# JunkyByte/deepcharuco

Hardware: AMD Instinct MI355X
Metric: frames/sec end-to-end (detect+refine) at 320x240; corner-id match vs ref (higher is better)
Workload: dtype f32; 1 GPU; bs=32/GPU x1 GPU(s) = 32 frames of 320x240, full detect+refine pipeline (BASELINE configs[1]); preset=cfg2, batch_per_gpu=32, global_batch=32, height=240, width=320, corner_pool_per_gpu=2048, frames=board, truncated_frames=0, distinct_ids_in_batch=16, parallelism=frames sharded, 1 process/GPU x1

## Files before the change

### deepcharuco_amd/_lib.py

```python
from __future__ import annotations

import ctypes as C
import os
import subprocess
from typing import Optional

_HERE = os.path.dirname(os.path.abspath(__file__))
LIB_PATH = os.environ.get("DCX_LIB") or os.path.join(_HERE, "libdeepcharuco_amd.so")
CSRC = os.path.join(_HERE, "csrc")

_lib: Optional[C.CDLL] = None


class DcxError(RuntimeError):
    def __init__(self, code: int, where: str):
        self.code = code
        try:
            msg = lib().dcx_error_string(code).decode()
        except Exception:
            msg = "?"
        super().__init__(f"{where} failed with code {code}: {msg}")


def build(force: bool = False, verbose: bool = False) -> str:
    cmd = ["make", "-C", CSRC, "-j4"]
    if force:
        subprocess.run(["make", "-C", CSRC, "clean"], check=True, capture_output=not verbose)
    res = subprocess.run(cmd, capture_output=True, text=True)
    if res.returncode != 0:
        raise RuntimeError("building libdeepcharuco_amd.so failed:\n" + res.stdout[-4000:] + res.stderr[-8000:])
    if verbose:
        print(res.stdout)
    return LIB_PATH


_vp, _i, _l, _sz = C.c_void_p, C.c_int, C.c_long, C.c_size_t

SIGNATURES = {
    "dcx_version": (C.c_char_p, []),
    "dcx_error_string": (C.c_char_p, [_i]),
    "dcx_detector_create": (_i, [C.POINTER(_vp), C.POINTER(_vp), _i, _i]),
    "dcx_detector_destroy": (_i, [_vp]),
    "dcx_refiner_create": (_i, [C.POINTER(_vp), C.POINTER(_vp), _i]),
    "dcx_refiner_destroy": (_i, [_vp]),
    "dcx_detector_workspace_bytes": (_sz, [_vp, _i, _i, _i]),
    "dcx_refiner_workspace_bytes": (_sz, [_vp, _i]),
    "dcx_bgr2gray": (_i, [_vp, _l, _i, _i, _i, _i, _vp, _vp]),
    "dcx_bgr2gray_legacy14": (_i, [_vp, _l, _i, _i, _i, _i, _vp, _vp]),
    "dcx_pre_image": (_i, [_vp, _vp, _sz, _vp]),
    "dcx_detector_forward": (_i, [_vp, _vp, _l, _i, _vp, _i, _i, _i, _vp, _sz, _vp, _vp, _vp]),
    "dcx_detector_decode": (_i, [_vp, _i, _i, _i, _vp, _i, _i, _vp, _vp, _vp, _vp, _vp]),
    "dcx_pred_to_keypoints": (_i, [_vp, _vp, _i, _i, _i, _i, _i, _i, _i, _vp, _vp, _vp, _vp, _vp]),
    "dcx_label_to_keypoints": (_i, [_vp, _vp, _i, _i, _i, _i, _i, _vp, _vp, _vp, _vp, _vp]),
    "dcx_build_patch_table": (_i, [_vp, _vp, _i, _i, _vp, _vp, _vp]),
    "dcx_extract_patches_u8": (_i, [_vp, _l, _i, _i, _i, _vp, _vp, _i, _vp, _vp]),
    "dcx_extract_patches_f32": (_i, [_vp, _i, _i, _vp, _vp, _i, _vp, _vp]),
    "dcx_refiner_forward": (_i, [_vp, _vp, _i, _vp, _vp, _vp, _sz, _vp, _vp, _vp, _vp]),
    "dcx_argmax2d": (_i, [_vp, _i, _i, _i, _vp, _vp]),
    "dcx_pipeline_workspace_bytes": (_sz, [_vp, _vp, _i, _i, _i, _i]),
    "dcx_infer_batch": (_i, [_vp, _vp, _vp, _l, _i, _i, _i, _i, _i, _i, _i, _vp, _sz, _vp, _vp, _vp, _vp, _vp, _vp]),
    "dcx_front_bytes": (_sz, [_vp, _i, _i, _i]),
    "dcx_detector_front": (_i, [_vp, _vp, _l, _i, _i, _i, _i, _i, _vp, _sz, _vp]),
    "dcx_infer_batch_prefetched": (_i, [_vp, _vp, _vp, _l, _i, _i, _i, _i, _i, _i, _i, _vp, _sz, _vp, _sz, _vp, _vp, _vp, _vp, _vp,
                                       _vp, _vp]),
    "dcx_stream_synchronize": (_i, [_vp]),
    "dcx_solve_pnp_pool": (_i, [_vp, _vp, _vp, _vp, _i, _i, _i, _i, C.c_double, C.POINTER(C.c_double), C.POINTER(C.c_double), _i,
                               _vp, _vp, _vp]),
    "dcx_solve_pnp_ransac_workspace_bytes": (_sz, [_i, _i, _i]),
    "dcx_solve_pnp_ransac_pool": (_i, [_vp, _vp, _vp, _vp, _i, _i, _i, _i, C.c_double, C.POINTER(C.c_double), C.POINTER(C.c_double), _i,
                                      _i, C.c_double, _i, C.c_uint, _vp, _sz, _vp, _vp, _vp, _vp, _vp]),
    "dcx_calibrate_workspace_bytes": (_sz, [_i]),
    "dcx_calibrate_pool": (_i, [_vp, _vp, _vp, _vp, _i, _i, _i, _i, C.c_double, _i, _i, _vp, _sz, _vp, _vp,
                               C.POINTER(C.c_double), _vp]),
    "dcx_calibrate_flags_workspace_bytes": (_sz, [_i, _i]),
    "dcx_calibrate_flags_pool": (_i, [_vp, _vp, _vp, _vp, _i, _i, _i, _i, C.c_double, _i, _i, _i, C.POINTER(C.c_double),
                                     C.POINTER(C.c_double), _i, _vp, _sz, _vp, _vp, C.POINTER(C.c_double), _vp]),
    "dcx_calibrate_ransac_workspace_bytes": (_sz, [_i, _i, _i]),
    "dcx_calibrate_ransac_pool": (_i, [_vp, _vp, _vp, _vp, _i, _i, _i, _i, C.c_double, _i, _i, _i, C.c_double, C.c_double, _i, _i,
                                      C.c_uint, _vp, _sz, _vp, _vp, _vp, _vp, C.POINTER(C.c_double), _vp]),
    "dcx_stereo_calibrate_workspace_bytes": (_sz, [_i, _i, _i]),
    "dcx_stereo_calibrate_pool": (_i, [_vp] * 10 + [_i, _i, _i, _i, _i, C.c_double, C.POINTER(C.c_double), C.POINTER(C.c_double), _i,
                                      C.POINTER(C.c_double), C.POINTER(C.c_double), _i, _vp, _sz, _vp, _vp, _vp,
                                      C.POINTER(C.c_double), _vp]),
    "dcx_stereo_calibrate_models_pool": (_i, [_vp] * 10 + [_i, _i, _i, _i, _i, C.c_double, C.POINTER(C.c_double),
                                             C.POINTER(C.c_double), _i, C.POINTER(C.c_double), C.POINTER(C.c_double), _i, _i, _i,
                                             _vp, _sz, _vp, _vp, _vp, C.POINTER(C.c_double), _vp]),
    "dcx_rig_calibrate_workspace_bytes": (_sz, [_i, _i, C.POINTER(C.c_int)]),
    "dcx_rig_calibrate_pool": (_i, [_i, _vp, _i, _i, _i, C.c_double, _vp, _sz, _vp, _vp, _vp, C.POINTER(C.c_int32),
                                   C.POINTER(C.c_double), _vp]),
    "dcx_rig_calibrate_models_pool": (_i, [_i, _vp, C.POINTER(C.c_int), _i, _i, _i, C.c_double, _vp, _sz, _vp, _vp, _vp,
                                          C.POINTER(C.c_int32), C.POINTER(C.c_double), _vp]),
    "dcx_rig_pose_workspace_bytes": (_sz, [_i, _i, C.POINTER(C.c_int)]),
    "dcx_rig_pose_pool": (_i, [_i, _vp, C.POINTER(C.c_int), C.POINTER(C.c_double), _i, _i, _i, C.c_double, _vp, _sz, _vp, _vp, _vp, _vp,
                              _vp, _vp, _vp]),
    "dcx_undistort_rectify_map": (_i, [C.POINTER(C.c_double), C.POINTER(C.c_double), _i, C.POINTER(C.c_double),
                                      C.POINTER(C.c_double), _i, _i, _vp, _vp]),
    "dcx_rectify_points_pool": (_i, [_vp, _vp, _i, C.POINTER(C.c_double), C.POINTER(C.c_double), _i, C.POINTER(C.c_double),
                                    C.POINTER(C.c_double), _vp, _vp]),
    "dcx_remap_u8": (_i, [_vp, _l, _i, _i, _i, _i, _vp, _i, _i, _i, _i, _vp, _vp]),
    "dcx_fisheye_solve_pnp_pool": (_i, [_vp, _vp, _vp, _vp, _i, _i, _i, _i, C.c_double, C.POINTER(C.c_double), C.POINTER(C.c_double),
                                       _vp, _vp, _vp]),
    "dcx_fisheye_solve_pnp_ransac_pool": (_i, [_vp, _vp, _vp, _vp, _i, _i, _i, _i, C.c_double, C.POINTER(C.c_double),
                                              C.POINTER(C.c_double), _i, C.c_double, _i, C.c_uint, _vp, _sz, _vp, _vp, _vp, _vp, _vp]),
    "dcx_fisheye_calibrate_workspace_bytes": (_sz, [_i]),
    "dcx_fisheye_calibrate_pool": (_i, [_vp, _vp, _vp, _vp, _i, _i, _i, _i, C.c_double, _i, _i, C.c_double, _vp, _sz, _vp, _vp,
                                       C.POINTER(C.c_double), _vp]),
    "dcx_calibrate_uncertainty_workspace_bytes": (_sz, [_i]),
    "dcx_calibrate_uncertainty_pool": (_i, [_vp, _vp, _vp, _vp, _i, _i, _i, _i, C.c_double, _i, C.POINTER(C.c_double), _vp, _vp, _vp,
                                           _vp, _sz, _vp, _vp, _vp]),
    "dcx_fisheye_undistort_rectify_map": (_i, [C.POINTER(C.c_double), C.POINTER(C.c_double), C.POINTER(C.c_double),
                                              C.POINTER(C.c_double), _i, _i, _vp, _vp]),
    "dcx_fisheye_rectify_points_pool": (_i, [_vp, _vp, _i, C.POINTER(C.c_double), C.POINTER(C.c_double), C.POINTER(C.c_double),
                                            C.POINTER(C.c_double), _vp, _vp]),
    "dcx_resize_u8": (_i, [_vp, _l, _i, _i, _i, _i, _i, _i, _i, _i, _vp, _vp]),
    "dcx_resize_area_u8": (_i, [_vp, _l, _i, _i, _i, _i, _i, _i, _i, _vp, _vp]),
    "dcx_sgm_workspace_bytes": (_sz, [_i, _i, _i, _i]),
    "dcx_sgm_u8": (_i, [_vp, _l, _i, _vp, _l, _i, _i, _i, _i, _i, _i, _i, _i, _i, _i, _vp, _vp, _sz, _vp]),
    "dcx_sgm_u8_paths": (_i, [_vp, _l, _i, _vp, _l, _i, _i, _i, _i, _i, _i, _i, _i, _i, _i, _i, _vp, _vp, _sz, _vp]),
    "dcx_disparity_to_points": (_i, [_vp, _i, _i, _i, _i, C.POINTER(C.c_double), _vp, _vp]),
    "dcx_filter_speckles_workspace_bytes": (_sz, [_i, _i, _i]),
    "dcx_filter_speckles_s16": (_i, [_vp, _vp, _i, _i, _i, _i, _i, _i, _vp, _sz, _vp]),
    "dcx_conv_layer": (_i, [_vp, _i, _i, _i, _i, _vp, _vp, _vp, _vp, _vp, _vp, _i, _i, _i, _i, _i, _i, _vp, _vp]),
    "dcx_nchw_to_c4": (_i, [_vp, _i, _i, _i, _i, _vp, _vp]),
    "dcx_c4_to_nchw": (_i, [_vp, _i, _i, _i, _i, _vp, _vp]),
    "dcx_set_timing": (_i, [_i]),
    "dcx_get_timing": (_i, []),
    "dcx_profile_enabled": (_i, []),
    "dcx_last_timings": (_i, [C.POINTER(C.c_float)]),
    "dcx_conv_pick_name": (C.c_char_p, [_i] * 8),
    "dcx_conv_pick_name_ups": (C.c_char_p, [_i] * 9),
    "dcx_set_deterministic": (_i, [_i]),
    "dcx_get_deterministic": (_i, []),
    "dcx_calibrate_xcd": (_i, [_i, C.POINTER(C.c_float), _vp]),
    "dcx_set_xcd_weights": (_i, [C.POINTER(C.c_float)]),
    "dcx_get_xcd_weights": (_i, [C.POINTER(C.c_float)]),
    "dcx_set_tail_fence": (_i, [_i]),
    "dcx_get_tail_fence": (_i, []),
    "dcx_profile_enable": (_i, [_i]),
    "dcx_profile_count": (_i, []),
    "dcx_profile_filter": (_i, [_i]),
    "dcx_profile_sample": (_i, [_i]),
    "dcx_profile_fetch": (_i, [C.POINTER(_i), C.POINTER(_i), C.POINTER(_i), C.POINTER(C.c_double), C.POINTER(C.c_float), _i]),
    "dcx_profile_kernel_name": (C.c_char_p, [_i]),
    "dcx_profile_clocks": (_i, [C.POINTER(C.c_float), _i]),
    "dcx_profile_probe_words": (_i, [_i, C.POINTER(C.c_ulonglong)]),
}


def lib() -> C.CDLL:
    global _lib
    if _lib is None:
        if not os.path.exists(LIB_PATH):
            raise RuntimeError(
                f"{LIB_PATH} not found: build it with `python -c 'import __graft_entry__ as g; g.build()'` "
                f"or `make -C {CSRC}`. deepcharuco_amd has no CPU / stock-PyTorch fallback.")
        handle = C.CDLL(LIB_PATH)
        for name, (res, args) in SIGNATURES.items():
            fn = getattr(handle, name)
            fn.restype = res
            fn.argtypes = args
        _lib = handle
    return _lib


def csrc_sha256() -> str:
    import hashlib
    h = hashlib.sha256()
    for name in sorted(os.listdir(CSRC)):
        if name.endswith((".hip", ".h")):
            with open(os.path.join(CSRC, name), "rb") as f:
                h.update(name.encode())
                h.update(f.read())
    return h.hexdigest()


def check(rc: int, where: str) -> None:
    if rc != 0:
        raise DcxError(rc, where)


def ptr(t) -> Optional[int]:
    if t is None:
        return None
    return t.data_ptr()


def current_stream() -> int:
    import torch
    return torch.cuda.current_stream().cuda_stream
```

### deepcharuco_amd/csrc/dcx_api.hip

```cpp
#include "dcx_common.h"

#include <math.h>
#include <stdlib.h>
#include <string.h>
#include <new>
#include <vector>

namespace {

constexpr float kBnEps = 1e-5f;

inline size_t align_up(size_t v, size_t a) { return (v + a - 1) / a * a; }


std::vector<float> pack_conv(const float* w, int cout, int cin, int ks, int cout_pad) {
    const int taps = ks * ks, cq = cin / 4;
    std::vector<float> out((size_t)taps * cq * cout_pad * 4, 0.0f);
    for (int o = 0; o < cout; ++o)
        for (int i = 0; i < cin; ++i)
            for (int t = 0; t < taps; ++t)
                out[(((size_t)t * cq + (i >> 2)) * cout_pad + o) * 4 + (i & 3)] = w[((size_t)o * cin + i) * taps + t];
    return out;
}

std::vector<float> pack_conv_wino2(const float* w, int cout, int cin, int cout_pad) {
    const int cq = cin / 4;
    std::vector<float> out((size_t)16 * cq * cout_pad * 4, 0.0f);
    for (int o = 0; o < cout; ++o)
        for (int i = 0; i < cin; ++i) {
            const float* g = w + ((size_t)o * cin + i) * 9;
            float h[4][3], u[4][4];
            for (int kx = 0; kx < 3; ++kx) {
                const float g0 = g[kx], g1 = g[3 + kx], g2 = g[6 + kx];
                h[0][kx] = g0; h[1][kx] = ((g0 + g1) + g2) * 0.5f; h[2][kx] = ((g0 - g1) + g2) * 0.5f; h[3][kx] = g2;
            }
            for (int xi = 0; xi < 4; ++xi) {
                u[xi][0] = h[xi][0]; u[xi][1] = ((h[xi][0] + h[xi][1]) + h[xi][2]) * 0.5f;
                u[xi][2] = ((h[xi][0] - h[xi][1]) + h[xi][2]) * 0.5f; u[xi][3] = h[xi][2];
            }
            for (int pos = 0; pos < 16; ++pos)
                out[(((size_t)pos * cq + (i >> 2)) * cout_pad + o) * 4 + (i & 3)] = u[pos >> 2][pos & 3];
        }
    return out;
}

std::vector<float> pack_conv_ups2(const float* w, int cout, int cin, int cout_pad) {
    const int cq = cin / 4;
    std::vector<float> out((size_t)16 * cq * cout_pad * 4, 0.0f);
    static const int lo[2][2] = {{0, 1}, {0, 2}}, hi[2][2] = {{0, 2}, {1, 2}};
    for (int o = 0; o < cout; ++o)
        for (int i = 0; i < cin; ++i) {
            const float* g = w + ((size_t)o * cin + i) * 9;
            for (int ph = 0; ph < 4; ++ph)
                for (int tap = 0; tap < 4; ++tap) {
                    const int a = ph >> 1, b = ph & 1, dy = tap >> 1, dx = tap & 1;
                    float r[3];
                    for (int kx = 0; kx < 3; ++kx) {
                        r[kx] = g[lo[a][dy] * 3 + kx];
                        for (int ky = lo[a][dy] + 1; ky <= hi[a][dy]; ++ky) r[kx] = r[kx] + g[ky * 3 + kx];
                    }
                    float v = r[lo[b][dx]];
                    for (int kx = lo[b][dx] + 1; kx <= hi[b][dx]; ++kx) v = v + r[kx];
                    out[(((size_t)(ph * 4 + tap) * cq + (i >> 2)) * cout_pad + o) * 4 + (i & 3)] = v;
                }
        }
    return out;
}

std::vector<float> pack_conv_ups2w(const float* w, int cout, int cin, int cout_pad) {
    const int cq = cin / 4;
    const std::vector<float> ph = pack_conv_ups2(w, cout, cin, cout_pad);
    std::vector<float> out((size_t)36 * cq * cout_pad * 4, 0.0f);
    const size_t plane = (size_t)cq * cout_pad * 4;
    for (int p = 0; p < 4; ++p)
        for (size_t e = 0; e < plane; ++e) {
            float wc[2][3];
            for (int dy = 0; dy < 2; ++dy) {
                const float g0 = ph[(size_t)(p * 4 + dy * 2 + 0) * plane + e], g1 = ph[(size_t)(p * 4 + dy * 2 + 1) * plane + e];
                wc[dy][0] = g0; wc[dy][1] = g0 + g1; wc[dy][2] = g1;
            }
            for (int nu = 0; nu < 3; ++nu) {
                out[(size_t)(p * 9 + 0 * 3 + nu) * plane + e] = wc[0][nu];
                out[(size_t)(p * 9 + 1 * 3 + nu) * plane + e] = wc[0][nu] + wc[1][nu];
                out[(size_t)(p * 9 + 2 * 3 + nu) * plane + e] = wc[1][nu];
            }
        }
    return out;
}

void fold_bn(const float* gamma, const float* bbeta, const float* mean, const float* var, int c, int c_pad,
             std::vector<float>& alpha, std::vector<float>& beta) {
    alpha.assign(c_pad, 0.0f);
    beta.assign(c_pad, 0.0f);
    for (int i = 0; i < c; ++i) {
        const float inv = 1.0f / sqrtf(var[i] + kBnEps);
        const float a = gamma[i] * inv;
        alpha[i] = a;
        beta[i] = bbeta[i] - mean[i] * a;
    }
}

std::vector<float> pad_vec(const float* v, int c, int c_pad) {
    std::vector<float> out(c_pad, 0.0f);
    memcpy(out.data(), v, sizeof(float) * c);
    return out;
}

struct DevLayer {
    float* w = nullptr;
    float* w_wino2 = nullptr;
    float* w_ups2w = nullptr;
    float* bias = nullptr;
    float* alpha = nullptr;
    float* beta = nullptr;
    int cin = 0, cout = 0, cout_pad = 0, ks = 3;
};

int upload(const std::vector<float>& h, float** d) {
    DCX_CHECK_HIP(hipMalloc((void**)d, h.size() * sizeof(float)));
    DCX_CHECK_HIP(hipMemcpy(*d, h.data(), h.size() * sizeof(float), hipMemcpyHostToDevice));
    return 0;
}

void free_layer(DevLayer& l) {
    if (l.w) (void)hipFree(l.w);
    if (l.w_wino2) (void)hipFree(l.w_wino2);
    if (l.w_ups2w) (void)hipFree(l.w_ups2w);
    if (l.bias) (void)hipFree(l.bias);
    if (l.alpha) (void)hipFree(l.alpha);
    if (l.beta) (void)hipFree(l.beta);
    l = DevLayer();
}

struct HostConv {
    const float* w; const float* b;
    const float* g; const float* be; const float* mu; const float* var;
};

int make_layer(const HostConv& h, int cin, int cout, int ks, DevLayer* out, bool ups_input = false) {
    DevLayer l;
    l.cin = cin; l.cout = cout; l.ks = ks;
    l.cout_pad = dcx_conv_cout_pad(cout);
    int rc = upload(pack_conv(h.w, cout, cin, ks, l.cout_pad), &l.w);
    if (rc == 0) rc = upload(pad_vec(h.b, cout, l.cout_pad), &l.bias);
    if (rc == 0 && h.g != nullptr) {
        std::vector<float> al, be;
        fold_bn(h.g, h.be, h.mu, h.var, cout, l.cout_pad, al, be);
        for (int i = 0; i < cout; ++i) be[i] = fmaf(h.b[i], al[i], be[i]);
        rc = upload(al, &l.alpha);
        if (rc == 0) rc = upload(be, &l.beta);
        if (rc == 0 && ks == 3) rc = upload(pack_conv_wino2(h.w, cout, cin, l.cout_pad), &l.w_wino2);
        if (rc == 0 && ks == 3 && ups_input) rc = upload(pack_conv_ups2w(h.w, cout, cin, l.cout_pad), &l.w_ups2w);
    }
    if (rc != 0) { free_layer(l); return rc; }
    *out = l;
    return 0;
}

int make_first_layer(const HostConv& h, DevLayer* out) {
    DevLayer l;
    l.cin = 1; l.cout = 64; l.cout_pad = 64; l.ks = 3;
    std::vector<float> w(9 * 64);
    for (int o = 0; o < 64; ++o)
        for (int t = 0; t < 9; ++t) w[t * 64 + o] = h.w[o * 9 + t];
    std::vector<float> al, be;
    fold_bn(h.g, h.be, h.mu, h.var, 64, 64, al, be);
    int rc = upload(w, &l.w);
    if (rc == 0) rc = upload(pad_vec(h.b, 64, 64), &l.bias);
    if (rc == 0) rc = upload(al, &l.alpha);
    if (rc == 0) rc = upload(be, &l.beta);
    if (rc != 0) { free_layer(l); return rc; }
    *out = l;
    return 0;
}

bool g_timing = false;
hipEvent_t g_ev[5];
bool g_ev_ok = false;
int timing_mark(int i, hipStream_t s) {
    if (!g_timing) return 0;
    if (!g_ev_ok) {
        for (auto& e : g_ev) DCX_CHECK_HIP(hipEventCreate(&e));
        g_ev_ok = true;
    }
    DCX_CHECK_HIP(hipEventRecord(g_ev[i], s));
    return 0;
}

}

struct dcx_detector {
    int n_ids = 16;
    DevLayer first;
    DevLayer enc[7];
    DevLayer heads_a;
    DevLayer head_loc, head_ids;
};

struct dcx_refiner {
    DevLayer first;
    DevLayer mid[9];
    DevLayer head_a;
    float* head_w = nullptr;
    float head_b = 0.f;
};

namespace {

struct Carve {
    size_t off = 0;
    size_t take(size_t bytes) { const size_t at = off; off = align_up(off + bytes, 256); return at; }
};

int check_pool(int pool) { return pool <= 0 || pool > (1 << 22) ? DCX_E_SHAPE : 0; }

struct DetWs {
    size_t buf0, buf1, loc, ids, codes, conf, total;
    int ids_quads;
};
DetWs det_layout(int n_ids, int b, int h, int w) {
    DetWs L;
    const size_t hw = (size_t)h * w, cells = (size_t)(h / 8) * (w / 8);
    L.ids_quads = (n_ids + 1 + 3) / 4;
    Carve c;
    L.buf0 = c.take((size_t)b * 64 * hw * 4);
    L.buf1 = c.take((size_t)b * 16 * hw * 4);
    L.loc = c.take((size_t)b * 68 * cells * 4);
    L.ids = c.take((size_t)b * L.ids_quads * 4 * cells * 4);
    L.codes = c.take((size_t)b * cells * 4);
    L.conf = c.take((size_t)b * cells * 8);
    L.total = c.off;
    return L;
}

struct RefWs {
    size_t buf0, buf1, pval, pidx, total;
};
constexpr int kRefTiles = 32;
RefWs ref_layout(int p) {
    RefWs L;
    Carve c;
    L.buf0 = c.take((size_t)p * 65536 * 4);
    L.buf1 = c.take((size_t)p * 65536 * 4);
    L.pval = c.take((size_t)p * kRefTiles * 4);
    L.pidx = c.take((size_t)p * kRefTiles * 4);
    L.total = c.off;
    return L;
}

DcxConvArgs conv_args(const DevLayer& l, const float* in, int n, int in_cq_total, int in_cq_off, int hin, int win,
                      int ups, int pad, float* out, int out_cq_total, const int* n_limit) {
    DcxConvArgs a;
    memset(&a, 0, sizeof(a));
    a.in = in; a.w = l.w; a.w_wino2 = l.w_wino2; a.w_ups2w = l.w_ups2w; a.bias = l.bias; a.alpha = l.alpha; a.beta = l.beta; a.out = out;
    a.n_limit = n_limit;
    a.n = n; a.in_cq_total = in_cq_total; a.in_cq_off = in_cq_off; a.cin = l.cin;
    a.hin = hin; a.win = win; a.ups = ups; a.pad = pad;
    a.ho = (hin << ups) + 2 * pad - (l.ks - 1);
    a.wo = (win << ups) + 2 * pad - (l.ks - 1);
    a.out_cq_total = out_cq_total; a.out_cq_off = 0;
    a.cout_pad = l.cout_pad; a.cout_quads = (l.cout + 3) / 4; a.cout_real = l.cout;
    return a;
}

}

extern "C" const char* dcx_version(void) { return "deepcharuco_amd 0.1 (gfx950, fp32 MFMA)"; }

extern "C" const char* dcx_error_string(int code) {
    switch (code) {
        case 0: return "ok";
        case DCX_E_ARG: return "DCX_E_ARG: null pointer or bad scalar argument";
        case DCX_E_SHAPE: return "DCX_E_SHAPE: unsupported shape (H/W below 8, patches not 24x24, batch x kmax too large, ...)";
        case DCX_E_WS: return "DCX_E_WS: workspace too small";
        case DCX_E_NIDS: return "DCX_E_NIDS: n_ids outside [1, 63] or dust_bin outside [0, 255]";
        default: return code > 0 ? hipGetErrorString((hipError_t)code) : "unknown dcx error";
    }
}

extern "C" int dcx_detector_create(dcx_detector** out, const float* const* t, int n_tensors, int n_ids) {
    if (!out || !t) return DCX_E_ARG;
    if (n_ids < 1 || n_ids > 63) return DCX_E_NIDS;
    if (n_tensors != 64) return DCX_E_ARG;
    for (int i = 0; i < n_tensors; ++i)
        if (!t[i]) return DCX_E_ARG;
    if (const int rc = dcx_xcd_init()) return rc;
    dcx_detector* d = new (std::nothrow) dcx_detector();
    if (!d) return (int)hipErrorOutOfMemory;
    d->n_ids = n_ids;
    auto hc = [&](int base, bool bn) {
        return HostConv{t[base], t[base + 1], bn ? t[base + 2] : nullptr, bn ? t[base + 3] : nullptr,
                        bn ? t[base + 4] : nullptr, bn ? t[base + 5] : nullptr};
    };
    static const int enc_cin[7] = {64, 64, 64, 64, 128, 128, 128};
    static const int enc_cout[7] = {64, 64, 64, 128, 128, 128, 128};
    int rc = make_first_layer(hc(0, true), &d->first);
    for (int i = 0; rc == 0 && i < 7; ++i) rc = make_layer(hc(6 + 6 * i, true), enc_cin[i], enc_cout[i], 3, &d->enc[i]);
    if (rc == 0) {
        const HostConv pa = hc(48, true), da = hc(56, true);
        const size_t wsz = (size_t)256 * 128 * 9;
        std::vector<float> w(2 * wsz), b(512), g(512), be(512), mu(512), var(512);
        memcpy(w.data(), pa.w, wsz * 4); memcpy(w.data() + wsz, da.w, wsz * 4);
        auto cat = [](std::vector<float>& dst, const float* x, const float* y) {
            memcpy(dst.data(), x, 256 * 4); memcpy(dst.data() + 256, y, 256 * 4);
        };
        cat(b, pa.b, da.b); cat(g, pa.g, da.g); cat(be, pa.be, da.be); cat(mu, pa.mu, da.mu); cat(var, pa.var, da.var);
        rc = make_layer(HostConv{w.data(), b.data(), g.data(), be.data(), mu.data(), var.data()}, 128, 512, 3,
                        &d->heads_a);
    }
    if (rc == 0) rc = make_layer(hc(54, false), 256, 65, 1, &d->head_loc);
    if (rc == 0) rc = make_layer(hc(62, false), 256, n_ids + 1, 1, &d->head_ids);
    if (rc != 0) { dcx_detector_destroy(d); return rc; }
    *out = d;
    return 0;
}

extern "C" int dcx_detector_destroy(dcx_detector* d) {
    if (!d) return 0;
    free_layer(d->first);
    for (auto& l : d->enc) free_layer(l);
    free_layer(d->heads_a); free_layer(d->head_loc); free_layer(d->head_ids);
    delete d;
    return 0;
}

extern "C" size_t dcx_detector_workspace_bytes(const dcx_detector* det, int batch, int height, int width) {
    if (!det || batch <= 0 || height <= 0 || width <= 0) return 0;
    return det_layout(det->n_ids, batch, height, width).total;
}

namespace {
int detector_front(const dcx_detector* det, const uint8_t* d_frames_u8, long frame_stride, int pitch, int pix,
                   const float* d_images_f32, int batch, int h, int w, float* out, int32_t* zero_words, int n_zero, hipStream_t s) {
    int rc;
    const int pt0 = dcx_prof_begin(DCX_PROF_CONV1A, batch, 0, s);
    if (d_frames_u8)
        rc = dcx_launch_conv1_u8(d_frames_u8, frame_stride, pitch, pix, batch, h, w, 1, det->first.w, det->first.bias,
                                 det->first.alpha, det->first.beta, out, nullptr, zero_words, n_zero, s);
    else
        rc = dcx_launch_conv1_f32(d_images_f32, (long)h * w, w, batch, h, w, 1, det->first.w, det->first.bias,
                                  det->first.alpha, det->first.beta, out, nullptr, s);
    if (rc) return rc;
    return dcx_prof_end(pt0, s);
}

int detector_run(const dcx_detector* det, const uint8_t* d_frames_u8, long frame_stride, int pitch, int pix,
                 const float* d_images_f32, int batch, int height, int width, void* d_ws, size_t ws_bytes,
                 bool with_heads, float* d_loc_nchw, float* d_ids_nchw, int32_t* zero_words, int n_zero, const float* act0,
                 void* stream) {
    if (!det || !d_ws) return DCX_E_ARG;
    if ((d_frames_u8 == nullptr) == (d_images_f32 == nullptr)) return DCX_E_ARG;
    if (batch <= 0 || height < 8 || width < 8) return DCX_E_SHAPE;
    const DetWs L = det_layout(det->n_ids, batch, height, width);
    if (ws_bytes < L.total) return DCX_E_WS;
    hipStream_t s = (hipStream_t)stream;
    char* ws = (char*)d_ws;
    float* buf0 = (float*)(ws + L.buf0);
    float* buf1 = (float*)(ws + L.buf1);
    float* loc = (float*)(ws + L.loc);
    float* ids = (float*)(ws + L.ids);
    const int h = height, w = width;
    int rc;
    if (act0 == nullptr && (rc = detector_front(det, d_frames_u8, frame_stride, pitch, pix, d_images_f32, batch, h, w, buf0,
                                                zero_words, n_zero, s)))
        return rc;
    struct Step { int layer, div, pool; };
    static const Step steps[7] = {{0, 1, 1}, {1, 2, 0}, {2, 2, 1}, {3, 4, 0}, {4, 4, 1}, {5, 8, 0}, {6, 8, 0}};
    const float* src = act0 ? act0 : buf0;
    float* dst = buf1;
    for (const Step& st : steps) {
        const DevLayer& l = det->enc[st.layer];
        DcxConvArgs a = conv_args(l, src, batch, l.cin / 4, 0, h / st.div, w / st.div, 0, 1, dst, l.cout / 4, nullptr);
        rc = dcx_launch_conv_mfma(a, 3, st.pool, DCX_EPI_BNRELU, s);
        if (rc) return rc;
        src = dst; dst = dst == buf1 ? buf0 : buf1;
    }
    const int hc = h / 8, wc = w / 8;
    {
        DcxConvArgs a = conv_args(det->heads_a, src, batch, 32, 0, hc, wc, 0, 1, dst, 128, nullptr);
        rc = dcx_launch_conv_mfma(a, 3, 0, DCX_EPI_BNRELU, s);
        if (rc) return rc;
    }
    if (!with_heads) return 0;
    {
        DcxConvArgs a = conv_args(det->head_loc, dst, batch, 128, 0, 1, hc * wc, 0, 0, loc, 17, nullptr);
        rc = dcx_launch_conv_mfma(a, 1, 0, DCX_EPI_RAW, s);
        if (rc) return rc;
    }
    {
        DcxConvArgs a = conv_args(det->head_ids, dst, batch, 128, 64, 1, hc * wc, 0, 0, ids, L.ids_quads, nullptr);
        rc = dcx_launch_conv_mfma(a, 1, 0, DCX_EPI_RAW, s);
        if (rc) return rc;
    }
    if (d_loc_nchw) { rc = dcx_c4_to_nchw(loc, batch, 65, hc, wc, d_loc_nchw, stream); if (rc) return rc; }
    if (d_ids_nchw) { rc = dcx_c4_to_nchw(ids, batch, det->n_ids + 1, hc, wc, d_ids_nchw, stream); if (rc) return rc; }
    return 0;
}
}

extern "C" int dcx_detector_forward(const dcx_detector* det, const uint8_t* d_frames_u8, long frame_stride, int pitch,
                                    const float* d_images_f32, int batch, int height, int width, void* d_ws,
                                    size_t ws_bytes, float* d_loc_nchw, float* d_ids_nchw, void* stream) {
    return detector_run(det, d_frames_u8, frame_stride, pitch, DCX_PIX_GRAY8, d_images_f32, batch, height, width, d_ws, ws_bytes, true,
                        d_loc_nchw, d_ids_nchw, nullptr, 0, nullptr, stream);
}

extern "C" int dcx_detector_decode(const dcx_detector* det, int batch, int height, int width, void* d_ws,
                                   int dust_bin, int kmax, int32_t* d_counts, int32_t* d_rows, int32_t* d_loc_argmax,
                                   int32_t* d_ids_argmax, void* stream) {
    if (!det || !d_ws) return DCX_E_ARG;
    if (batch <= 0 || height < 8 || width < 8) return DCX_E_SHAPE;
    const DetWs L = det_layout(det->n_ids, batch, height, width);
    const int hc = height / 8, wc = width / 8;
    const long cells = (long)hc * wc;
    char* ws = (char*)d_ws;
    DcxLogitView lv{(const float*)(ws + L.loc), 17 * 4 * cells, 4 * cells, 4, 1};
    DcxLogitView iv{(const float*)(ws + L.ids), (long)L.ids_quads * 4 * cells, 4 * cells, 4, 1};
    return dcx_launch_decode(lv, iv, batch, 65, det->n_ids + 1, hc, wc, dust_bin, kmax, d_counts, d_rows,
                             d_loc_argmax, d_ids_argmax, (int32_t*)(ws + L.codes), (hipStream_t)stream);
}

extern "C" int dcx_refiner_create(dcx_refiner** out, const float* const* t, int n_tensors) {
    if (!out || !t) return DCX_E_ARG;
    if (n_tensors != 68) return DCX_E_ARG;
    for (int i = 0; i < n_tensors; ++i)
        if (!t[i]) return DCX_E_ARG;
    if (const int rc = dcx_xcd_init()) return rc;
    dcx_refiner* r = new (std::nothrow) dcx_refiner();
    if (!r) return (int)hipErrorOutOfMemory;
    auto hc = [&](int base) { return HostConv{t[base], t[base + 1], t[base + 2], t[base + 3], t[base + 4], t[base + 5]}; };
    static const int cin[9] = {64, 64, 128, 128, 128, 128, 128, 128, 64};
    static const int cout[9] = {64, 128, 128, 128, 128, 128, 128, 64, 64};
    int rc = make_first_layer(hc(0), &r->first);
    for (int i = 0; rc == 0 && i < 9; ++i) rc = make_layer(hc(6 + 6 * i), cin[i], cout[i], 3, &r->mid[i], i == 5 || i == 7);
    if (rc == 0) rc = make_layer(hc(60), 64, 64, 3, &r->head_a, true);
    if (rc == 0) {
        std::vector<float> hw(t[66], t[66] + 64);
        rc = upload(hw, &r->head_w);
        r->head_b = t[67][0];
    }
    if (rc != 0) { dcx_refiner_destroy(r); return rc; }
    *out = r;
    return 0;
}

extern "C" int dcx_refiner_destroy(dcx_refiner* r) {
    if (!r) return 0;
    free_layer(r->first);
    for (auto& l : r->mid) free_layer(l);
    free_layer(r->head_a);
    if (r->head_w) (void)hipFree(r->head_w);
    delete r;
    return 0;
}

extern "C" size_t dcx_refiner_workspace_bytes(const dcx_refiner* rf, int max_patches) {
    if (!rf || max_patches <= 0) return 0;
    return ref_layout(max_patches).total;
}

namespace {
struct FrameSrc { const uint8_t* frames; long frame_stride; int pitch, pix, height, width; };
int refiner_run(const dcx_refiner* rf, const float* d_patches, const FrameSrc* fsrc, int max_patches, int n_hint,
                const int32_t* d_total, const int32_t* d_table, void* d_ws, size_t ws_bytes, int32_t* d_corners, float* d_xy,
                float* d_heat, void* stream) {
    if (!rf || !d_ws || ((d_patches == nullptr) == (fsrc == nullptr))) return DCX_E_ARG;
    if (fsrc != nullptr && (d_total == nullptr || d_table == nullptr)) return DCX_E_ARG;
    if (d_xy != nullptr && d_table == nullptr) return DCX_E_ARG;
    if (const int rc = check_pool(max_patches)) return rc;
    const RefWs L = ref_layout(max_patches);
    if (ws_bytes < L.total) return DCX_E_WS;
    hipStream_t s = (hipStream_t)stream;
    char* ws = (char*)d_ws;
    float* buf0 = (float*)(ws + L.buf0);
    float* buf1 = (float*)(ws + L.buf1);
    const int p = max_patches;
    const int* lim = d_total;
    const int pt0 = dcx_prof_begin(DCX_PROF_PATCHES, p, lim != nullptr, s);
    int rc = fsrc != nullptr
        ? dcx_launch_conv1_patches_u8(fsrc->frames, fsrc->frame_stride, fsrc->pitch, fsrc->pix, fsrc->height, fsrc->width, d_table, d_total, p, n_hint,
                                      rf->first.w, rf->first.bias, rf->first.alpha, rf->first.beta, buf0, s)
        : dcx_launch_conv1_f32(d_patches, 576, 24, p, 24, 24, 0, rf->first.w, rf->first.bias, rf->first.alpha,
                               rf->first.beta, buf0, lim, s);
    if (rc) return rc;
    if ((rc = dcx_prof_end(pt0, s))) return rc;
    struct Step { int layer, hin, ups, pad, pool; };
    static const Step steps[9] = {
        {0, 22, 0, 0, 0},
        {1, 20, 0, 0, 0},
        {2, 18, 0, 0, 1},
        {3, 8, 0, 1, 0},
        {4, 8, 0, 1, 0},
        {5, 8, 1, 1, 0},
        {6, 16, 0, 1, 0},
        {7, 16, 1, 1, 0},
        {8, 32, 0, 1, 0},
    };
    float* src = buf0;
    float* dst = buf1;
    for (const Step& st : steps) {
        const DevLayer& l = rf->mid[st.layer];
        DcxConvArgs a = conv_args(l, src, p, l.cin / 4, 0, st.hin, st.hin, st.ups, st.pad, dst, l.cout / 4, lim);
        a.n_hint = lim != nullptr ? n_hint : 0;
        rc = dcx_launch_conv_mfma(a, 3, st.pool, DCX_EPI_BNRELU, s);
        if (rc) return rc;
        float* t = src; src = dst; dst = t;
    }
    int heat_tiles = 0;
    {
        DcxConvArgs a = conv_args(rf->head_a, src, p, 16, 0, 32, 32, 1, 1, nullptr, 16, lim);
        a.head_w = rf->head_w; a.head_b = rf->head_b; a.heat = d_heat;
        a.part_val = (float*)(ws + L.pval); a.part_idx = (int*)(ws + L.pidx);
        heat_tiles = dcx_conv_heat_tiles(a.ho, a.wo, a.w_ups2w != nullptr ? 1 : 0);
        if (heat_tiles <= 0 || heat_tiles > kRefTiles) return DCX_E_SHAPE;
        rc = dcx_launch_conv_mfma(a, 3, 0, DCX_EPI_HEAT, s);
        if (rc) return rc;
    }
    const int pt1 = dcx_prof_begin(DCX_PROF_FINALIZE, p, lim != nullptr, s);
    rc = dcx_launch_refine_finalize((const float*)(ws + L.pval), (const int*)(ws + L.pidx), heat_tiles, 64, p, lim,
                                    d_table, d_corners, d_xy, s);
    if (rc) return rc;
    return dcx_prof_end(pt1, s);
}
}

extern "C" int dcx_refiner_forward(const dcx_refiner* rf, const float* d_patches, int max_patches,
                                   const int32_t* d_total, const int32_t* d_table, void* d_ws, size_t ws_bytes,
                                   int32_t* d_corners, float* d_xy, float* d_heat, void* stream) {
    return refiner_run(rf, d_patches, nullptr, max_patches, 0, d_total, d_table, d_ws, ws_bytes, d_corners, d_xy, d_heat, stream);
}

namespace {
struct PipeWs { size_t det, table, ctrl, ref, total; int ctrl_words; };
inline int ctrl_word_count(int b) { return 64 + b; }
struct FrontWs { size_t act, ctrl, total; int ctrl_words; };
FrontWs front_layout(int b, int h, int w) {
    FrontWs F;
    Carve c;
    F.act = c.take((size_t)b * 64 * h * w * 4);
    F.ctrl_words = ctrl_word_count(b);
    F.ctrl = c.take((size_t)F.ctrl_words * 4);
    F.total = c.off;
    return F;
}
PipeWs pipe_layout(const dcx_detector* det, const dcx_refiner* rf, int b, int h, int w, int pool) {
    PipeWs L;
    Carve c;
    L.det = c.take(det_layout(det->n_ids, b, h, w).total);
    L.table = c.take((size_t)pool * 16);
    L.ctrl_words = ctrl_word_count(b);
    L.ctrl = c.take((size_t)L.ctrl_words * 4);
    L.ref = c.take(rf ? ref_layout(pool).total : 0);
    L.total = c.off;
    return L;
}
}

extern "C" size_t dcx_pipeline_workspace_bytes(const dcx_detector* det, const dcx_refiner* rf, int batch, int height,
                                               int width, int pool) {
    if (!det || batch <= 0 || height <= 0 || width <= 0 || pool <= 0) return 0;
    return pipe_layout(det, rf, batch, height, width, pool).total;
}

extern "C" size_t dcx_front_bytes(const dcx_detector* det, int batch, int height, int width) {
    if (!det || batch <= 0 || height <= 0 || width <= 0) return 0;
    return front_layout(batch, height, width).total;
}

namespace {
int check_batch_args(const dcx_detector* det, const uint8_t* d_frames_u8, int pitch, int pixel_format, int batch, int height,
                     int width) {
    if (!det || !d_frames_u8) return DCX_E_ARG;
    if (!dcx_pix_valid(pixel_format)) return DCX_E_ARG;
    if (batch <= 0 || batch > (1 << 20) || height < 8 || width < 8) return DCX_E_SHAPE;
    if (pitch < width * dcx_pix_bpp(pixel_format)) return DCX_E_SHAPE;
    return 0;
}
}

extern "C" int dcx_detector_front(const dcx_detector* det, const uint8_t* d_frames_u8, long frame_stride, int pitch,
                                  int pixel_format, int batch, int height, int width, void* d_front, size_t front_bytes,
                                  void* stream) {
    if (!d_front) return DCX_E_ARG;
    if (const int rc = check_batch_args(det, d_frames_u8, pitch, pixel_format, batch, height, width)) return rc;
    const FrontWs F = front_layout(batch, height, width);
    if (front_bytes < F.total) return DCX_E_WS;
    char* front = (char*)d_front;
    return detector_front(det, d_frames_u8, frame_stride, pitch, pixel_format, nullptr, batch, height, width, (float*)(front + F.act),
                          (int32_t*)(front + F.ctrl), F.ctrl_words, (hipStream_t)stream);
}

namespace {
int infer_range(const dcx_detector* det, const dcx_refiner* rf, const uint8_t* d_frames_u8, long frame_stride, int pitch, int pix,
                int batch, int height, int width, int dust_bin, int pool, char* ws, size_t ws_bytes, char* front,
                hipEvent_t detector_done, int32_t* d_counts, int32_t* d_starts, int32_t* d_rows, float* d_xy, float* d_conf,
                hipStream_t s, bool timing) {
    void* stream = (void*)s;
    const PipeWs L = pipe_layout(det, rf, batch, height, width, pool);
    if (ws_bytes < L.total) return DCX_E_WS;
    int rc = timing ? timing_mark(0, s) : 0;
    if (rc) return rc;
    const FrontWs F = front_layout(batch, height, width);
    int32_t* ctrl = (int32_t*)(front ? front + F.ctrl : ws + L.ctrl);
    rc = detector_run(det, d_frames_u8, frame_stride, pitch, pix, nullptr, batch, height, width, ws + L.det, L.table - L.det,
                      false, nullptr, nullptr, ctrl, L.ctrl_words, front ? (const float*)(front + F.act) : nullptr, stream);
    if (rc) return rc;
    if (detector_done) DCX_CHECK_HIP(hipEventRecord(detector_done, s));
    if (timing && (rc = timing_mark(1, s))) return rc;
    int32_t* table = (int32_t*)(ws + L.table);
    {
        const DetWs D = det_layout(det->n_ids, batch, height, width);
        const int hc = height / 8, wc = width / 8;
        const float* act = (const float*)(ws + L.det + D.buf0);
        int32_t* codes = (int32_t*)(ws + L.det + D.codes);
        DcxPoolOut po;
        po.tickets = ctrl + 64; po.cursor = ctrl; po.counts = d_counts; po.starts = d_starts; po.rows = d_rows;
        po.table = rf ? table : nullptr; po.conf = d_conf; po.conf_cells = (float*)(ws + L.det + D.conf);
        po.wc = wc; po.pool = pool;
        const int pt = dcx_prof_begin(DCX_PROF_TAIL, batch, 0, s);
        rc = dcx_launch_tail(act, batch, hc * wc, det->head_loc.w, det->head_loc.bias, det->head_ids.w, det->head_ids.bias,
                             det->head_ids.cout_pad, det->n_ids + 1, dust_bin, codes, nullptr, nullptr, &po, s);
        if (rc) return rc;
        if ((rc = dcx_prof_end(pt, s))) return rc;
    }
    if (timing && (rc = timing_mark(2, s))) return rc;
    if (rf == nullptr) return timing ? timing_mark(3, s) : 0;
    const long expect = (long)batch * det->n_ids;
    const FrameSrc src{d_frames_u8, frame_stride, pitch, pix, height, width};
    rc = refiner_run(rf, nullptr, &src, pool, (int)(expect < pool ? expect : pool), ctrl, table,
                     ws + L.ref, L.total - L.ref, nullptr, d_xy, nullptr, stream);
    if (rc) return rc;
    return timing ? timing_mark(3, s) : 0;
}
}

extern "C" int dcx_infer_batch(const dcx_detector* det, const dcx_refiner* rf, const uint8_t* d_frames_u8,
                               long frame_stride, int pitch, int pixel_format, int batch, int height, int width, int dust_bin,
                               int pool, void* d_ws, size_t ws_bytes, int32_t* d_counts, int32_t* d_starts, int32_t* d_rows,
                               float* d_xy, float* d_conf, void* stream) {
    if (!d_ws || !d_counts || !d_starts || !d_rows) return DCX_E_ARG;
    if (rf != nullptr && d_xy == nullptr) return DCX_E_ARG;
    if (const int rc = check_batch_args(det, d_frames_u8, pitch, pixel_format, batch, height, width)) return rc;
    if (const int rc = check_pool(pool)) return rc;
    if (const int rc = dcx_check_dust_bin(dust_bin)) return rc;
    hipStream_t s = (hipStream_t)stream;
    char* ws = (char*)d_ws;
    return infer_range(det, rf, d_frames_u8, frame_stride, pitch, pixel_format, batch, height, width, dust_bin, pool, ws, ws_bytes,
                       nullptr, nullptr, d_counts, d_starts, d_rows, d_xy, d_conf, s, true);
}

extern "C" int dcx_infer_batch_prefetched(const dcx_detector* det, const dcx_refiner* rf, const uint8_t* d_frames_u8,
                                          long frame_stride, int pitch, int pixel_format, int batch, int height, int width,
                                          int dust_bin, int pool, void* d_ws, size_t ws_bytes, void* d_front, size_t front_bytes,
                                          int32_t* d_counts, int32_t* d_starts, int32_t* d_rows, float* d_xy, float* d_conf,
                                          void* detector_done_event, void* stream) {
    if (!d_ws || !d_front || !d_counts || !d_starts || !d_rows) return DCX_E_ARG;
    if (rf != nullptr && d_xy == nullptr) return DCX_E_ARG;
    if (const int rc = check_batch_args(det, d_frames_u8, pitch, pixel_format, batch, height, width)) return rc;
    if (const int rc = check_pool(pool)) return rc;
    if (const int rc = dcx_check_dust_bin(dust_bin)) return rc;
    if (front_bytes < front_layout(batch, height, width).total) return DCX_E_WS;
    return infer_range(det, rf, d_frames_u8, frame_stride, pitch, pixel_format, batch, height, width, dust_bin, pool, (char*)d_ws,
                       ws_bytes, (char*)d_front, (hipEvent_t)detector_done_event, d_counts, d_starts, d_rows, d_xy, d_conf,
                       (hipStream_t)stream, true);
}

extern "C" int dcx_stream_synchronize(void* stream) { return (int)hipStreamSynchronize((hipStream_t)stream); }

extern "C" int dcx_set_timing(int enabled) { g_timing = enabled != 0; return 0; }
extern "C" int dcx_get_timing(void) { return g_timing ? 1 : 0; }

extern "C" int dcx_last_timings(float* h_ms4) {
    if (!h_ms4) return DCX_E_ARG;
    if (!g_ev_ok) return DCX_E_ARG;
    DCX_CHECK_HIP(hipEventElapsedTime(&h_ms4[0], g_ev[0], g_ev[1]));
    DCX_CHECK_HIP(hipEventElapsedTime(&h_ms4[1], g_ev[1], g_ev[2]));
    DCX_CHECK_HIP(hipEventElapsedTime(&h_ms4[2], g_ev[2], g_ev[3]));
    DCX_CHECK_HIP(hipEventElapsedTime(&h_ms4[3], g_ev[0], g_ev[3]));
    return 0;
}

extern "C" int dcx_conv_layer(const float* d_in, int n, int cin, int hin, int win, const float* h_w, const float* h_b,
                              const float* h_g, const float* h_be, const float* h_mu, const float* h_var, int cout,
                              int ksize, int pad, int ups, int pool, int relu, float* d_out, void* stream) {
    if (!d_in || !h_w || !h_b || !d_out) return DCX_E_ARG;
    if (cin % 32 != 0 || (ksize != 3 && ksize != 1) || n <= 0) return DCX_E_SHAPE;
    const bool bn = h_g != nullptr;
    if (bn != (relu != 0)) return DCX_E_ARG;
    if (bn && (!h_be || !h_mu || !h_var)) return DCX_E_ARG;
    if (const int rc = dcx_xcd_init()) return rc;
    DevLayer l;
    int rc = make_layer(HostConv{h_w, h_b, h_g, h_be, h_mu, h_var}, cin, cout, ksize, &l, ups != 0);
    if (rc) return rc;
    DcxConvArgs a;
    if (ksize == 1) {
        if (pad != 0 || ups != 0 || pool != 0) { free_layer(l); return DCX_E_SHAPE; }
        a = conv_args(l, d_in, n, cin / 4, 0, 1, hin * win, 0, 0, d_out, (cout + 3) / 4, nullptr);
    } else {
        a = conv_args(l, d_in, n, cin / 4, 0, hin, win, ups, pad, d_out, (cout + 3) / 4, nullptr);
    }
    rc = dcx_launch_conv_mfma(a, ksize, pool, bn ? DCX_EPI_BNRELU : DCX_EPI_RAW, (hipStream_t)stream);
    hipError_t e = hipStreamSynchronize((hipStream_t)stream);
    free_layer(l);
    if (rc) return rc;
    return (int)e;
}
```

### deepcharuco_amd/csrc/dcx_common.h

```cpp
#pragma once
#include <hip/hip_runtime.h>
#include <stdint.h>
#include <stddef.h>

#include "../../include/deepcharuco_amd.h"

#define DCX_CHECK_HIP(expr)                              \
    do {                                                 \
        hipError_t _e = (expr);                          \
        if (_e != hipSuccess) return (int)_e;            \
    } while (0)


enum DcxEpilogue {
    DCX_EPI_BNRELU = 0,
    DCX_EPI_RAW = 1,
    DCX_EPI_HEAT = 2,
};

struct DcxConvArgs {
    const float* in;
    const float* w;
    const float* w_wino2;
    const float* w_ups2w;
    const float* bias;
    const float* alpha;
    const float* beta;
    float* out;
    const int* n_limit;
    unsigned long long* clk_probe;
    int probe_u0;
    const float* head_w;
    float head_b;
    float* heat;
    float* part_val;
    int* part_idx;
    int n;
    int n_hint;
    int in_cq_total, in_cq_off;
    int cin;
    int hin, win;
    int ups;
    int pad;
    int ho, wo;
    int out_cq_total, out_cq_off;
    int cout_pad;
    int cout_quads;
    int cout_real;
    int tiles_x, tiles_y;
    int xcd_walk;
    const int* xcd_cum;
    unsigned long long* xcd_stat;
    int ct_outer;
};

int dcx_launch_conv_mfma(DcxConvArgs a, int ks, int pool, int epi, hipStream_t stream);
int dcx_xcd_init();
int dcx_conv_cout_pad(int cout);
int dcx_conv_heat_tiles(int ho, int wo, int ups);

enum { DCX_PROF_CONV1A = 100, DCX_PROF_PATCHES = 101, DCX_PROF_TAIL = 102, DCX_PROF_FINALIZE = 103 };
int dcx_prof_begin(int kernel_id, int n, int limited, hipStream_t s);
int dcx_prof_end(int token, hipStream_t s);


constexpr bool dcx_pix_valid(int pix) { return pix == DCX_PIX_GRAY8 || pix == DCX_PIX_BGR8 || pix == DCX_PIX_BGR8_LEGACY14; }
constexpr int dcx_pix_bpp(int pix) { return pix == DCX_PIX_GRAY8 ? 1 : 3; }
int dcx_launch_conv1_u8(const uint8_t* frames, long frame_stride, int pitch, int pix, int n, int h, int w, int pad,
                        const float* w9x64, const float* bias, const float* alpha, const float* beta,
                        float* out_c4, const int* n_limit, int32_t* zero_words, int n_zero, hipStream_t s);
int dcx_launch_conv1_f32(const float* images, long image_stride, int pitch, int n, int h, int w, int pad,
                         const float* w9x64, const float* bias, const float* alpha, const float* beta,
                         float* out_c4, const int* n_limit, hipStream_t s);

struct DcxLogitView {
    const float* p;
    long sb, sq, sp, sc;
};
inline int dcx_check_dust_bin(int dust_bin, int last = 255) { return dust_bin < 0 || dust_bin > last ? DCX_E_NIDS : 0; }
int dcx_launch_decode(DcxLogitView loc, DcxLogitView ids, int batch, int n_loc, int n_ids1, int hc, int wc,
                      int dust_bin, int kmax, int32_t* counts, int32_t* rows,
                      int32_t* loc_argmax, int32_t* ids_argmax, int32_t* codes_scratch, hipStream_t s);
struct DcxPoolOut {
    int32_t* tickets;
    int32_t* cursor;
    int32_t* counts;
    int32_t* starts;
    int32_t* rows;
    int32_t* table;
    float* conf;
    float* conf_cells;
    int wc, pool;
};
int dcx_launch_tail(const float* act_c4_512, int batch, int cells, const float* w_loc, const float* b_loc,
                    const float* w_ids, const float* b_ids, int ids_cout_pad, int n_ids1, int dust_bin,
                    int32_t* codes, int32_t* loc_argmax, int32_t* ids_argmax, const DcxPoolOut* po, hipStream_t s);
int dcx_launch_compact(const int32_t* codes, int batch, int hc, int wc, int dust_bin, int kmax, int32_t* counts,
                       int32_t* rows, hipStream_t s);
int dcx_launch_conv1_patches_u8(const uint8_t* frames, long frame_stride, int pitch, int pix, int h, int w, const int32_t* table,
                                const int* total, int max_patches, int n_hint, const float* w9x64, const float* bias,
                                const float* alpha, const float* beta, float* out_c4, hipStream_t s);
int dcx_launch_refine_finalize(const float* part_val, const int* part_idx, int tiles, int wo,
                               int max_patches, const int* total, const int32_t* table,
                               int32_t* corners, float* xy, hipStream_t s);
```

### deepcharuco_amd/csrc/dcx_conv_mfma.hip

```cpp
#include "dcx_conv_mfma.h"
#include "dcx_conv_wino2h.h"
#include "dcx_conv_wino2hs.h"
#include "dcx_conv_wino2p.h"
#include "dcx_conv_wino2ps.h"

#include <stdlib.h>
#include <string.h>
#include <atomic>
#include <mutex>
#include <vector>

namespace {

enum { FAM_DIRECT = 0,
       FAM_W2H = 3,
       FAM_W2P = 4 };

struct CfgEntry {
    int cout_tile, cap, th, tw, ks, pool, epi, acc_tiles;
    int inlane;
    int group;
    int fam;
    int (*launch)(DcxConvArgs, hipStream_t);
    const char* name;
};

#define DCX_CFG(WM, WN, MT, NT, TH, TW, KS, POOL, EPI)                                              \
    { WM * MT * 32, WN * NT * 32, TH, TW, KS, POOL, EPI, MT * NT, ((POOL) != 0 && MT == 1 && NT == 4) ? 1 : 0, 1, FAM_DIRECT, \
      &dcx_conv_launch_cfg<DcxConvCfg<WM, WN, MT, NT, TH, TW, KS, (POOL) != 0, EPI>>,                 \
      "dcx_conv_mfma_kernel<DcxConvCfg<" #WM "," #WN "," #MT "," #NT "," #TH "," #TW "," #KS "," #POOL "," #EPI ">>" }

#define DCX_W2HCFG(TH, TW, POOL, G)                                                                   \
    { 64, 128, TH, TW, 3, POOL, DCX_EPI_BNRELU, 8, 0, G, FAM_W2H,                                            \
      &dcx_conv_wino2h_launch_cfg<DcxWino2hCfg<TH, TW, (POOL) != 0, G>>,                                   \
      "dcx_conv_wino2h_kernel<DcxWino2hCfg<" #TH "," #TW "," #POOL "," #G ">>" }
#define DCX_W2HCFG_S(TH, TW, POOL)                                                                    \
    { 64, 64, TH, TW, 3, POOL, DCX_EPI_BNRELU, 4, 0, 1, FAM_W2H,                                             \
      &dcx_conv_wino2h_launch_cfg<DcxWino2hCfg<TH, TW, (POOL) != 0, 1, 1>>,                                \
      "dcx_conv_wino2h_kernel<DcxWino2hCfg<" #TH "," #TW "," #POOL ",1,1>>" }

#define DCX_W2HSCFG(POOL, CG)                                                                         \
    { 16 * CG, 64, 8, 8, 3, POOL, DCX_EPI_BNRELU, 1, 0, 1, FAM_W2H,                                          \
      &dcx_conv_wino2hs_launch_cfg<DcxWino2hsCfg<(POOL) != 0, CG>>,                                        \
      "dcx_conv_wino2hs_kernel<DcxWino2hsCfg<" #POOL "," #CG ">>" }

#define DCX_W2PCFG(TH, TW, EPI, G)                                                                    \
    { 64, 128, TH, TW, 3, 0, EPI, 5, 0, G, FAM_W2P,                                                          \
      &dcx_conv_wino2p_launch_cfg<DcxWino2pCfg<TH, TW, EPI, G>>,                                           \
      "dcx_conv_wino2p_kernel<DcxWino2pCfg<" #TH "," #TW "," #EPI "," #G ">>" }

#define DCX_W2PSCFG(CG)                                                                               \
    { 16 * CG, 64, 8, 8, 3, 0, DCX_EPI_BNRELU, 1, 0, 1, FAM_W2P,                                             \
      &dcx_conv_wino2ps_launch_cfg<DcxWino2psCfg<CG>>,                                                     \
      "dcx_conv_wino2ps_kernel<DcxWino2psCfg<" #CG ">>" }

const CfgEntry kCfgs[] = {
    DCX_CFG(1, 4, 2, 2, 8, 32, 3, 0, DCX_EPI_BNRELU),
    DCX_CFG(2, 2, 1, 1, 8, 8, 3, 0, DCX_EPI_BNRELU),
    DCX_CFG(2, 2, 1, 1, 8, 8, 3, 1, DCX_EPI_BNRELU),
    DCX_CFG(2, 2, 1, 4, 8, 32, 3, 1, DCX_EPI_BNRELU),
    DCX_CFG(1, 4, 2, 2, 1, 256, 1, 0, DCX_EPI_RAW),
    DCX_CFG(1, 4, 2, 2, 8, 32, 3, 0, DCX_EPI_HEAT),
    DCX_W2HCFG(8, 16, 0, 1),
    DCX_W2HCFG(8, 16, 1, 1),
    DCX_W2HCFG(6, 20, 0, 1),
    DCX_W2HCFG(6, 20, 1, 1),
    DCX_W2HCFG(8, 8, 0, 2),
    DCX_W2HCFG_S(8, 8, 0),
    DCX_W2HCFG_S(8, 8, 1),
    DCX_W2HSCFG(0, 4), DCX_W2HSCFG(0, 2), DCX_W2HSCFG(0, 1),
    DCX_W2HSCFG(1, 4), DCX_W2HSCFG(1, 2), DCX_W2HSCFG(1, 1),
    DCX_W2PCFG(8, 16, DCX_EPI_BNRELU, 1),
    DCX_W2PCFG(8, 16, DCX_EPI_HEAT, 1),
    DCX_W2PCFG(8, 8, DCX_EPI_BNRELU, 2),
    DCX_W2PSCFG(4), DCX_W2PSCFG(2), DCX_W2PSCFG(1),
};

int g_deterministic = -1;
int dcx_deterministic_enabled() {
    if (g_deterministic < 0) g_deterministic = dcx_env_knob(DCX_KNOB_DETERMINISTIC) ? 1 : 0;
    return g_deterministic;
}

int family_of(int cin, int cout_pad, int ks, int pool, int epi, int ups_phase) {
    if (dcx_deterministic_enabled() || ks != 3 || epi == DCX_EPI_RAW || cin < 2 * DCX_CCH) return FAM_DIRECT;
    if (ups_phase && !pool && (epi == DCX_EPI_BNRELU || (epi == DCX_EPI_HEAT && cout_pad == 64))) return FAM_W2P;
    if (epi == DCX_EPI_BNRELU) return FAM_W2H;
    return FAM_DIRECT;
}

const CfgEntry* pick(int n, int cin, int ho, int wo, int cout_pad, int ks, int pool, int epi, int allow_group = 1, int ups = 0) {
    const CfgEntry* best = nullptr;
    double best_cost = 0.0;
    const int n_cu = dcx_device_cu_count();
    auto can_run = [&](const CfgEntry& c) {
        if (c.ks != ks || c.pool != pool || c.epi != epi || cout_pad % c.cout_tile != 0) return false;
        if (c.fam == FAM_W2P) return ups == 1 && cin >= 2 * DCX_CCH && (epi != DCX_EPI_HEAT || cout_pad == 64) &&
                                     (c.group == 1 || (ho <= 2 * c.th && wo <= 2 * c.tw));
        if (c.fam == FAM_W2H) return cin >= 2 * DCX_CCH && (c.group == 1 || (allow_group && ups == 0 && ho <= c.th && wo <= c.tw));
        return true;
    };
    const char* force = getenv("DCX_FORCE_CFG");
    if (force != nullptr && force[0] != 0) {
        for (const CfgEntry& c : kCfgs)
            if (strcmp(c.name, force) == 0 && can_run(c)) return &c;
    }
    const int fam = family_of(cin, cout_pad, ks, pool, epi, ups);
    const int units = cin / DCX_CCH;
    for (const CfgEntry& c : kCfgs) {
        if (c.fam != fam || !can_run(c)) continue;
        const int ph = c.fam == FAM_W2P ? 2 : 1;
        const long tiles = (long)((ho / ph + c.th - 1) / c.th) * ((wo / ph + c.tw - 1) / c.tw);
        const long items = (long)((n + c.group - 1) / c.group) * (cout_pad / c.cout_tile) * tiles * (ph * ph);
        const double rounds = (double)((items + n_cu - 1) / n_cu);
        double cost;
        if (c.fam == FAM_W2H) {
            double item_cost = (double)units * (64 * 64.0 + (c.tw == 20 ? 700.0 : 560.0)) + 2600.0;
            if (c.acc_tiles == 4)
                item_cost = (double)units * (32 * 64.0 + 600.0) + 2000.0;
            if (c.acc_tiles == 1) {
                const int w2hs = dcx_env_knob(DCX_KNOB_W2HS);
                const int w2hs_rounds = dcx_env_knob(DCX_KNOB_W2HS_ROUNDS);
                if (!(w2hs & (c.cout_tile / 16)) || items > (long)w2hs_rounds * n_cu) continue;
                item_cost = (double)units * (8 * 64.0 * (c.cout_tile / 16) + 400.0) + 1200.0;
                if (w2hs_rounds > 1 && items > n_cu) item_cost *= 0.8;
            }
            cost = rounds * item_cost * (1.0 + 1e-6 * (double)items);
        } else if (c.fam == FAM_W2P) {
            double item_cost = (double)units * (72 * 32.0 + 500.0) + 2400.0;
            if (c.acc_tiles == 1) {
                const int w2ps = dcx_env_knob(DCX_KNOB_W2PS);
                if (!(w2ps & (c.cout_tile / 16)) || items > n_cu) continue;
                item_cost = (double)units * (12 * 32.0 * ((3 * (c.cout_tile / 16) + 3) / 4) + 400.0) + 1200.0;
            }
            cost = rounds * item_cost * (1.0 + 1e-6 * (double)items);
        } else {
            const int steps = ks * ks * (DCX_CCH / 8);
            const double item_cost = (double)units * steps * (4 * c.acc_tiles) * 64.0 + units * 520.0
                                   + c.acc_tiles * 16 * (c.inlane ? 35.0 : (pool ? 60.0 : 40.0));
            cost = rounds * item_cost;
            if (c.cout_tile == 64 && c.cap == 256) cost *= 0.999;
        }
        if (best == nullptr || cost < best_cost) { best_cost = cost; best = &c; }
    }
    return best;
}

struct ProfRec { int kernel_id, n, limited; double flops_per_image; hipEvent_t e0, e1; int slot; };
unsigned long long* g_clk_dev = nullptr;
constexpr int kClkSlots = 1024;
constexpr int kClkWords = 64;
bool g_prof = false;
int g_prof_filter = -1;
int g_prof_every = 1;
long g_prof_seen = 0;
std::vector<ProfRec> g_recs;
std::vector<hipEvent_t> g_pool;
size_t g_pool_used = 0;

hipEvent_t prof_event() {
    if (g_pool_used == g_pool.size()) {
        hipEvent_t e;
        if (hipEventCreate(&e) != hipSuccess) return nullptr;
        g_pool.push_back(e);
    }
    return g_pool[g_pool_used++];
}

}

extern "C" const char* dcx_conv_pick_name(int n, int cin, int ho, int wo, int cout, int ks, int pool, int epi) {
    const CfgEntry* c = pick(n, cin, ho, wo, dcx_conv_cout_pad(cout), ks, pool, epi);
    return c ? c->name : "";
}
extern "C" const char* dcx_conv_pick_name_ups(int n, int cin, int ho, int wo, int cout, int ks, int pool, int epi, int ups) {
    const CfgEntry* c = pick(n, cin, ho, wo, dcx_conv_cout_pad(cout), ks, pool, epi, ups == 0, ups);
    return c ? c->name : "";
}

extern "C" int dcx_set_deterministic(int enabled) { g_deterministic = enabled ? 1 : 0; return 0; }
extern "C" int dcx_get_deterministic(void) { return dcx_deterministic_enabled(); }

extern "C" int dcx_profile_enable(int enabled) {
    g_prof = enabled != 0;
    if (g_prof) {
        g_recs.clear(); g_pool_used = 0;
        if (g_clk_dev != nullptr) {
            DCX_CHECK_HIP(hipMemset(g_clk_dev, 0, sizeof(unsigned long long) * kClkWords * kClkSlots));
            DCX_CHECK_HIP(hipStreamSynchronize(nullptr));
        }
    }
    return 0;
}
extern "C" int dcx_profile_enabled(void) { return g_prof ? 1 : 0; }
extern "C" int dcx_profile_filter(int kernel_id) { g_prof_filter = kernel_id; return 0; }
extern "C" int dcx_profile_sample(int every) { g_prof_every = every > 1 ? every : 1; g_prof_seen = 0; return 0; }
extern "C" int dcx_profile_count(void) { return (int)g_recs.size(); }
extern "C" const char* dcx_profile_kernel_name(int id) {
    const int n = (int)(sizeof(kCfgs) / sizeof(kCfgs[0]));
    switch (id) {
        case DCX_PROF_CONV1A: return "dcx_conv1_kernel (detector conv1a)";
        case DCX_PROF_PATCHES: return "dcx_conv1_patches_kernel (RefineNet conv1a + patch gather)";
        case DCX_PROF_TAIL: return "dcx_tail_kernel (1x1 heads + arg-max + compaction)";
        case DCX_PROF_FINALIZE: return "dcx_refine_finalize_kernel";
        default: break;
    }
    return id >= 0 && id < n ? kCfgs[id].name : "?";
}

int dcx_prof_begin(int kernel_id, int n, int limited, hipStream_t stream) {
    if (!g_prof || g_prof_filter >= 0) return -1;
    ProfRec r;
    r.kernel_id = kernel_id; r.n = n; r.limited = limited ? 1 : 0; r.flops_per_image = 0.0;
    r.e0 = prof_event();
    r.e1 = prof_event();
    r.slot = (int)g_recs.size();
    if (!r.e0 || !r.e1 || hipEventRecord(r.e0, stream) != hipSuccess) return -1;
    g_recs.push_back(r);
    return r.slot;
}
int dcx_prof_end(int token, hipStream_t stream) {
    if (token < 0 || token >= (int)g_recs.size()) return 0;
    DCX_CHECK_HIP(hipEventRecord(g_recs[token].e1, stream));
    return 0;
}
extern "C" int dcx_profile_probe_words(int record, unsigned long long* out64) {
    if (!out64 || record < 0 || record >= kClkSlots || g_clk_dev == nullptr) return DCX_E_ARG;
    DCX_CHECK_HIP(hipMemcpy(out64, g_clk_dev + (size_t)kClkWords * record, kClkWords * 8, hipMemcpyDeviceToHost));
    return 0;
}

extern "C" int dcx_profile_clocks(float* ghz, int max_records) {
    if (!ghz) return DCX_E_ARG;
    const int n = (int)g_recs.size() < max_records ? (int)g_recs.size() : max_records;
    std::vector<unsigned long long> h((size_t)kClkWords * kClkSlots, 0ull);
    if (g_clk_dev != nullptr) DCX_CHECK_HIP(hipMemcpy(h.data(), g_clk_dev, h.size() * 8, hipMemcpyDeviceToHost));
    for (int i = 0; i < n; ++i) {
        ghz[i] = 0.f;
        if (i < kClkSlots) {
            const unsigned long long* p = &h[(size_t)kClkWords * i];
            if (p[3] > p[1]) ghz[i] = (float)((double)(p[2] - p[0]) / (double)(p[3] - p[1]) * 0.1);
        }
    }
    return n;
}

extern "C" int dcx_profile_fetch(int* kernel_ids, int* n_images, int* limited, double* flops_per_image, float* ms,
                                 int max_records) {
    if (!kernel_ids || !n_images || !limited || !flops_per_image || !ms) return DCX_E_ARG;
    int k = 0;
    for (const ProfRec& r : g_recs) {
        if (k >= max_records) break;
        float t = 0.f;
        if (hipEventElapsedTime(&t, r.e0, r.e1) != hipSuccess) t = -1.f;
        kernel_ids[k] = r.kernel_id; n_images[k] = r.n; limited[k] = r.limited;
        flops_per_image[k] = r.flops_per_image; ms[k] = t;
        ++k;
    }
    return k;
}

int dcx_conv_cout_pad(int cout) { return cout <= 64 ? 64 : (cout + 127) / 128 * 128; }

int dcx_current_device() {
    int dev = 0;
    if (hipGetDevice(&dev) != hipSuccess || dev < 0) dev = 0;
    return dev < DCX_MAX_DEVICES ? dev : DCX_MAX_DEVICES - 1;
}

int dcx_device_cu_count() {
    static int cus[DCX_MAX_DEVICES] = {};
    const int dev = dcx_current_device();
    if (cus[dev] == 0) {
        int v = 0;
        if (hipDeviceGetAttribute(&v, hipDeviceAttributeMultiprocessorCount, dev) == hipSuccess && v > 0)
            cus[dev] = v;
        else
            cus[dev] = 256;
    }
    return cus[dev];
}

int dcx_env_knob(DcxKnob k) {
    static struct { const char* name; int unset; bool read; int value; } knobs[DCX_KNOB_COUNT] = {
        {"DCX_DETERMINISTIC", 0},
        {"DCX_XCD_WALK", 1},
        {"DCX_OCC", 0},
        {"DCX_CT_OUTER", -1},
        {"DCX_W2HS", 7},
        {"DCX_W2HS_ROUNDS", 1},
        {"DCX_W2PS", 7},
        {"DCX_PROBE_U0", 0},
    };
    if (!knobs[k].read) { const char* e = getenv(knobs[k].name); knobs[k].value = e ? atoi(e) : knobs[k].unset; knobs[k].read = true; }
    return knobs[k].value;
}

namespace {
constexpr int kXcdTables = 256;
std::mutex g_xcd_mutex;
int* g_xcd_tab[DCX_MAX_DEVICES] = {};
int g_xcd_next[DCX_MAX_DEVICES] = {};
std::atomic<const int*> g_xcd_cur[DCX_MAX_DEVICES] = {};
float g_xcd_w[DCX_MAX_DEVICES][8];
int xcd_set_locked(int dev, const float* w8) {
    if (g_xcd_tab[dev] == nullptr)
        DCX_CHECK_HIP(hipMalloc((void**)&g_xcd_tab[dev], sizeof(int) * 16 * kXcdTables));
    double sum = 0.0;
    for (int x = 0; x < 8; ++x) { g_xcd_w[dev][x] = w8 ? w8[x] : 1.0f; sum += g_xcd_w[dev][x]; }
    double acc = 0.0;
    int cum[16] = {};
    for (int x = 0; x < 8; ++x) {
        g_xcd_w[dev][x] = (float)(g_xcd_w[dev][x] / sum);
        acc += g_xcd_w[dev][x];
        cum[x + 1] = x == 7 ? 65536 : (int)(acc * 65536.0 + 0.5);
    }
    int* slot = g_xcd_tab[dev] + 16 * (g_xcd_next[dev]++ % kXcdTables);
    DCX_CHECK_HIP(hipMemcpy(slot, cum, sizeof(cum), hipMemcpyHostToDevice));
    g_xcd_cur[dev].store(slot, std::memory_order_release);
    return 0;
}
int xcd_set(int dev, const float* w8) {
    std::lock_guard<std::mutex> lk(g_xcd_mutex);
    return xcd_set_locked(dev, w8);
}
}

int dcx_xcd_init() {
    const int dev = dcx_current_device();
    std::lock_guard<std::mutex> lk(g_xcd_mutex);
    return g_xcd_cur[dev].load(std::memory_order_relaxed) != nullptr ? 0 : xcd_set_locked(dev, nullptr);
}

int dcx_fill_xcd_cum(DcxConvArgs& a) {
    a.xcd_cum = g_xcd_cur[dcx_current_device()].load(std::memory_order_acquire);
    return a.xcd_cum != nullptr ? 0 : (int)hipErrorNotInitialized;
}

extern "C" int dcx_set_xcd_weights(const float* w8) {
    if (w8 != nullptr) {
        double sum = 0.0;
        for (int x = 0; x < 8; ++x) { if (!(w8[x] > 0.f)) return DCX_E_ARG; sum += w8[x]; }
        for (int x = 0; x < 8; ++x) { const double r = 8.0 * w8[x] / sum; if (r < 0.75 || r > 1.25) return DCX_E_ARG; }
    }
    return xcd_set(dcx_current_device(), w8);
}
extern "C" int dcx_get_xcd_weights(float* w8) {
    if (!w8) return DCX_E_ARG;
    const int rc = dcx_xcd_init();
    if (rc) return rc;
    const int dev = dcx_current_device();
    std::lock_guard<std::mutex> lk(g_xcd_mutex);
    for (int x = 0; x < 8; ++x) w8[x] = 8.0f * g_xcd_w[dev][x];
    return 0;
}

namespace {
__global__ void dcx_fill_hash_kernel(float* __restrict__ p, size_t n, float lo, float scale) {
    for (size_t i = (size_t)blockIdx.x * blockDim.x + threadIdx.x; i < n; i += (size_t)gridDim.x * blockDim.x) {
        unsigned h = (unsigned)i * 2654435761u;
        h ^= h >> 15; h *= 2246822519u; h ^= h >> 13;
        p[i] = lo + scale * (float)(h >> 8) * (1.0f / 16777216.0f);
    }
}
}

extern "C" int dcx_calibrate_xcd(int rounds, float* w8_out, void* stream) {
    if (rounds < 1 || rounds > 64) return DCX_E_ARG;
    hipStream_t s = (hipStream_t)stream;
    const int n = 32, c = 64, h = 240, w = 320;
    const size_t in_elems = (size_t)n * c * h * w, out_elems = in_elems / 4, w_elems = (size_t)16 * c * c;
    float *d_in = nullptr, *d_out = nullptr, *d_w = nullptr, *d_ab = nullptr;
    unsigned long long* d_stat = nullptr;
    auto cleanup = [&]() { (void)hipFree(d_in); (void)hipFree(d_out); (void)hipFree(d_w); (void)hipFree(d_ab); (void)hipFree(d_stat); };
    hipError_t e = hipMalloc((void**)&d_in, in_elems * 4);
    if (e == hipSuccess) e = hipMalloc((void**)&d_out, out_elems * 4);
    if (e == hipSuccess) e = hipMalloc((void**)&d_w, w_elems * 4);
    if (e == hipSuccess) e = hipMalloc((void**)&d_ab, 3 * c * 4);
    if (e == hipSuccess) e = hipMalloc((void**)&d_stat, 17 * 8);
    if (e == hipSuccess) e = hipMemsetD32Async((hipDeviceptr_t)d_ab, 0x3f800000, 3 * c, s);
    if (e != hipSuccess) { cleanup(); return (int)e; }
    hipLaunchKernelGGL(dcx_fill_hash_kernel, dim3(4096), dim3(256), 0, s, d_in, in_elems, -1.0f, 2.0f);
    hipLaunchKernelGGL(dcx_fill_hash_kernel, dim3(64), dim3(256), 0, s, d_w, w_elems, -0.05f, 0.1f);
    if ((e = hipGetLastError()) != hipSuccess) { cleanup(); return (int)e; }
    DcxConvArgs a;
    memset(&a, 0, sizeof(a));
    a.in = d_in; a.w = d_w; a.w_wino2 = d_w; a.bias = d_ab; a.alpha = d_ab + c; a.beta = d_ab + 2 * c; a.out = d_out;
    a.n = n; a.in_cq_total = c / 4; a.cin = c; a.hin = h; a.win = w; a.pad = 1; a.ho = h; a.wo = w;
    a.out_cq_total = c / 4; a.cout_pad = c; a.cout_quads = c / 4; a.cout_real = c;
    const int dev = dcx_current_device();
    float keep[8];
    {
        std::lock_guard<std::mutex> lk(g_xcd_mutex);
        for (int x = 0; x < 8; ++x) keep[x] = g_xcd_cur[dev].load(std::memory_order_relaxed) != nullptr ? g_xcd_w[dev][x] : 0.125f;
        const int rc = xcd_set_locked(dev, nullptr);
        if (rc) { cleanup(); return rc; }
    }
    double speed[8] = {};
    int rc = 0, used = 0;
    for (int r = 0; r < rounds + 2 && rc == 0; ++r) {
        if ((e = hipMemsetAsync(d_stat, 0, 17 * 8, s)) != hipSuccess) { rc = (int)e; break; }
        a.xcd_stat = r >= 2 ? d_stat : nullptr;
        rc = dcx_launch_conv_mfma(a, 3, 1, DCX_EPI_BNRELU, s);
        if (rc != 0 || r < 2) continue;
        unsigned long long hst[17];
        if ((e = hipMemcpyAsync(hst, d_stat, sizeof(hst), hipMemcpyDeviceToHost, s)) != hipSuccess || (e = hipStreamSynchronize(s)) != hipSuccess) { rc = (int)e; break; }
        bool ok = hst[8] != 0;
        double dur[8];
        for (int x = 0; x < 8 && ok; ++x) {
            ok = hst[9 + x] > 0;
            if (ok) { dur[x] = (double)hst[x] / (double)hst[9 + x] - (double)hst[8]; ok = dur[x] > 0.0; }
        }
        if (!ok) continue;
        for (int x = 0; x < 8; ++x) speed[x] += 1.0 / dur[x];
        ++used;
    }
    (void)hipStreamSynchronize(s);
    cleanup();
    if (rc == 0 && used > 0) {
        float w8[8];
        for (int x = 0; x < 8; ++x) w8[x] = (float)(speed[x] / used);
        rc = dcx_set_xcd_weights(w8);
    } else if (rc == 0) {
        rc = DCX_E_SHAPE;
    }
    if (rc != 0) (void)xcd_set(dev, keep);
    if (rc == 0 && w8_out != nullptr) (void)dcx_get_xcd_weights(w8_out);
    return rc;
}

int dcx_conv_heat_tiles(int ho, int wo, int ups) {
    const CfgEntry* c = pick(1 << 20, 64, ho, wo, 64, 3, 0, DCX_EPI_HEAT, 1, ups);
    if (c == nullptr) return 0;
    if (c->fam == FAM_W2P) return 4 * ((ho / 2 + c->th - 1) / c->th) * ((wo / 2 + c->tw - 1) / c->tw);
    return ((ho + c->th - 1) / c->th) * ((wo + c->tw - 1) / c->tw);
}

int dcx_launch_conv_mfma(DcxConvArgs a, int ks, int pool, int epi, hipStream_t stream) {
    if (a.in == nullptr || a.w == nullptr || a.bias == nullptr) return DCX_E_ARG;
    if (epi != DCX_EPI_HEAT && a.out == nullptr) return DCX_E_ARG;
    if (epi != DCX_EPI_RAW && (a.alpha == nullptr || a.beta == nullptr)) return DCX_E_ARG;
    if (pool && (a.ho < 2 || a.wo < 2)) return DCX_E_SHAPE;
    const CfgEntry* c = pick(epi == DCX_EPI_HEAT ? (1 << 20) : (a.n_hint > 0 && a.n_hint < a.n ? a.n_hint : a.n), a.cin, a.ho, a.wo, a.cout_pad, ks, pool, epi,
                             a.ups == 0 && a.pad == 1,
                             (a.ups == 1 && a.pad == 1 && ks == 3 && a.w_ups2w != nullptr) ? 1 : 0);
    if (c == nullptr) return DCX_E_SHAPE;
    if (!g_prof || (g_prof_filter >= 0 && g_prof_filter != (int)(c - kCfgs))) return c->launch(a, stream);
    if (g_prof_every > 1 && (g_prof_seen++ % g_prof_every) != 0) return c->launch(a, stream);
    ProfRec r;
    r.kernel_id = (int)(c - kCfgs);
    r.n = a.n;
    r.limited = a.n_limit != nullptr;
    r.flops_per_image = 2.0 * a.cout_real * a.cin * ks * ks
                      * (double)a.ho * a.wo;
    r.e0 = prof_event();
    r.e1 = prof_event();
    r.slot = (int)g_recs.size();
    if (g_clk_dev == nullptr) {
        if (hipMalloc((void**)&g_clk_dev, sizeof(unsigned long long) * kClkWords * kClkSlots) != hipSuccess) g_clk_dev = nullptr;
        else (void)hipMemset(g_clk_dev, 0, sizeof(unsigned long long) * kClkWords * kClkSlots);
    }
    if (g_clk_dev != nullptr && r.slot < kClkSlots) a.clk_probe = g_clk_dev + (size_t)kClkWords * r.slot;
    a.probe_u0 = dcx_env_knob(DCX_KNOB_PROBE_U0);
    if (!r.e0 || !r.e1) return (int)hipErrorOutOfMemory;
    DCX_CHECK_HIP(hipEventRecord(r.e0, stream));
    const int rc = c->launch(a, stream);
    DCX_CHECK_HIP(hipEventRecord(r.e1, stream));
    if (rc == 0) g_recs.push_back(r);
    return rc;
}
```

### deepcharuco_amd/csrc/dcx_conv_shared.h

```cpp
#pragma once
#include "dcx_common.h"

typedef float dcx_f32x16 __attribute__((ext_vector_type(16)));
typedef float dcx_f32x4 __attribute__((ext_vector_type(4)));
typedef float dcx_f32x2 __attribute__((ext_vector_type(2)));
typedef unsigned int dcx_u32x4 __attribute__((ext_vector_type(4)));

#define DCX_CCH 16

__device__ __forceinline__ float4 dcx_f4_zero() { return make_float4(0.f, 0.f, 0.f, 0.f); }

__device__ __forceinline__ float dcx_vmax(float x, float y) {
    float r;
    asm("v_max_f32 %0, %1, %2" : "=v"(r) : "v"(x), "v"(y));
    return r;
}
__device__ __forceinline__ dcx_f32x2 dcx_pk_add(dcx_f32x2 x, dcx_f32x2 y) {
    dcx_f32x2 r;
    asm("v_pk_add_f32 %0, %1, %2" : "=v"(r) : "v"(x), "v"(y));
    return r;
}
__device__ __forceinline__ dcx_f32x2 dcx_pk_sub(dcx_f32x2 x, dcx_f32x2 y) {
    dcx_f32x2 r;
    asm("v_pk_add_f32 %0, %1, %2 neg_lo:[0,1] neg_hi:[0,1]" : "=v"(r) : "v"(x), "v"(y));
    return r;
}
__device__ __forceinline__ float4 dcx_sub4(const float4& x, const float4& y) {
    const dcx_f32x2 lo = dcx_pk_sub(dcx_f32x2{x.x, x.y}, dcx_f32x2{y.x, y.y}), hi = dcx_pk_sub(dcx_f32x2{x.z, x.w}, dcx_f32x2{y.z, y.w});
    return make_float4(lo.x, lo.y, hi.x, hi.y);
}
__device__ __forceinline__ float4 dcx_add4(const float4& x, const float4& y) {
    const dcx_f32x2 lo = dcx_pk_add(dcx_f32x2{x.x, x.y}, dcx_f32x2{y.x, y.y}), hi = dcx_pk_add(dcx_f32x2{x.z, x.w}, dcx_f32x2{y.z, y.w});
    return make_float4(lo.x, lo.y, hi.x, hi.y);
}
__device__ __forceinline__ float4 dcx_fmas4(const float4& x, const dcx_f32x2 s, const float4& y) {
    const dcx_f32x2 lo = __builtin_elementwise_fma(dcx_f32x2{x.x, x.y}, s, dcx_f32x2{y.x, y.y});
    const dcx_f32x2 hi = __builtin_elementwise_fma(dcx_f32x2{x.z, x.w}, s, dcx_f32x2{y.z, y.w});
    return make_float4(lo.x, lo.y, hi.x, hi.y);
}
__device__ __forceinline__ float4 dcx_fma4(float4 x, float4 al, float4 be) {
    const dcx_f32x2 lo = __builtin_elementwise_fma(dcx_f32x2{x.x, x.y}, dcx_f32x2{al.x, al.y}, dcx_f32x2{be.x, be.y});
    const dcx_f32x2 hi = __builtin_elementwise_fma(dcx_f32x2{x.z, x.w}, dcx_f32x2{al.z, al.w}, dcx_f32x2{be.z, be.w});
    return make_float4(lo.x, lo.y, hi.x, hi.y);
}
#define DCX_VMAX0(x) asm volatile("v_max_f32 %0, 0, %0" : "+v"(x))
#define DCX_MAX_DPP(x, PERM) asm volatile("v_max_f32_dpp %0, %0, %0 quad_perm:" PERM " row_mask:0xf bank_mask:0xf" : "+v"(x))
__device__ __forceinline__ float4 dcx_relu_quad_max(float4 v) {
    DCX_VMAX0(v.x); DCX_VMAX0(v.y); DCX_VMAX0(v.z); DCX_VMAX0(v.w);
    DCX_MAX_DPP(v.x, "[1,0,3,2]"); DCX_MAX_DPP(v.y, "[1,0,3,2]"); DCX_MAX_DPP(v.z, "[1,0,3,2]"); DCX_MAX_DPP(v.w, "[1,0,3,2]");
    DCX_MAX_DPP(v.x, "[2,3,0,1]"); DCX_MAX_DPP(v.y, "[2,3,0,1]"); DCX_MAX_DPP(v.z, "[2,3,0,1]"); DCX_MAX_DPP(v.w, "[2,3,0,1]");
    return v;
}

constexpr unsigned DCX_OOB = 0x80000000u;
__device__ __forceinline__ float4 dcx_buffer_load_f4(__amdgpu_buffer_rsrc_t rsrc, unsigned voff, unsigned soff = 0) {
    const dcx_u32x4 v = __builtin_amdgcn_raw_buffer_load_b128(rsrc, voff, soff, 0);
    return make_float4(__uint_as_float(v.x), __uint_as_float(v.y), __uint_as_float(v.z), __uint_as_float(v.w));
}

struct DcxItem {
    int n, ct, ty, tx;
    int ph;
};
__device__ __forceinline__ DcxItem dcx_decode_item(int wi, int tiles_x, int tiles_y, int n_ct) {
    DcxItem it;
    it.tx = wi % tiles_x; wi /= tiles_x;
    it.ty = wi % tiles_y; wi /= tiles_y;
    it.ct = wi % n_ct;
    it.n = wi / n_ct;
    it.ph = 0;
    return it;
}
__device__ __forceinline__ DcxItem dcx_decode_item_phases(int wi, int tiles_x, int tiles_y, int n_ct) {
    DcxItem it;
    it.ph = wi & 3; wi >>= 2;
    it.tx = wi % tiles_x; wi /= tiles_x;
    it.ty = wi % tiles_y; wi /= tiles_y;
    it.ct = wi % n_ct;
    it.n = wi / n_ct;
    return it;
}

__device__ __forceinline__ int dcx_n_eff(const DcxConvArgs& a) {
    int n_eff = a.n;
    if (a.n_limit != nullptr) n_eff = min(n_eff, *a.n_limit);
    return n_eff;
}
__device__ __forceinline__ int dcx_xcd_bound(int total, int x, int cum) {
    const int eq = (int)(((long)total * x) >> 3);
    const int dev = (int)(((long)total * (cum - (x << 13))) >> 16);
    return eq + ((dev + (dev >= 0 ? 16 : -16)) / 32) * 32;
}
struct DcxWalk { int w, w_end, gstride; };
__device__ __forceinline__ DcxWalk dcx_item_walk(const DcxConvArgs& a, int total) {
    int w = blockIdx.x, w_end = total, gstride = gridDim.x;
    if (a.xcd_walk && (gridDim.x & 7) == 0) {
        const int x = blockIdx.x & 7;
        const int lo = dcx_xcd_bound(total, x, a.xcd_cum[x]);
        w_end = dcx_xcd_bound(total, x + 1, a.xcd_cum[x + 1]);
        gstride = gridDim.x >> 3;
        w = lo + (blockIdx.x >> 3);
    }
    return {w, w_end, gstride};
}

__device__ __forceinline__ void dcx_probe_ends(const DcxConvArgs& a, int tid, int word) {
    if (a.clk_probe != nullptr && blockIdx.x == 0 && tid == 0) {
        a.clk_probe[word] = __builtin_amdgcn_s_memtime();
        a.clk_probe[word + 1] = __builtin_amdgcn_s_memrealtime();
    }
}

__device__ __forceinline__ int dcx_f23_a(int xi) { return xi == 0 ? 0 : xi == 2 ? 2 : 1; }
__device__ __forceinline__ int dcx_f23_b(int xi) { return xi == 2 ? 1 : xi == 3 ? 3 : 2; }
__device__ __forceinline__ float dcx_f23_sgn(int xi) { return xi == 1 ? 1.f : -1.f; }
template <class T> __device__ __forceinline__ T dcx_at23(int i, int xi) { return i == 0 ? (xi < 3 ? T(1) : T(0)) : (xi == 0 ? T(0) : xi == 1 ? T(1) : T(-1)); }

constexpr int DCX_MAX_DEVICES = 64;
int dcx_current_device();
int dcx_device_cu_count();
int dcx_fill_xcd_cum(DcxConvArgs& a);
enum DcxKnob { DCX_KNOB_DETERMINISTIC, DCX_KNOB_XCD_WALK, DCX_KNOB_OCC, DCX_KNOB_CT_OUTER, DCX_KNOB_W2HS, DCX_KNOB_W2HS_ROUNDS,
               DCX_KNOB_W2PS, DCX_KNOB_PROBE_U0, DCX_KNOB_COUNT };
int dcx_env_knob(DcxKnob k);

template <void (*KERNEL)(const DcxConvArgs)>
static int dcx_launch_persistent(DcxConvArgs& a, long items, int threads, int occ, bool honour_dcx_occ, size_t lds_bytes, int max_dyn_lds,
                                 hipStream_t stream, void (*after_walk)(DcxConvArgs&) = nullptr) {
    if (items <= 0 || items > 0x7fffffffL) return DCX_E_SHAPE;
    if (honour_dcx_occ) {
        const int occ_env = dcx_env_knob(DCX_KNOB_OCC);
        if (occ_env > 0 && occ_env < occ) occ = occ_env;
    }
    const long resident = (long)occ * dcx_device_cu_count();
    const long blocks = items < resident ? items : resident;
    a.xcd_walk = dcx_env_knob(DCX_KNOB_XCD_WALK) && blocks == resident && (resident & 7) == 0 ? 1 : 0;
    if (const int rc = dcx_fill_xcd_cum(a)) return rc;
    if (after_walk != nullptr) after_walk(a);
    static bool attr_set[DCX_MAX_DEVICES] = {};
    const int dev_i = dcx_current_device();
    if (!attr_set[dev_i]) {
        DCX_CHECK_HIP(hipFuncSetAttribute(reinterpret_cast<const void*>(KERNEL), hipFuncAttributeMaxDynamicSharedMemorySize, max_dyn_lds));
        attr_set[dev_i] = true;
    }
    if (lds_bytes > 160 * 1024) return DCX_E_SHAPE;
    hipLaunchKernelGGL(KERNEL, dim3((unsigned)blocks), dim3(threads), lds_bytes, stream, a);
    return (int)hipGetLastError();
}
```

### deepcharuco_amd/csrc/dcx_first_dev.h

```cpp
#pragma once
#include "dcx_common.h"

__device__ __forceinline__ float dcx_norm_u8(uint8_t g) { return ((float)g - 128.0f) / 255.0f; }

template <unsigned B, unsigned G, unsigned R, int S>
struct DcxBgrGray {
    static constexpr unsigned CB = B, CG = G, CR = R;
    static constexpr int SHIFT = S;
    static_assert(CB + CG + CR == (1u << SHIFT), "the weights of a gray conversion sum to one");
    static __device__ __forceinline__ uint8_t gray(unsigned bb, unsigned gg, unsigned rr) {
        return (uint8_t)((bb * CB + gg * CG + rr * CR + (1u << (SHIFT - 1))) >> SHIFT);
    }
};
using DcxGray15 = DcxBgrGray<3735u, 19235u, 9798u, 15>;
using DcxGray14 = DcxBgrGray<1868u, 9617u, 4899u, 14>;

template <int PIX>
struct DcxPix {
    static_assert(dcx_pix_valid(PIX), "DCX_PIX_*");
    static constexpr int BPP = dcx_pix_bpp(PIX);
    static __device__ __forceinline__ float load(const uint8_t* p) {
        if constexpr (PIX == DCX_PIX_GRAY8) return dcx_norm_u8(*p);
        else if constexpr (PIX == DCX_PIX_BGR8) return dcx_norm_u8(DcxGray15::gray(p[0], p[1], p[2]));
        else return dcx_norm_u8(DcxGray14::gray(p[0], p[1], p[2]));
    }
};
struct DcxPixF32 {
    static constexpr int BPP = 4;
    static __device__ __forceinline__ float load(const uint8_t* p) { return *reinterpret_cast<const float*>(p); }
};

template <typename F>
static int dcx_with_pix(int pix, F&& f) {
    switch (pix) {
        case DCX_PIX_GRAY8: return f(DcxPix<DCX_PIX_GRAY8>());
        case DCX_PIX_BGR8: return f(DcxPix<DCX_PIX_BGR8>());
        case DCX_PIX_BGR8_LEGACY14: return f(DcxPix<DCX_PIX_BGR8_LEGACY14>());
        default: return DCX_E_ARG;
    }
}

template <class PX>
__device__ __forceinline__ float dcx_px_padded(const uint8_t* img, int pitch, int h, int w, int iy, int ix) {
    const bool inb = (unsigned)iy < (unsigned)h && (unsigned)ix < (unsigned)w;
    const int cy = min(max(iy, 0), h - 1), cx = min(max(ix, 0), w - 1);
    const float v = PX::load(img + (size_t)cy * pitch + (size_t)cx * PX::BPP);
    return inb ? v : 0.0f;
}

constexpr int kConv1LdsFloats = 9 * 64 + 3 * 64;
__device__ __forceinline__ void dcx_conv1_stage(float* sw, const float* __restrict__ w9x64, const float* __restrict__ bias,
                                                const float* __restrict__ alpha, const float* __restrict__ beta) {
    const int tid = threadIdx.x;
    for (int i = tid; i < 9 * 64; i += 256) sw[i] = w9x64[i];
    if (tid < 64) {
        sw[576 + tid] = bias[tid];
        sw[640 + tid] = alpha[tid];
        sw[704 + tid] = beta[tid];
    }
}

__device__ __forceinline__ float4 dcx_conv1_quad(const float4* sw4, const float (&x)[9], int cq) {
    float4 acc = make_float4(0.f, 0.f, 0.f, 0.f);
#pragma unroll
    for (int t = 0; t < 9; ++t) {
        const float4 wv = sw4[t * 16 + cq];
        acc.x = fmaf(wv.x, x[t], acc.x);
        acc.y = fmaf(wv.y, x[t], acc.y);
        acc.z = fmaf(wv.z, x[t], acc.z);
        acc.w = fmaf(wv.w, x[t], acc.w);
    }
    const float4 bi = sw4[144 + cq], al = sw4[160 + cq], be = sw4[176 + cq];
    float4 y;
    y.x = fmaxf(fmaf(acc.x + bi.x, al.x, be.x), 0.f);
    y.y = fmaxf(fmaf(acc.y + bi.y, al.y, be.y), 0.f);
    y.z = fmaxf(fmaf(acc.z + bi.z, al.z, be.z), 0.f);
    y.w = fmaxf(fmaf(acc.w + bi.w, al.w, be.w), 0.f);
    return y;
}

__device__ __forceinline__ void dcx_zero_words(int32_t* __restrict__ zero_words, int n_zero) {
    if (zero_words != nullptr && blockIdx.x == 0 && blockIdx.y == 0 && blockIdx.z == 0)
        for (int i = threadIdx.x; i < n_zero; i += 256) zero_words[i] = 0;
}
```

### deepcharuco_amd/csrc/dcx_misc.hip

```cpp
#include "dcx_cell_dev.h"
#include "dcx_common.h"
#include "dcx_first_dev.h"

#include <stdlib.h>

template <typename PX, int CS>
__global__ __launch_bounds__(256) void dcx_conv1_kernel(const uint8_t* __restrict__ in, long image_stride, int pitch,
                                                          int h, int w, int pad,
                                                          const float* __restrict__ w9x64,
                                                          const float* __restrict__ bias,
                                                          const float* __restrict__ alpha,
                                                          const float* __restrict__ beta,
                                                          float* __restrict__ out, int ho, int wo,
                                                          const int* __restrict__ n_limit, int n_images,
                                                          int32_t* __restrict__ zero_words, int n_zero) {
    __shared__ __attribute__((aligned(16))) float sw[kConv1LdsFloats];
    dcx_zero_words(zero_words, n_zero);
    int n_end = n_images;
    if (n_limit != nullptr) n_end = min(n_end, *n_limit);
    if ((int)blockIdx.y >= n_end) return;
    dcx_conv1_stage(sw, w9x64, bias, alpha, beta);
    __syncthreads();
    const int p = blockIdx.x * 256 + threadIdx.x;
    if (p >= ho * wo) return;
    const int oy = p / wo, ox = p - oy * wo;
    float4* out4 = reinterpret_cast<float4*>(out);
    const float4* sw4 = reinterpret_cast<const float4*>(sw);
    const int cq_lo = CS == 1 ? 0 : (int)blockIdx.z * (16 / CS);
    for (int n = blockIdx.y; n < n_end; n += gridDim.y) {
        const uint8_t* img = in + (size_t)n * image_stride;
        float x[9];
#pragma unroll
        for (int dy = 0; dy < 3; ++dy)
#pragma unroll
            for (int dx = 0; dx < 3; ++dx) x[dy * 3 + dx] = dcx_px_padded<PX>(img, pitch, h, w, oy - pad + dy, ox - pad + dx);
#pragma unroll 4
        for (int cq = cq_lo; cq < cq_lo + 16 / CS; ++cq)
            out4[((size_t)n * 16 + cq) * (size_t)(ho * wo) + p] = dcx_conv1_quad(sw4, x, cq);
    }
}

template <typename PX>
__global__ __launch_bounds__(256) void dcx_conv1_tile_kernel(const uint8_t* __restrict__ in, long image_stride, int pitch,
                                                               int h, int w, int pad,
                                                               const float* __restrict__ w9x64,
                                                               const float* __restrict__ bias,
                                                               const float* __restrict__ alpha,
                                                               const float* __restrict__ beta,
                                                               float* __restrict__ out, int ho, int wo, int tiles_y,
                                                               int32_t* __restrict__ zero_words, int n_zero) {
    __shared__ __attribute__((aligned(16))) float sw[kConv1LdsFloats];
    __shared__ float sp[18 * 18];
    dcx_zero_words(zero_words, n_zero);
    const int tid = threadIdx.x;
    const int n = (int)blockIdx.y / tiles_y, ty = (int)blockIdx.y - n * tiles_y, tx = (int)blockIdx.x;
    dcx_conv1_stage(sw, w9x64, bias, alpha, beta);
    const uint8_t* img = in + (size_t)n * image_stride;
    for (int e = tid; e < 18 * 18; e += 256) {
        const int i = e / 18, j = e - i * 18;
        sp[e] = dcx_px_padded<PX>(img, pitch, h, w, ty * 16 - pad + i, tx * 16 - pad + j);
    }
    __syncthreads();
    const int ly = tid >> 4, lx = tid & 15;
    const int oy = ty * 16 + ly, ox = tx * 16 + lx;
    if (oy >= ho || ox >= wo) return;
    float x[9];
#pragma unroll
    for (int dy = 0; dy < 3; ++dy)
#pragma unroll
        for (int dx = 0; dx < 3; ++dx) x[dy * 3 + dx] = sp[(ly + dy) * 18 + lx + dx];
    float4* out4 = reinterpret_cast<float4*>(out);
    const float4* sw4 = reinterpret_cast<const float4*>(sw);
    const int p = oy * wo + ox;
    const int cq_lo = (int)blockIdx.z * 4;
#pragma unroll
    for (int cq = cq_lo; cq < cq_lo + 4; ++cq) out4[((size_t)n * 16 + cq) * (size_t)(ho * wo) + p] = dcx_conv1_quad(sw4, x, cq);
}

template <typename PX>
__global__ __launch_bounds__(256) void dcx_conv1_patches_kernel(const uint8_t* __restrict__ frames, long frame_stride, int pitch,
                                                                  int h, int w, const int32_t* __restrict__ table,
                                                                  const int* __restrict__ total, int max_patches,
                                                                  const float* __restrict__ w9x64, const float* __restrict__ bias,
                                                                  const float* __restrict__ alpha, const float* __restrict__ beta,
                                                                  float* __restrict__ out) {
    __shared__ __attribute__((aligned(16))) float sw[kConv1LdsFloats];
    __shared__ float sp[24 * 24];
    int4 t = reinterpret_cast<const int4*>(table)[blockIdx.y];
    const int n_end = min(max_patches, *total);
    if ((int)blockIdx.y >= n_end) return;
    const int tid = threadIdx.x;
    const int cq0 = blockIdx.x * 4;
    dcx_conv1_stage(sw, w9x64, bias, alpha, beta);
    const float4* sw4 = reinterpret_cast<const float4*>(sw);
    float4* out4 = reinterpret_cast<float4*>(out);
    for (int n = blockIdx.y; n < n_end; n += gridDim.y) {
        if (n != (int)blockIdx.y) t = reinterpret_cast<const int4*>(table)[n];
        const uint8_t* img = frames + (size_t)t.x * frame_stride;
        __syncthreads();
        for (int e = tid; e < 576; e += 256) {
            const int i = e / 24, j = e - i * 24;
            sp[e] = dcx_px_padded<PX>(img, pitch, h, w, t.z - 12 + i, t.y - 12 + j);
        }
        __syncthreads();
        for (int p = tid; p < 22 * 22; p += 256) {
            const int oy = p / 22, ox = p - oy * 22;
            float x[9];
#pragma unroll
            for (int dy = 0; dy < 3; ++dy)
#pragma unroll
                for (int dx = 0; dx < 3; ++dx) x[dy * 3 + dx] = sp[(oy + dy) * 24 + ox + dx];
#pragma unroll
            for (int cq = cq0; cq < cq0 + 4; ++cq) out4[((size_t)n * 16 + cq) * (size_t)(22 * 22) + p] = dcx_conv1_quad(sw4, x, cq);
        }
    }
}

int dcx_launch_conv1_patches_u8(const uint8_t* frames, long frame_stride, int pitch, int pix, int h, int w, const int32_t* table,
                                const int* total, int max_patches, int n_hint, const float* w9x64, const float* bias,
                                const float* alpha, const float* beta, float* out_c4, hipStream_t s) {
    if (!frames || !table || !total || !w9x64 || !bias || !alpha || !beta || !out_c4) return DCX_E_ARG;
    if (max_patches <= 0 || h <= 0 || w <= 0) return DCX_E_SHAPE;
    int gy = n_hint > 0 && n_hint < max_patches ? n_hint : max_patches;
    if (gy > 65535) gy = 65535;
    const dim3 grid(4, (unsigned)gy);
    return dcx_with_pix(pix, [&](auto px) {
        hipLaunchKernelGGL((dcx_conv1_patches_kernel<decltype(px)>), grid, dim3(256), 0, s, frames, frame_stride, pitch, h, w, table,
                           total, max_patches, w9x64, bias, alpha, beta, out_c4);
        return (int)hipGetLastError();
    });
}

template <typename PX>
static int launch_conv1(const uint8_t* in, long image_stride, int pitch, int n, int h, int w, int pad,
                        const float* w9x64, const float* bias, const float* alpha, const float* beta,
                        float* out, const int* n_limit, int32_t* zero_words, int n_zero, hipStream_t s) {
    if (!in || !w9x64 || !bias || !alpha || !beta || !out) return DCX_E_ARG;
    const int ho = h + 2 * pad - 2, wo = w + 2 * pad - 2;
    if (ho <= 0 || wo <= 0 || n <= 0) return DCX_E_SHAPE;
    const unsigned gx = (unsigned)((ho * wo + 255) / 256), gy = (unsigned)(n < 65535 ? n : 65535);
    static int tile = -1;
    if (tile < 0) { const char* e = getenv("DCX_CONV1_TILE"); tile = (e && !atoi(e)) ? 0 : 1; }
    if (n_limit == nullptr && (long)gx * gy < 1024 && tile) {
        const int tiles_x = (wo + 15) / 16, tiles_y = (ho + 15) / 16;
        hipLaunchKernelGGL((dcx_conv1_tile_kernel<PX>), dim3((unsigned)tiles_x, (unsigned)(tiles_y * n), 4), dim3(256), 0, s, in, image_stride,
                           pitch, h, w, pad, w9x64, bias, alpha, beta, out, ho, wo, tiles_y, zero_words, n_zero);
    } else if (n_limit == nullptr && (long)gx * gy < 1024)
        hipLaunchKernelGGL((dcx_conv1_kernel<PX, 4>), dim3(gx, gy, 4), dim3(256), 0, s, in, image_stride, pitch, h, w, pad,
                           w9x64, bias, alpha, beta, out, ho, wo, n_limit, n, zero_words, n_zero);
    else
        hipLaunchKernelGGL((dcx_conv1_kernel<PX, 1>), dim3(gx, gy), dim3(256), 0, s, in, image_stride, pitch, h, w, pad,
                           w9x64, bias, alpha, beta, out, ho, wo, n_limit, n, zero_words, n_zero);
    return (int)hipGetLastError();
}

int dcx_launch_conv1_u8(const uint8_t* frames, long frame_stride, int pitch, int pix, int n, int h, int w, int pad,
                        const float* w9x64, const float* bias, const float* alpha, const float* beta,
                        float* out_c4, const int* n_limit, int32_t* zero_words, int n_zero, hipStream_t s) {
    return dcx_with_pix(pix, [&](auto px) {
        return launch_conv1<decltype(px)>(frames, frame_stride, pitch, n, h, w, pad, w9x64, bias, alpha, beta, out_c4, n_limit, zero_words,
                                          n_zero, s);
    });
}
int dcx_launch_conv1_f32(const float* images, long image_stride, int pitch, int n, int h, int w, int pad,
                         const float* w9x64, const float* bias, const float* alpha, const float* beta,
                         float* out_c4, const int* n_limit, hipStream_t s) {
    return launch_conv1<DcxPixF32>(reinterpret_cast<const uint8_t*>(images), image_stride * 4, pitch * 4, n, h, w, pad, w9x64, bias, alpha,
                                   beta, out_c4, n_limit, nullptr, 0, s);
}

__device__ __forceinline__ float dcx_logit(const DcxLogitView& v, int b, int c, int cell) {
    return v.p[(size_t)b * v.sb + (size_t)(c >> 2) * v.sq + (size_t)cell * v.sp + (size_t)(c & 3) * v.sc];
}

__device__ __forceinline__ bool dcx_argmax_takes(float v, float best) { return v > best || (v != v && best == best); }
__device__ __forceinline__ bool dcx_argmax_takes(float v, int i, float best, int besti) {
    const bool vn = v != v, bn = best != best;
    if (vn || bn) return vn && (!bn || i < besti);
    return v > best || (v == best && i < besti);
}

template <bool C4>
__device__ __forceinline__ void dcx_cell_argmax(const DcxLogitView& loc, const DcxLogitView& ids, int n_loc, int n_ids1,
                                                int cells, int dust_bin, int b, int cell, int& la, int& ia) {
    la = 0; ia = 0;
    if (C4) {
        const float4* lq = reinterpret_cast<const float4*>(loc.p) + (size_t)b * (loc.sb >> 2) + cell;
        const float4* iq = reinterpret_cast<const float4*>(ids.p) + (size_t)b * (ids.sb >> 2) + cell;
        float best = -INFINITY;
        for (int q = 0; 4 * q < n_loc; ++q) {
            const float4 v = lq[(size_t)q * cells];
            const float e[4] = {v.x, v.y, v.z, v.w};
#pragma unroll
            for (int k = 0; k < 4; ++k)
                if (4 * q + k < n_loc && (dcx_argmax_takes(e[k], best) || (q == 0 && k == 0))) { best = e[k]; la = 4 * q + k; }
        }
        best = -INFINITY;
        for (int q = 0; 4 * q < n_ids1; ++q) {
            const float4 v = iq[(size_t)q * cells];
            const float e[4] = {v.x, v.y, v.z, v.w};
#pragma unroll
            for (int k = 0; k < 4; ++k)
                if (4 * q + k < n_ids1 && (dcx_argmax_takes(e[k], best) || (q == 0 && k == 0))) { best = e[k]; ia = 4 * q + k; }
        }
    } else {
        float best = dcx_logit(loc, b, 0, cell);
        for (int c = 1; c < n_loc; ++c) {
            const float v = dcx_logit(loc, b, c, cell);
            if (dcx_argmax_takes(v, best)) { best = v; la = c; }
        }
        best = dcx_logit(ids, b, 0, cell);
        for (int c = 1; c < n_ids1; ++c) {
            const float v = dcx_logit(ids, b, c, cell);
            if (dcx_argmax_takes(v, best)) { best = v; ia = c; }
        }
    }
    ia = dcx_cell_masked_id(la, n_loc - 1, ia, dust_bin);
}

template <class CellCode>
__device__ __forceinline__ void dcx_frame_walk(CellCode cell_code, int hc, int wc, int dust_bin, int kmax,
                                               int32_t* __restrict__ counts, int32_t* __restrict__ rows) {
    __shared__ int wave_cnt[4];
    __shared__ int base_s;
    const int b = blockIdx.x;
    const int tid = threadIdx.x, lane = tid & 63, wave = tid >> 6;
    const int cells = hc * wc;
    if (tid == 0) base_s = 0;
    __syncthreads();
    for (int c0 = 0; c0 < cells; c0 += 256) {
        const int cell = c0 + tid;
        int code = 0;
        bool fire = false;
        if (cell < cells) {
            code = cell_code(b, cells, cell);
            fire = dcx_cell_fires(code, dust_bin);
        }
        const unsigned long long m = __ballot(fire);
        const int before = __popcll(m & ((1ull << lane) - 1ull));
        if (lane == 0) wave_cnt[wave] = __popcll(m);
        __syncthreads();
        int off = base_s;
        for (int w = 0; w < wave; ++w) off += wave_cnt[w];
        const int total = wave_cnt[0] + wave_cnt[1] + wave_cnt[2] + wave_cnt[3];
        if (fire) {
            const int pos = off + before;
            if (pos < kmax) reinterpret_cast<int4*>(rows)[(size_t)b * kmax + pos] = dcx_cell_row(code, cell, wc);
        }
        __syncthreads();
        if (tid == 0) base_s += total;
        __syncthreads();
    }
    if (tid == 0) counts[b] = base_s;
}

__global__ __launch_bounds__(256) void dcx_decode_kernel(DcxLogitView loc, DcxLogitView ids, int n_loc, int n_ids1,
                                                           int hc, int wc, int dust_bin, int kmax,
                                                           int32_t* __restrict__ counts, int32_t* __restrict__ rows,
                                                           int32_t* __restrict__ loc_argmax,
                                                           int32_t* __restrict__ ids_argmax) {
    dcx_frame_walk([&](int b, int cells, int cell) {
        int la, ia;
        dcx_cell_argmax<false>(loc, ids, n_loc, n_ids1, cells, dust_bin, b, cell, la, ia);
        if (loc_argmax) loc_argmax[(size_t)b * cells + cell] = la;
        if (ids_argmax) ids_argmax[(size_t)b * cells + cell] = ia;
        return dcx_cell_pack(la, ia);
    }, hc, wc, dust_bin, kmax, counts, rows);
}

template <bool C4>
__global__ __launch_bounds__(256) void dcx_cell_argmax_kernel(DcxLogitView loc, DcxLogitView ids, int n_loc, int n_ids1,
                                                                int cells, int dust_bin, int32_t* __restrict__ codes,
                                                                int32_t* __restrict__ loc_argmax,
                                                                int32_t* __restrict__ ids_argmax) {
    const int b = blockIdx.y;
    const int cell = blockIdx.x * 256 + threadIdx.x;
    if (cell >= cells) return;
    int la, ia;
    dcx_cell_argmax<C4>(loc, ids, n_loc, n_ids1, cells, dust_bin, b, cell, la, ia);
    codes[(size_t)b * cells + cell] = dcx_cell_pack(la, ia);
    if (loc_argmax) loc_argmax[(size_t)b * cells + cell] = la;
    if (ids_argmax) ids_argmax[(size_t)b * cells + cell] = ia;
}

__global__ __launch_bounds__(256) void dcx_compact_kernel(const int32_t* __restrict__ codes, int hc, int wc, int dust_bin,
                                                            int kmax, int32_t* __restrict__ counts,
                                                            int32_t* __restrict__ rows) {
    dcx_frame_walk([&](int b, int cells, int cell) { return codes[(size_t)b * cells + cell]; }, hc, wc, dust_bin, kmax, counts, rows);
}

int dcx_launch_decode(DcxLogitView loc, DcxLogitView ids, int batch, int n_loc, int n_ids1, int hc, int wc,
                      int dust_bin, int kmax, int32_t* counts, int32_t* rows,
                      int32_t* loc_argmax, int32_t* ids_argmax, int32_t* codes_scratch, hipStream_t s) {
    if (!loc.p || !ids.p || !counts || !rows) return DCX_E_ARG;
    if (batch <= 0 || hc <= 0 || wc <= 0 || kmax <= 0 || n_loc != 65 || n_ids1 < 2 || n_ids1 > 256) return DCX_E_SHAPE;
    if (const int rc = dcx_check_dust_bin(dust_bin)) return rc;
    const bool c4 = loc.sc == 1 && loc.sp == 4 && ids.sc == 1 && ids.sp == 4 && loc.sq == 4L * hc * wc && ids.sq == 4L * hc * wc
                    && (loc.sb & 3) == 0 && (ids.sb & 3) == 0;
    if (codes_scratch != nullptr) {
        const int cells = hc * wc;
        const dim3 grid((unsigned)((cells + 255) / 256), (unsigned)batch);
        if (c4)
            hipLaunchKernelGGL(dcx_cell_argmax_kernel<true>, grid, dim3(256), 0, s, loc, ids, n_loc, n_ids1, cells, dust_bin,
                               codes_scratch, loc_argmax, ids_argmax);
        else
            hipLaunchKernelGGL(dcx_cell_argmax_kernel<false>, grid, dim3(256), 0, s, loc, ids, n_loc, n_ids1, cells, dust_bin,
                               codes_scratch, loc_argmax, ids_argmax);
        hipLaunchKernelGGL(dcx_compact_kernel, dim3((unsigned)batch), dim3(256), 0, s, codes_scratch, hc, wc, dust_bin, kmax,
                           counts, rows);
        return (int)hipGetLastError();
    }
    hipLaunchKernelGGL(dcx_decode_kernel, dim3((unsigned)batch), dim3(256), 0, s, loc, ids, n_loc, n_ids1, hc, wc,
                       dust_bin, kmax, counts, rows, loc_argmax, ids_argmax);
    return (int)hipGetLastError();
}

int dcx_launch_compact(const int32_t* codes, int batch, int hc, int wc, int dust_bin, int kmax, int32_t* counts,
                       int32_t* rows, hipStream_t s) {
    if (!codes || !counts || !rows) return DCX_E_ARG;
    if (batch <= 0 || hc <= 0 || wc <= 0 || kmax <= 0) return DCX_E_SHAPE;
    if (const int rc = dcx_check_dust_bin(dust_bin, 256)) return rc;
    hipLaunchKernelGGL(dcx_compact_kernel, dim3((unsigned)batch), dim3(256), 0, s, codes, hc, wc, dust_bin, kmax, counts, rows);
    return (int)hipGetLastError();
}

extern "C" int dcx_pred_to_keypoints(const float* d_loc, const float* d_ids, int batch, int n_loc, int n_ids1,
                                     int hc, int wc, int dust_bin, int kmax, int32_t* d_counts, int32_t* d_rows,
                                     int32_t* d_loc_argmax, int32_t* d_ids_argmax, void* stream) {
    const long cells = (long)hc * wc;
    DcxLogitView lv{d_loc, (long)n_loc * cells, 4 * cells, 1, cells};
    DcxLogitView iv{d_ids, (long)n_ids1 * cells, 4 * cells, 1, cells};
    return dcx_launch_decode(lv, iv, batch, n_loc, n_ids1, hc, wc, dust_bin, kmax, d_counts, d_rows,
                             d_loc_argmax, d_ids_argmax, nullptr, (hipStream_t)stream);
}

__global__ __launch_bounds__(256) void dcx_pack_labels_kernel(const long long* __restrict__ loc, const long long* __restrict__ ids,
                                                              long n, int32_t* __restrict__ codes, int* __restrict__ bad) {
    const long i = (long)blockIdx.x * 256 + threadIdx.x;
    if (i >= n) return;
    const long long l = loc[i], d = ids[i];
    if (l < 0 || l > 255 || d < 0 || d > 255) { if (bad) *bad = 1; codes[i] = 0; return; }
    codes[i] = dcx_cell_pack((int)l, (int)d);
}

extern "C" int dcx_label_to_keypoints(const long long* d_loc, const long long* d_ids, int batch, int hc, int wc, int dust_bin,
                                      int kmax, int32_t* d_counts, int32_t* d_rows, int32_t* d_codes, int32_t* d_bad, void* stream) {
    if (!d_loc || !d_ids || !d_counts || !d_rows || !d_codes) return DCX_E_ARG;
    if (batch <= 0 || hc <= 0 || wc <= 0 || kmax <= 0) return DCX_E_SHAPE;
    if (dust_bin < 0 || dust_bin > 255) dust_bin = 256;
    const long n = (long)batch * hc * wc;
    hipLaunchKernelGGL(dcx_pack_labels_kernel, dim3((unsigned)((n + 255) / 256)), dim3(256), 0, (hipStream_t)stream, d_loc, d_ids, n,
                       d_codes, d_bad);
    return dcx_launch_compact(d_codes, batch, hc, wc, dust_bin, kmax, d_counts, d_rows, (hipStream_t)stream);
}

__device__ __forceinline__ void dcx_patch_table_body(const int32_t* __restrict__ counts, const int32_t* __restrict__ rows,
                                                     int batch, int kmax, int32_t* __restrict__ table, int32_t* __restrict__ total,
                                                     int* s_cnt, int* s_start, int* wave_tot, int* carry) {
    const int tid = threadIdx.x, lane = tid & 63, wave = tid >> 6;
    if (tid == 0) *carry = 0;
    __syncthreads();
    for (int b0 = 0; b0 < batch; b0 += 256) {
        const int b = b0 + tid;
        const int c = b < batch ? min(counts[b], kmax) : 0;
        int incl = c;
#pragma unroll
        for (int d = 1; d < 64; d <<= 1) {
            const int v = __shfl_up(incl, d);
            if (lane >= d) incl += v;
        }
        if (lane == 63) wave_tot[wave] = incl;
        __syncthreads();
        int off = *carry;
        for (int w = 0; w < wave; ++w) off += wave_tot[w];
        s_cnt[tid] = c;
        s_start[tid] = off + incl - c;
        __syncthreads();
        const int nb = min(256, batch - b0);
        for (int idx = tid; idx < nb * kmax; idx += 256) {
            const int bl = idx / kmax, k = idx - bl * kmax;
            if (k < s_cnt[bl]) {
                const int bb = b0 + bl;
                const int4 r = reinterpret_cast<const int4*>(rows)[(size_t)bb * kmax + k];
                reinterpret_cast<int4*>(table)[s_start[bl] + k] = make_int4(bb, r.x, r.y, bb * kmax + k);
            }
        }
        __syncthreads();
        if (tid == 0) *carry += wave_tot[0] + wave_tot[1] + wave_tot[2] + wave_tot[3];
        __syncthreads();
    }
    if (tid == 0) *total = *carry;
}

__global__ __launch_bounds__(256) void dcx_patch_table_kernel(const int32_t* __restrict__ counts,
                                                                const int32_t* __restrict__ rows, int batch, int kmax,
                                                                int32_t* __restrict__ table, int32_t* __restrict__ total) {
    __shared__ int s_cnt[256], s_start[256];
    __shared__ int wave_tot[4];
    __shared__ int carry;
    dcx_patch_table_body(counts, rows, batch, kmax, table, total, s_cnt, s_start, wave_tot, &carry);
}

extern "C" int dcx_build_patch_table(const int32_t* d_counts, const int32_t* d_rows, int batch, int kmax,
                                     int32_t* d_table, int32_t* d_total, void* stream) {
    if (!d_counts || !d_rows || !d_table || !d_total) return DCX_E_ARG;
    if (batch <= 0 || kmax <= 0) return DCX_E_SHAPE;
    hipLaunchKernelGGL(dcx_patch_table_kernel, dim3(1), dim3(256), 0, (hipStream_t)stream, d_counts, d_rows, batch,
                       kmax, d_table, d_total);
    return (int)hipGetLastError();
}

template <typename PX>
__global__ __launch_bounds__(192) void dcx_gather_kernel(const uint8_t* __restrict__ frames, long frame_stride, int pitch,
                                                           int h, int w, const int32_t* __restrict__ table,
                                                           const int32_t* __restrict__ total,
                                                           float* __restrict__ patches) {
    const int p = blockIdx.x;
    if (total != nullptr && p >= *total) return;
    const int4 t = reinterpret_cast<const int4*>(table)[p];
    const uint8_t* img = frames + (size_t)t.x * frame_stride;
    for (int e = threadIdx.x; e < 576; e += 192) {
        const int i = e / 24, j = e - i * 24;
        patches[(size_t)p * 576 + e] = dcx_px_padded<PX>(img, pitch, h, w, t.z - 12 + i, t.y - 12 + j);
    }
}

template <typename PX>
static int launch_gather(const uint8_t* frames, long frame_stride, int pitch, int height, int width, const int32_t* d_table,
                         const int32_t* d_total, int max_patches, float* d_patches, void* stream) {
    if (!frames || !d_table || !d_patches) return DCX_E_ARG;
    if (max_patches <= 0 || height <= 0 || width <= 0) return DCX_E_SHAPE;
    hipLaunchKernelGGL((dcx_gather_kernel<PX>), dim3((unsigned)max_patches), dim3(192), 0, (hipStream_t)stream, frames, frame_stride,
                       pitch, height, width, d_table, d_total, d_patches);
    return (int)hipGetLastError();
}

extern "C" int dcx_extract_patches_u8(const uint8_t* d_frames, long frame_stride, int pitch, int height, int width,
                                      const int32_t* d_table, const int32_t* d_total, int max_patches,
                                      float* d_patches, void* stream) {
    return launch_gather<DcxPix<DCX_PIX_GRAY8>>(d_frames, frame_stride, pitch, height, width, d_table, d_total, max_patches, d_patches,
                                                stream);
}

extern "C" int dcx_extract_patches_f32(const float* d_images, int height, int width, const int32_t* d_table,
                                       const int32_t* d_total, int max_patches, float* d_patches, void* stream) {
    return launch_gather<DcxPixF32>(reinterpret_cast<const uint8_t*>(d_images), (long)height * width * 4, width * 4, height, width,
                                    d_table, d_total, max_patches, d_patches, stream);
}

__global__ __launch_bounds__(64) void dcx_refine_finalize_kernel(const float* __restrict__ part_val,
                                                                   const int* __restrict__ part_idx, int tiles, int wo,
                                                                   int max_patches, const int* __restrict__ total,
                                                                   const int32_t* __restrict__ table,
                                                                   int32_t* __restrict__ corners,
                                                                   float* __restrict__ xy) {
    const int p = blockIdx.x * 64 + threadIdx.x;
    if (p >= max_patches) return;
    if (total != nullptr && p >= *total) return;
    float best = part_val[(size_t)p * tiles];
    int besti = part_idx[(size_t)p * tiles];
    for (int t = 1; t < tiles; ++t) {
        const float v = part_val[(size_t)p * tiles + t];
        const int i = part_idx[(size_t)p * tiles + t];
        if (v > best || (v == best && i < besti)) { best = v; besti = i; }
    }
    const int row = besti / wo, col = besti - row * wo;
    if (corners) { corners[2 * p] = col; corners[2 * p + 1] = row; }
    if (xy != nullptr && table != nullptr) {
        const int4 t = reinterpret_cast<const int4*>(table)[p];
        xy[2 * (size_t)t.w] = (float)(col - 32) / 8.0f + (float)t.y;
        xy[2 * (size_t)t.w + 1] = (float)(row - 32) / 8.0f + (float)t.z;
    }
}

int dcx_launch_refine_finalize(const float* part_val, const int* part_idx, int tiles, int wo, int max_patches,
                               const int* total, const int32_t* table, int32_t* corners, float* xy, hipStream_t s) {
    hipLaunchKernelGGL(dcx_refine_finalize_kernel, dim3((unsigned)((max_patches + 63) / 64)), dim3(64), 0, s, part_val,
                       part_idx, tiles, wo, max_patches, total, table, corners, xy);
    return (int)hipGetLastError();
}

__global__ __launch_bounds__(256) void dcx_argmax2d_kernel(const float* __restrict__ x, int hw, int w,
                                                             int32_t* __restrict__ out) {
    __shared__ float sv[4];
    __shared__ int si[4];
    const int k = blockIdx.x;
    const int tid = threadIdx.x, lane = tid & 63, wave = tid >> 6;
    const float* p = x + (size_t)k * hw;
    float best = -INFINITY;
    int besti = 0x7fffffff;
    for (int i = tid; i < hw; i += 256) {
        const float v = p[i];
        if (dcx_argmax_takes(v, i, best, besti)) { best = v; besti = i; }
    }
    for (int off = 32; off >= 1; off >>= 1) {
        const float ov = __shfl_xor(best, off);
        const int oi = __shfl_xor(besti, off);
        if (dcx_argmax_takes(ov, oi, best, besti)) { best = ov; besti = oi; }
    }
    if (lane == 0) { sv[wave] = best; si[wave] = besti; }
    __syncthreads();
    if (tid == 0) {
        for (int wv = 1; wv < 4; ++wv)
            if (dcx_argmax_takes(sv[wv], si[wv], best, besti)) { best = sv[wv]; besti = si[wv]; }
        if (besti == 0x7fffffff) besti = 0;
        out[2 * k] = besti % w;
        out[2 * k + 1] = besti / w;
    }
}

extern "C" int dcx_argmax2d(const float* d_x, int k, int h, int w, int32_t* d_out, void* stream) {
    if (!d_x || !d_out) return DCX_E_ARG;
    if (k <= 0 || h <= 0 || w <= 0) return DCX_E_SHAPE;
    hipLaunchKernelGGL(dcx_argmax2d_kernel, dim3((unsigned)k), dim3(256), 0, (hipStream_t)stream, d_x, h * w, w, d_out);
    return (int)hipGetLastError();
}

__global__ __launch_bounds__(256) void dcx_pre_image_kernel(const uint8_t* __restrict__ g, float* __restrict__ out,
                                                              size_t n) {
    for (size_t i = (size_t)blockIdx.x * 256 + threadIdx.x; i < n; i += (size_t)gridDim.x * 256)
        out[i] = dcx_norm_u8(g[i]);
}

extern "C" int dcx_pre_image(const uint8_t* d_gray, float* d_out, size_t n, void* stream) {
    if (!d_gray || !d_out) return DCX_E_ARG;
    if (n == 0) return 0;
    const unsigned blocks = (unsigned)((n + 255) / 256 > 4096 ? 4096 : (n + 255) / 256);
    hipLaunchKernelGGL(dcx_pre_image_kernel, dim3(blocks), dim3(256), 0, (hipStream_t)stream, d_gray, d_out, n);
    return (int)hipGetLastError();
}

template <unsigned CB, unsigned CG, unsigned CR, int SHIFT>
__global__ __launch_bounds__(256) void dcx_bgr2gray_kernel(const uint8_t* __restrict__ bgr, long frame_stride, int pitch,
                                                             int h, int w, uint8_t* __restrict__ gray) {
    const int b = blockIdx.z, y = blockIdx.y;
    const int x0 = (blockIdx.x * 256 + threadIdx.x) * 4;
    if (x0 >= w) return;
    const uint8_t* src = bgr + (size_t)b * frame_stride + (size_t)y * pitch + (size_t)x0 * 3;
    uint8_t* dst = gray + ((size_t)b * h + y) * w + x0;
    const int n = min(4, w - x0);
    uint8_t g[4] = {0, 0, 0, 0};
    for (int i = 0; i < n; ++i) {
        g[i] = DcxBgrGray<CB, CG, CR, SHIFT>::gray(src[3 * i], src[3 * i + 1], src[3 * i + 2]);
    }
    if (n == 4 && ((w & 3) == 0)) *reinterpret_cast<uchar4*>(dst) = make_uchar4(g[0], g[1], g[2], g[3]);
    else for (int i = 0; i < n; ++i) dst[i] = g[i];
}

template <class G>
static int bgr2gray_launch(const uint8_t* d_bgr, long frame_stride, int pitch, int batch, int height, int width,
                           uint8_t* d_gray, void* stream) {
    if (!d_bgr || !d_gray) return DCX_E_ARG;
    if (batch <= 0 || height <= 0 || width <= 0 || batch > 65535 || height > 65535 || pitch < 3 * width) return DCX_E_SHAPE;
    const dim3 grid((unsigned)((width + 1023) / 1024), (unsigned)height, (unsigned)batch);
    hipLaunchKernelGGL((dcx_bgr2gray_kernel<G::CB, G::CG, G::CR, G::SHIFT>), grid, dim3(256), 0, (hipStream_t)stream, d_bgr, frame_stride,
                       pitch, height, width, d_gray);
    return (int)hipGetLastError();
}

extern "C" int dcx_bgr2gray(const uint8_t* d_bgr, long frame_stride, int pitch, int batch, int height, int width,
                            uint8_t* d_gray, void* stream) {
    return bgr2gray_launch<DcxGray15>(d_bgr, frame_stride, pitch, batch, height, width, d_gray, stream);
}

extern "C" int dcx_bgr2gray_legacy14(const uint8_t* d_bgr, long frame_stride, int pitch, int batch, int height, int width,
                                     uint8_t* d_gray, void* stream) {
    return bgr2gray_launch<DcxGray14>(d_bgr, frame_stride, pitch, batch, height, width, d_gray, stream);
}

__global__ __launch_bounds__(256) void dcx_nchw_to_c4_kernel(const float* __restrict__ src, int c, int hw,
                                                               float* __restrict__ dst) {
    const int cq_n = (c + 3) >> 2;
    const int n = blockIdx.z, cq = blockIdx.y;
    const int p = blockIdx.x * 256 + threadIdx.x;
    if (p >= hw) return;
    float4 v = make_float4(0.f, 0.f, 0.f, 0.f);
    const float* s = src + ((size_t)n * c + 4 * cq) * hw + p;
    if (4 * cq + 0 < c) v.x = s[0];
    if (4 * cq + 1 < c) v.y = s[(size_t)hw];
    if (4 * cq + 2 < c) v.z = s[2 * (size_t)hw];
    if (4 * cq + 3 < c) v.w = s[3 * (size_t)hw];
    reinterpret_cast<float4*>(dst)[((size_t)n * cq_n + cq) * hw + p] = v;
}

__global__ __launch_bounds__(256) void dcx_c4_to_nchw_kernel(const float* __restrict__ src, int c, int hw,
                                                               float* __restrict__ dst) {
    const int cq_n = (c + 3) >> 2;
    const int n = blockIdx.z, cq = blockIdx.y;
    const int p = blockIdx.x * 256 + threadIdx.x;
    if (p >= hw) return;
    const float4 v = reinterpret_cast<const float4*>(src)[((size_t)n * cq_n + cq) * hw + p];
    float* d = dst + ((size_t)n * c + 4 * cq) * hw + p;
    if (4 * cq + 0 < c) d[0] = v.x;
    if (4 * cq + 1 < c) d[(size_t)hw] = v.y;
    if (4 * cq + 2 < c) d[2 * (size_t)hw] = v.z;
    if (4 * cq + 3 < c) d[3 * (size_t)hw] = v.w;
}

template <typename K>
static int launch_c4_convert(K kernel, const float* src, int n, int c, int h, int w, float* dst, void* stream) {
    if (!src || !dst) return DCX_E_ARG;
    if (n <= 0 || c <= 0 || h <= 0 || w <= 0 || n > 65535) return DCX_E_SHAPE;
    dim3 grid((unsigned)((h * w + 255) / 256), (unsigned)((c + 3) / 4), (unsigned)n);
    hipLaunchKernelGGL(kernel, grid, dim3(256), 0, (hipStream_t)stream, src, c, h * w, dst);
    return (int)hipGetLastError();
}

extern "C" int dcx_nchw_to_c4(const float* d_nchw, int n, int c, int h, int w, float* d_c4, void* stream) {
    return launch_c4_convert(dcx_nchw_to_c4_kernel, d_nchw, n, c, h, w, d_c4, stream);
}

extern "C" int dcx_c4_to_nchw(const float* d_c4, int n, int c, int h, int w, float* d_nchw, void* stream) {
    return launch_c4_convert(dcx_c4_to_nchw_kernel, d_c4, n, c, h, w, d_nchw, stream);
}
```

### deepcharuco_amd/inference.py

```python
from __future__ import annotations

import ctypes as _ctypes
import warnings
from typing import List, Optional

import numpy as np
import torch

from . import _lib
from .corner_pool import frame_keypoints, packed_len, ptrs, views
from .imgproc import _opencv, bgr2gray
from .models._handles import require_cuda, unwrap
from .models.model_utils import extract_patches, pre_bgr_image, pred_to_keypoints
from .models.net import dcModel, lModel
from .models.refinenet import RefineNet, lRefineNet
from .pnp import (solve_pnp_batch_device, solve_pnp_device, solve_pnp_host, solve_pnp_pool, solve_pnp_ransac_batch_device,
                  solve_pnp_ransac_device, solve_pnp_ransac_host, solve_pnp_ransac_pool, unpack_poses, unpack_ransac)

__all__ = ["load_models", "infer_image", "infer_image_staged", "infer_batch", "infer_batch_device", "unpack_results", "packed_len",
           "solve_pnp", "solve_pnp_batch", "solve_pnp_submit", "set_deterministic", "InferenceModel", "calibrate_xcd",
           "set_xcd_weights", "get_xcd_weights", "solve_pnp_host", "solve_pnp_device", "solve_pnp_batch_device", "solve_pnp_pool",
           "unpack_poses", "solve_pnp_ransac_host", "solve_pnp_ransac_device", "solve_pnp_ransac_batch_device",
           "solve_pnp_ransac_pool", "unpack_ransac"]

DEFAULT_KMAX = 64


def load_models(deepc_ckpt: str, refinenet_ckpt: Optional[str] = None, n_ids: int = 16, device="cuda"):
    deepc = lModel.load_from_checkpoint(deepc_ckpt, dcModel=dcModel(n_ids))
    deepc.eval()
    deepc.to(device)
    refinenet = None
    if refinenet_ckpt is not None:
        refinenet = lRefineNet.load_from_checkpoint(refinenet_ckpt, refinenet=RefineNet())
        refinenet.eval()
        refinenet.to(device)
    return deepc, refinenet


def _cv2_solvepnp():
    try:
        import cv2
    except ImportError as e:
        raise ImportError("solve_pnp needs OpenCV (cv2.solvePnP), which is not installed") from e
    return cv2.solvePnP


def _pnp_points(keypoints, col_count, row_count, square_len):
    inn_rc = np.arange(1, row_count)
    inn_cc = np.arange(1, col_count)
    object_points = np.zeros(((col_count - 1) * (row_count - 1), 3), np.float32)
    object_points[:, :2] = np.array(np.meshgrid(inn_rc, inn_cc)).reshape((2, -1)).T * square_len
    image_points = keypoints[:, :2].astype(np.float32)
    return object_points[keypoints[:, 2].astype(int)], image_points


def solve_pnp(keypoints, col_count, row_count, square_len, camera_matrix, dist_coeffs):
    if keypoints.shape[0] < 4:
        return False, None, None
    object_points_found, image_points = _pnp_points(keypoints, col_count, row_count, square_len)
    return _cv2_solvepnp()(object_points_found, image_points, camera_matrix, dist_coeffs)


_pnp_pools: dict = {}


def _pool(workers: Optional[int]):
    import concurrent.futures as cf
    import os
    n = int(workers) if workers else min(32, os.cpu_count() or 1)
    pool = _pnp_pools.get(n)
    if pool is None:
        pool = _pnp_pools[n] = cf.ThreadPoolExecutor(max_workers=n, thread_name_prefix="dcx-pnp")
    return pool


def solve_pnp_submit(keypoints_list, col_count, row_count, square_len, camera_matrix, dist_coeffs, workers: Optional[int] = None):
    import concurrent.futures as cf
    fn = _cv2_solvepnp()
    pool = _pool(workers)
    futs = []
    for kp in keypoints_list:
        kp = np.asarray(kp)
        if kp.ndim != 2 or kp.shape[0] < 4:
            f = cf.Future()
            f.set_result((False, None, None))
        else:
            obj, img = _pnp_points(kp, col_count, row_count, square_len)
            f = pool.submit(fn, obj, img, camera_matrix, dist_coeffs)
        futs.append(f)
    return futs


def solve_pnp_batch(keypoints_list, col_count, row_count, square_len, camera_matrix, dist_coeffs, workers: Optional[int] = None):
    return [f.result() for f in solve_pnp_submit(keypoints_list, col_count, row_count, square_len, camera_matrix,
                                                dist_coeffs, workers)]



def set_deterministic(enabled: bool = True) -> None:
    _lib.check(_lib.lib().dcx_set_deterministic(1 if enabled else 0), "dcx_set_deterministic")
    from .graph import clear_graph_cache
    clear_graph_cache()


def calibrate_xcd(device="cuda", rounds: int = 8) -> List[float]:
    dev = require_cuda(device)
    w = (_ctypes.c_float * 8)()
    with torch.cuda.device(dev):
        torch.cuda.synchronize()
        _lib.check(_lib.lib().dcx_calibrate_xcd(int(rounds), w, _lib.current_stream()), "dcx_calibrate_xcd")
    from .graph import clear_graph_cache
    clear_graph_cache()
    return [float(v) for v in w]


def set_xcd_weights(weights=None, device="cuda") -> None:
    dev = require_cuda(device)
    arr = None if weights is None else (_ctypes.c_float * 8)(*[float(v) for v in weights])
    with torch.cuda.device(dev):
        _lib.check(_lib.lib().dcx_set_xcd_weights(arr), "dcx_set_xcd_weights")
    from .graph import clear_graph_cache
    clear_graph_cache()


def get_xcd_weights(device="cuda") -> List[float]:
    dev = require_cuda(device)
    w = (_ctypes.c_float * 8)()
    with torch.cuda.device(dev):
        _lib.check(_lib.lib().dcx_get_xcd_weights(w), "dcx_get_xcd_weights")
    return [float(v) for v in w]


PIXEL_FORMATS = {"gray": 0, "opencv4": 1, "legacy14": 2}


def launch_pipeline(det, ref, frames_ptr: int, b: int, h: int, w: int, bpp: int, pix: int, dust_bin_ids: int, pool: int,
                    ws: torch.Tensor, out_ptr: int, conf: bool = False, front: Optional[torch.Tensor] = None,
                    detector_done: Optional[int] = None) -> None:
    counts_p, starts_p, rows_p, xy_p, conf_p = ptrs(out_ptr, b, pool)
    head = (det.handle, ref.handle if ref else None, frames_ptr, h * w * bpp, w * bpp, pix, b, h, w, dust_bin_ids, pool,
            ws.data_ptr(), ws.numel())
    tail = (counts_p, starts_p, rows_p, xy_p if ref else None, conf_p if conf else None, _lib.current_stream())
    if front is None:
        _lib.check(_lib.lib().dcx_infer_batch(*head, *tail), "dcx_infer_batch")
    else:
        _lib.check(_lib.lib().dcx_infer_batch_prefetched(*head, front.data_ptr(), front.numel(), *tail[:-1], detector_done, tail[-1]),
                   "dcx_infer_batch_prefetched")


def launch_front(det, frames_ptr: int, b: int, h: int, w: int, bpp: int, pix: int, front: torch.Tensor) -> None:
    _lib.check(_lib.lib().dcx_detector_front(det.handle, frames_ptr, h * w * bpp, w * bpp, pix, b, h, w, front.data_ptr(),
                                             front.numel(), _lib.current_stream()), "dcx_detector_front")


def pipeline_workspace(det, ref, b: int, h: int, w: int, pool: int, ws: Optional[torch.Tensor] = None) -> torch.Tensor:
    dev = det.device
    nbytes = _lib.lib().dcx_pipeline_workspace_bytes(det.handle, ref.handle if ref else None, b, h, w, pool)
    if nbytes == 0:
        raise ValueError("bad batch/shape for dcx_pipeline_workspace_bytes")
    if ws is None:
        return det._ws.get("pipe", dev, nbytes)
    if ws.device != dev or ws.dtype != torch.uint8 or not ws.is_contiguous() or ws.numel() < nbytes:
        raise ValueError(f"ws must be a contiguous uint8 tensor of >= {nbytes} bytes on {dev}")
    return ws


def infer_batch_device(frames: torch.Tensor, dust_bin_ids: int, deepc, refinenet=None, kmax: int = DEFAULT_KMAX,
                       out: Optional[torch.Tensor] = None, ws: Optional[torch.Tensor] = None, pool: Optional[int] = None,
                       conf: bool = False, bgr_variant: str = "opencv4") -> torch.Tensor:
    det, ref = unwrap(deepc), unwrap(refinenet)
    dev = det.device
    if (not isinstance(frames, torch.Tensor) or frames.device != dev or frames.dtype != torch.uint8 or not frames.is_contiguous()
            or not (frames.ndim == 3 or (frames.ndim == 4 and frames.shape[3] == 3))):
        raise ValueError("frames must be a contiguous (B,H,W) gray or (B,H,W,3) BGR uint8 tensor on the model's GPU")
    b, h, w = frames.shape[:3]
    bpp = 1 if frames.ndim == 3 else 3
    if bgr_variant not in ("opencv4", "legacy14"):
        raise ValueError(f"unknown BGR->gray variant {bgr_variant!r}")
    pix = PIXEL_FORMATS["gray" if bpp == 1 else bgr_variant]
    if pool is None:
        pool = b * kmax
    if pool <= 0:
        raise ValueError("pool must be positive")
    with torch.cuda.device(dev):
        ws = pipeline_workspace(det, ref, b, h, w, pool, ws)
        n_i32 = packed_len(b, pool, conf)
        if out is None:
            out = torch.empty((n_i32,), dtype=torch.int32, device=dev)
        elif out.device != dev or out.dtype != torch.int32 or out.numel() != n_i32 or not out.is_contiguous():
            raise ValueError(f"out must be a contiguous int32 tensor of {n_i32} elements on {dev}")
        launch_pipeline(det, ref, frames.data_ptr(), b, h, w, bpp, pix, dust_bin_ids, pool, ws, out.data_ptr(), conf)
    return out


def unpack_results(packed: np.ndarray, batch: int, pool: int, refined: bool, conf: bool = False):
    packed = np.asarray(packed, dtype=np.int32)
    counts, starts, rows, xy, cf = views(packed, batch, pool)
    res: List[Optional[np.ndarray]] = []
    confs: List[Optional[np.ndarray]] = []
    for k, s0 in zip(counts.tolist(), starts.tolist()):
        if k == 0:
            res.append(np.array([]))
            confs.append(np.zeros((0, 2), np.float32))
            continue
        if s0 + k > pool:
            res.append(None)
            confs.append(None)
            continue
        a, order = frame_keypoints(rows, xy, s0, k, refined)
        res.append(a)
        if conf:
            confs.append(cf[s0:s0 + k][order].copy())
    if conf:
        return res, counts.copy(), confs
    return res, counts.copy()


def _to_device_frames(frames, dev):
    if isinstance(frames, torch.Tensor):
        d = frames
    else:
        frames = np.ascontiguousarray(frames, dtype=np.uint8)
        d = torch.from_numpy(frames)
    if d.dtype != torch.uint8 or not (d.ndim == 3 or (d.ndim == 4 and d.shape[3] == 3)):
        raise ValueError("expected (B,H,W) uint8 gray frames or (B,H,W,3) uint8 BGR frames")
    return d.to(dev).contiguous()


def infer_batch(frames, dust_bin_ids: int, deepc, refinenet=None, kmax: int = DEFAULT_KMAX, pool: Optional[int] = None,
                conf: bool = False, bgr_variant: str = "opencv4"):
    det = unwrap(deepc)
    d_frames = _to_device_frames(frames, det.device)
    b = d_frames.shape[0]
    if pool is None:
        pool = b * kmax
    while True:
        packed = infer_batch_device(d_frames, dust_bin_ids, deepc, refinenet, pool=pool, conf=conf, bgr_variant=bgr_variant).cpu().numpy()
        out = unpack_results(packed, b, pool, refinenet is not None, conf)
        need = int(out[1].astype(np.int64).sum())
        if need <= pool:
            return (out[0], out[2]) if conf else out[0]
        warnings.warn(f"the batch produced {need} corners > pool={pool}; re-running with pool={need}")
        pool = need


_graph_state = {"enabled": None, "warned": False}
_graph_mod = [None]
_cuda_seen = [False]


def _graphs_enabled() -> bool:
    if _graph_state["enabled"] is None:
        import os
        _graph_state["enabled"] = os.environ.get("DCX_GRAPH", "1") not in ("", "0")
    return bool(_graph_state["enabled"])


def infer_image(img: np.ndarray, dust_bin_ids: int, deepc, refinenet=None, draw_pred: bool = False, device="cuda"):
    if device != "cuda":
        require_cuda(device)
    elif not _cuda_seen[0]:
        require_cuda(device)
        _cuda_seen[0] = True
    if not isinstance(img, np.ndarray) or img.ndim != 3 or img.shape[2] != 3 or img.dtype != np.uint8:
        raise ValueError("expected a (H,W,3) uint8 BGR image")
    if draw_pred:
        return infer_image_staged(img, dust_bin_ids, deepc, refinenet, True, device)
    keypoints = None
    frame = bgr2gray(img)[None] if _opencv() else img[None]
    G = _graph_mod[0]
    if G is None:
        from . import graph as G
        _graph_mod[0] = G
    graphs_usable, cached_pipeline = G.graphs_usable, G.cached_pipeline
    if _graphs_enabled() and graphs_usable():
        try:
            for attempt in (0, 1):
                pipe = cached_pipeline(dust_bin_ids, deepc, refinenet, img.shape[0], img.shape[1], bgr=frame.ndim == 4)
                try:
                    keypoints = pipe.run(frame)[0]
                    break
                except ReferenceError:
                    continue
        except (_lib.DcxError, ValueError):
            raise
        except RuntimeError as e:
            if not _graph_state["warned"]:
                warnings.warn(f"hipGraph capture failed ({e}); falling back to eager kernel launches")
                _graph_state["warned"] = True
            _graph_state["enabled"] = False
    if keypoints is None:
        keypoints = infer_batch(frame, dust_bin_ids, deepc, refinenet)[0]
    return keypoints, img


def infer_image_staged(img: np.ndarray, dust_bin_ids: int, deepc, refinenet=None, draw_pred: bool = False,
                       device="cuda"):
    require_cuda(device)
    img_gray = bgr2gray(img)
    img_gray = pre_bgr_image(img_gray)
    img_gray = torch.tensor(img_gray, device=device)
    loc_hat, ids_hat = deepc.infer_image(img_gray)
    keypoints, ids_found = pred_to_keypoints(loc_hat, ids_hat, dust_bin_ids)
    if draw_pred:
        img = (draw_inner_corners(img, keypoints.cpu().numpy(), ids_found.cpu().numpy(), radius=3, draw_ids=True, color=(0, 0, 255))
               if ids_found.shape[0] else img.copy())
    if ids_found.shape[0] == 0:
        return np.array([]), img
    if refinenet is not None:
        patches = extract_patches(img_gray, keypoints)
        keypoints, _ = refinenet.infer_patches(patches, keypoints)
    keypoints = keypoints.cpu().numpy()
    ids_found = ids_found.cpu().numpy()
    if draw_pred and refinenet is not None:
        img = draw_inner_corners(img, keypoints, ids_found, draw_ids=False, radius=1, color=(0, 255, 255))
    keypoints = np.array([[k[0], k[1], idx] for k, idx in sorted(zip(keypoints, ids_found), key=lambda x: x[1])])
    return keypoints, img


def draw_inner_corners(img: np.ndarray, corners: np.ndarray, ids: np.ndarray, draw_ids: bool = False, radius: int = 2,
                       color=(0, 0, 255)) -> np.ndarray:
    try:
        import cv2
    except ImportError as e:
        raise ImportError("draw_pred=True needs OpenCV for drawing, which is not installed") from e
    assert img.ndim == 3 and img.shape[-1] == 3
    out = img.copy()
    font, thickness = cv2.FONT_HERSHEY_COMPLEX_SMALL, 1
    for corner, idx in zip(corners, ids):
        c = np.round(corner).astype(int)
        if c[0] > out.shape[1] or c[1] > out.shape[0]:
            continue
        cv2.circle(out, (int(c[0]), int(c[1])), radius=radius, color=color, thickness=thickness)
        if draw_ids:
            (tw, th), _ = cv2.getTextSize(str(idx), font, .5, thickness)
            cv2.putText(out, str(idx), (int(c[0]) - tw // 2 - 7, int(c[1]) + th // 2 - 3), font, .45, (0, 255, 0), thickness)
    return out


class InferenceModel:

    def __init__(self, deepc_ckpt: str, refinenet_ckpt: Optional[str] = None, n_ids: int = 16, device="cuda"):
        self.n_ids = n_ids
        self.device = device
        self.deepc, self.refinenet = load_models(deepc_ckpt, refinenet_ckpt, n_ids, device)

    def infer_image(self, img: np.ndarray, draw_pred: bool = False):
        return infer_image(img, self.n_ids, self.deepc, self.refinenet, draw_pred, self.device)

    def infer_batch(self, frames: np.ndarray, kmax: int = DEFAULT_KMAX, conf: bool = False):
        return infer_batch(frames, self.n_ids, self.deepc, self.refinenet, kmax, conf=conf)
```

### deepcharuco_amd/stream.py

```python
from __future__ import annotations

import os
import time
import warnings
from typing import Iterable, Iterator, List, Optional, Tuple

import numpy as np
import torch

from . import _lib
from .corner_pool import views
from .inference import (DEFAULT_KMAX, PIXEL_FORMATS, infer_batch, infer_batch_device, launch_front, launch_pipeline, packed_len, pipeline_workspace, solve_pnp_submit,
                        unpack_results)
from .models._handles import unwrap
from .pnp import (POSE_WORDS, ransac_workspace_bytes, solve_pnp_batch_device, solve_pnp_pool, solve_pnp_ransac_batch_device,
                  solve_pnp_ransac_pool, unpack_poses, unpack_ransac)


class FrameStream:
    def __init__(self, dust_bin_ids: int, deepc, refinenet=None, batch: int = 32, height: int = 240,
                 width: int = 320, kmax: int = DEFAULT_KMAX, depth: int = 2, pnp: Optional[dict] = None,
                 compute_streams: int = 1, bgr: bool = False, h2d_on_compute: Optional[bool] = None, pnp_device: bool = False,
                 pnp_ransac: Optional[dict] = None):
        det = unwrap(deepc)
        self.dev = det.device
        self.dust_bin_ids, self.deepc, self.refinenet = dust_bin_ids, deepc, refinenet
        self.batch, self.h, self.w, self.kmax, self.depth = batch, height, width, kmax, depth
        self.pool = batch * kmax
        self.bgr = bool(bgr)
        self.h2d_on_compute = compute_streams > 1 if h2d_on_compute is None else bool(h2d_on_compute)
        self.pnp = pnp
        self.pnp_device = bool(pnp_device) and pnp is not None
        if pnp_ransac is not None and not self.pnp_device:
            raise ValueError("pnp_ransac needs pnp=... and pnp_device=True")
        self.pnp_ransac = None if pnp_ransac is None else dict(pnp_ransac)
        if not (1 <= compute_streams <= depth):
            raise ValueError("compute_streams must be between 1 and depth")
        n_out = packed_len(batch, self.pool)
        shape = (batch, height, width, 3) if self.bgr else (batch, height, width)
        with torch.cuda.device(self.dev):
            self.copy_stream = torch.cuda.Stream()
            self.compute = [torch.cuda.Stream() for _ in range(compute_streams)] if compute_streams > 1 else None
            self.pin_in = [torch.empty(shape, dtype=torch.uint8).pin_memory() for _ in range(depth)]
            self.dev_in = [torch.empty(shape, dtype=torch.uint8, device=self.dev) for _ in range(depth)]
            self.dev_out = [torch.empty((n_out,), dtype=torch.int32, device=self.dev) for _ in range(depth)]
            self.pin_out = [torch.empty((n_out,), dtype=torch.int32).pin_memory() for _ in range(depth)]
            self.ev_h2d = [torch.cuda.Event() for _ in range(depth)]
            self.ev_free = [torch.cuda.Event() for _ in range(depth)]
            self.ev_done = [torch.cuda.Event() for _ in range(depth)]
            if self.pnp_device:
                self.dev_pnp = [(torch.empty((batch,), dtype=torch.int32, device=self.dev),
                                 torch.empty((batch, POSE_WORDS), dtype=torch.float64, device=self.dev)) for _ in range(depth)]
                self.pin_pnp = [(torch.empty((batch,), dtype=torch.int32).pin_memory(),
                                 torch.empty((batch, POSE_WORDS), dtype=torch.float64).pin_memory()) for _ in range(depth)]
            if self.pnp_ransac is not None:
                ws = ransac_workspace_bytes(batch, self.pool, self.pnp_ransac.get("iterations", 100))
                self.dev_pnp = [o + (torch.empty((batch, 2), dtype=torch.int32, device=self.dev),
                                     torch.zeros((self.pool,), dtype=torch.uint8, device=self.dev)) for o in self.dev_pnp]
                self.pin_pnp = [o + (torch.empty((batch, 2), dtype=torch.int32).pin_memory(),
                                     torch.zeros((self.pool,), dtype=torch.uint8).pin_memory()) for o in self.pin_pnp]
                self.ws_pnp = [torch.empty(((ws + 7) // 8,), dtype=torch.float64, device=self.dev) for _ in range(depth)]
        self._pending: List[Optional[Tuple[int, int, np.ndarray]]] = [None] * depth
        self._ticket = 0

    def _collect(self, slot: int):
        ticket, n, frames = self._pending[slot]
        self._pending[slot] = None
        self.ev_done[slot].synchronize()
        res, counts = unpack_results(self.pin_out[slot].numpy(), self.batch, self.pool, self.refinenet is not None)
        res = res[:n]
        need = int(counts.astype(np.int64).sum())
        if need > self.pool:
            warnings.warn(f"a batch produced {need} corners > pool={self.pool} (batch x kmax); re-running it with pool={need}")
            res = infer_batch(frames, self.dust_bin_ids, self.deepc, self.refinenet, pool=need)
            if self.pnp_ransac is not None:
                return ticket, res, solve_pnp_ransac_batch_device(res, device=self.dev, **self.pnp, **self.pnp_ransac)
            if self.pnp_device:
                return ticket, res, solve_pnp_batch_device(res, device=self.dev, **self.pnp)
        if self.pnp_ransac is not None:
            st, pose, _, mask = self.pin_pnp[slot]
            counts, starts, rows, _, _ = views(self.pin_out[slot].numpy(), self.batch, self.pool)
            return ticket, res, unpack_ransac(st.numpy()[:n], pose.numpy()[:n], mask.numpy(), counts, starts, rows[:, 2])
        if self.pnp_device:
            st, pose = self.pin_pnp[slot]
            return ticket, res, unpack_poses(st.numpy()[:n], pose.numpy()[:n])
        if self.pnp is not None:
            return ticket, res, solve_pnp_submit(res, **self.pnp)
        return ticket, res

    def submit(self, frames_gray: np.ndarray):
        n = frames_gray.shape[0]
        want = (self.h, self.w, 3) if self.bgr else (self.h, self.w)
        if n > self.batch or tuple(frames_gray.shape[1:]) != want or frames_gray.dtype != np.uint8:
            raise ValueError(f"frames must be (n<=batch, {', '.join(map(str, want))}) uint8")
        slot = self._ticket % self.depth
        retired = self._collect(slot) if self._pending[slot] is not None else None
        self.pin_in[slot][:n].numpy()[...] = frames_gray
        if n < self.batch:
            self.pin_in[slot][n:].zero_()
        with torch.cuda.device(self.dev):
            compute = torch.cuda.current_stream() if self.compute is None else self.compute[self._ticket % len(self.compute)]
            if not self.h2d_on_compute:
                with torch.cuda.stream(self.copy_stream):
                    self.copy_stream.wait_event(self.ev_free[slot])
                    self.dev_in[slot].copy_(self.pin_in[slot], non_blocking=True)
                    self.ev_h2d[slot].record(self.copy_stream)
            with torch.cuda.stream(compute):
                if self.h2d_on_compute:
                    compute.wait_event(self.ev_free[slot])
                    self.dev_in[slot].copy_(self.pin_in[slot], non_blocking=True)
                else:
                    compute.wait_event(self.ev_h2d[slot])
                infer_batch_device(self.dev_in[slot], self.dust_bin_ids, self.deepc, self.refinenet, out=self.dev_out[slot],
                                   pool=self.pool)
                self.ev_free[slot].record(compute)
                if self.pnp_ransac is not None:
                    solve_pnp_ransac_pool(self.dev_out[slot], self.batch, self.pool, self.refinenet is not None,
                                          out=self.dev_pnp[slot], workspace=self.ws_pnp[slot], **self.pnp, **self.pnp_ransac)
                elif self.pnp_device:
                    solve_pnp_pool(self.dev_out[slot], self.batch, self.pool, self.refinenet is not None, out=self.dev_pnp[slot],
                                   **self.pnp)
                self.pin_out[slot].copy_(self.dev_out[slot], non_blocking=True)
                if self.pnp_device:
                    for h, d in zip(self.pin_pnp[slot], self.dev_pnp[slot]):
                        h.copy_(d, non_blocking=True)
                self.ev_done[slot].record(compute)
        self._pending[slot] = (self._ticket, n, frames_gray)
        self._ticket += 1
        return retired

    def _resolve(self, r):
        return r if len(r) == 2 or self.pnp_device else (r[0], r[1], [f.result() for f in r[2]])

    def flush(self) -> Iterator[Tuple]:
        order = sorted((p[0], s) for s, p in enumerate(self._pending) if p is not None)
        for _, slot in order:
            yield self._resolve(self._collect(slot))

    def run(self, batches: Iterable[np.ndarray]) -> Iterator[Tuple]:
        if self.pnp is None:
            for fr in batches:
                r = self.submit(fr)
                if r is not None:
                    yield r
            yield from self.flush()
            return
        held = None
        for fr in batches:
            r = self.submit(fr)
            if held is not None:
                yield self._resolve(held)
                held = None
            if r is not None:
                held = r
        if held is not None:
            yield self._resolve(held)
        yield from self.flush()


class ResidentStream:

    PREFETCH_MAX_BYTES = 1 << 30

    def __init__(self, dust_bin_ids: int, deepc, refinenet=None, batch: int = 32, height: int = 240, width: int = 320,
                 kmax: int = DEFAULT_KMAX, compute_streams: int = 1, depth: Optional[int] = None, bgr: bool = False,
                 raw: bool = False, timing: bool = False, prefetch: Optional[bool] = None):
        det = unwrap(deepc)
        self.dev = det.device
        self.dust_bin_ids, self.deepc, self.refinenet = dust_bin_ids, deepc, refinenet
        self.batch, self.h, self.w, self.kmax = batch, height, width, kmax
        self.pool = batch * kmax
        self.bgr, self.raw, self.timing = bool(bgr), bool(raw), bool(timing)
        if compute_streams < 1:
            raise ValueError("compute_streams must be >= 1")
        self.depth = depth = compute_streams + 2 if depth is None else depth
        if depth < compute_streams:
            raise ValueError("depth must be >= compute_streams")
        n_out = packed_len(batch, self.pool)
        with torch.cuda.device(self.dev):
            self.compute = [torch.cuda.Stream() for _ in range(compute_streams)]
            self.pin_out = [torch.empty((n_out,), dtype=torch.int32).pin_memory() for _ in range(depth)]
            self.ev_in = [torch.cuda.Event() for _ in range(depth)]
            self.ev_start = [torch.cuda.Event(enable_timing=True) for _ in range(depth)] if self.timing else None
            self.ev_done = [torch.cuda.Event(enable_timing=self.timing) for _ in range(depth)]
            self._front = None
            if prefetch and compute_streams != 1:
                raise ValueError("prefetch needs compute_streams == 1 (several streams already overlap everything)")
            nb = _lib.lib().dcx_front_bytes(det.handle, batch, height, width)
            if prefetch is None and os.environ.get("DCX_RS_PREFETCH"):
                prefetch = os.environ["DCX_RS_PREFETCH"] != "0"
            if os.environ.get("DCX_RS_PRIO", "0") != "0":
                self.compute = [torch.cuda.Stream(priority=-1)]
            if prefetch is None:
                prefetch = compute_streams == 1 and nb <= self.PREFETCH_MAX_BYTES
            if prefetch and compute_streams == 1:
                try:
                    self._front = [torch.empty((nb,), dtype=torch.uint8, device=self.dev) for _ in range(2)]
                except torch.cuda.OutOfMemoryError:
                    warnings.warn(f"ResidentStream: no memory for two prefetch sets of {nb} bytes; running without the conv1a prefetch")
                else:
                    self.side = torch.cuda.Stream()
                    self.ev_front = [torch.cuda.Event() for _ in range(depth)]
                    self.ev_det = [torch.cuda.Event() for _ in range(depth)]
                    for e in self.ev_det:
                        e.record(self.side)
                    self._last_det: Optional[torch.cuda.Event] = None
        self._pending: List[Optional[Tuple[int, torch.Tensor, torch.cuda.Stream]]] = [None] * depth
        self._ticket = 0
        self.gpu_ms: List[float] = []
        self.host_enqueue_s = 0.0
        self.host_wait_s = 0.0

    def reset_stats(self) -> None:
        self.gpu_ms = []
        self.host_enqueue_s = self.host_wait_s = 0.0

    def _collect(self, slot: int):
        ticket, frames, compute = self._pending[slot]
        self._pending[slot] = None
        n = frames.shape[0]
        t0 = time.perf_counter()
        self.ev_done[slot].synchronize()
        self.host_wait_s += time.perf_counter() - t0
        if self.timing:
            self.gpu_ms.append(self.ev_start[slot].elapsed_time(self.ev_done[slot]))
        packed = self.pin_out[slot].numpy()[:packed_len(n, self.pool)]
        need = int(packed[:n].astype(np.int64).sum())
        if need > self.pool:
            warnings.warn(f"a batch produced {need} corners > pool={self.pool} (batch x kmax); re-running it with pool={need}")
            n_big = packed_len(n, need)
            with torch.cuda.device(self.dev):
                host = torch.empty((n_big,), dtype=torch.int32).pin_memory()
                done = torch.cuda.Event()
                with torch.cuda.stream(compute):
                    big = infer_batch_device(frames, self.dust_bin_ids, self.deepc, self.refinenet, pool=need)
                    host.copy_(big, non_blocking=True)
                    done.record(compute)
            t0 = time.perf_counter()
            done.synchronize()
            self.host_wait_s += time.perf_counter() - t0
            packed = host.numpy()
            if self.raw:
                return ticket, packed
            return ticket, unpack_results(packed, n, need, self.refinenet is not None)[0]
        if self.raw:
            return ticket, packed.copy()
        return ticket, unpack_results(packed, n, self.pool, self.refinenet is not None)[0]

    def submit(self, frames: torch.Tensor):
        want = (self.h, self.w, 3) if self.bgr else (self.h, self.w)
        if (not isinstance(frames, torch.Tensor) or frames.device != self.dev or frames.dtype != torch.uint8
                or not frames.is_contiguous() or tuple(frames.shape[1:]) != want or not (1 <= frames.shape[0] <= self.batch)):
            raise ValueError(f"frames must be a contiguous (1 <= n <= batch, {', '.join(map(str, want))}) uint8 tensor on {self.dev}")
        n = frames.shape[0]
        slot = self._ticket % self.depth
        retired = self._collect(slot) if self._pending[slot] is not None else None
        t0 = time.perf_counter()
        with torch.cuda.device(self.dev):
            compute = self.compute[self._ticket % len(self.compute)]
            self.ev_in[slot].record(torch.cuda.current_stream())
            det, ref = unwrap(self.deepc), unwrap(self.refinenet)
            bpp, pix = (3, PIXEL_FORMATS["opencv4"]) if self.bgr else (1, PIXEL_FORMATS["gray"])
            front = None
            if self._front is not None:
                front = self._front[self._ticket % 2]
                with torch.cuda.stream(self.side):
                    self.side.wait_event(self.ev_in[slot])
                    if self._last_det is not None:
                        self.side.wait_event(self._last_det)
                    launch_front(det, frames.data_ptr(), n, self.h, self.w, bpp, pix, front)
                    self.ev_front[slot].record(self.side)
                self._last_det = self.ev_det[slot]
            with torch.cuda.stream(compute):
                compute.wait_event(self.ev_in[slot])
                if self.timing:
                    self.ev_start[slot].record(compute)
                if front is not None:
                    compute.wait_event(self.ev_front[slot])
                launch_pipeline(det, ref, frames.data_ptr(), n, self.h, self.w, bpp, pix, self.dust_bin_ids, self.pool,
                                pipeline_workspace(det, ref, n, self.h, self.w, self.pool), self.pin_out[slot].data_ptr(), front=front,
                                detector_done=self.ev_det[slot].cuda_event if front is not None else None)
                self.ev_done[slot].record(compute)
        self._pending[slot] = (self._ticket, frames, compute)
        self._ticket += 1
        self.host_enqueue_s += time.perf_counter() - t0
        return retired

    def flush(self) -> Iterator[Tuple]:
        order = sorted((p[0], s) for s, p in enumerate(self._pending) if p is not None)
        for _, slot in order:
            yield self._collect(slot)

    def run(self, batches: Iterable[torch.Tensor]) -> Iterator[Tuple]:
        for fr in batches:
            r = self.submit(fr)
            if r is not None:
                yield r
        yield from self.flush()
```

### include/deepcharuco_amd.h

```cpp
#ifndef DEEPCHARUCO_AMD_H
#define DEEPCHARUCO_AMD_H

#include <stddef.h>
#include <stdint.h>

#ifdef __cplusplus
extern "C" {
#endif

#define DCX_E_ARG      (-1)
#define DCX_E_SHAPE    (-2)
#define DCX_E_WS       (-3)
#define DCX_E_NIDS     (-4)

typedef struct dcx_detector dcx_detector;
typedef struct dcx_refiner  dcx_refiner;

const char* dcx_version(void);
const char* dcx_error_string(int code);

int dcx_detector_create(dcx_detector** out, const float* const* h_tensors, int n_tensors, int n_ids);
int dcx_detector_destroy(dcx_detector* det);
int dcx_refiner_create(dcx_refiner** out, const float* const* h_tensors, int n_tensors);
int dcx_refiner_destroy(dcx_refiner* rf);

size_t dcx_detector_workspace_bytes(const dcx_detector* det, int batch, int height, int width);
size_t dcx_refiner_workspace_bytes(const dcx_refiner* rf, int max_patches);

int dcx_bgr2gray(const uint8_t* d_bgr, long frame_stride, int pitch, int batch, int height, int width,
                 uint8_t* d_gray, void* stream);
int dcx_bgr2gray_legacy14(const uint8_t* d_bgr, long frame_stride, int pitch, int batch, int height, int width,
                          uint8_t* d_gray, void* stream);

int dcx_pre_image(const uint8_t* d_gray, float* d_out, size_t n, void* stream);

int dcx_detector_forward(const dcx_detector* det,
                         const uint8_t* d_frames_u8, long frame_stride, int pitch,
                         const float* d_images_f32,
                         int batch, int height, int width,
                         void* d_ws, size_t ws_bytes,
                         float* d_loc_nchw, float* d_ids_nchw, void* stream);

int dcx_detector_decode(const dcx_detector* det, int batch, int height, int width,
                        void* d_ws, int dust_bin, int kmax,
                        int32_t* d_counts, int32_t* d_rows,
                        int32_t* d_loc_argmax, int32_t* d_ids_argmax, void* stream);
int dcx_pred_to_keypoints(const float* d_loc_nchw, const float* d_ids_nchw,
                          int batch, int n_loc, int n_ids1, int hc, int wc,
                          int dust_bin, int kmax,
                          int32_t* d_counts, int32_t* d_rows,
                          int32_t* d_loc_argmax, int32_t* d_ids_argmax, void* stream);
int dcx_label_to_keypoints(const long long* d_loc, const long long* d_ids, int batch, int hc, int wc, int dust_bin, int kmax,
                           int32_t* d_counts, int32_t* d_rows, int32_t* d_codes, int32_t* d_bad, void* stream);

int dcx_build_patch_table(const int32_t* d_counts, const int32_t* d_rows, int batch, int kmax,
                          int32_t* d_table, int32_t* d_total, void* stream);

int dcx_extract_patches_u8(const uint8_t* d_frames, long frame_stride, int pitch, int height, int width,
                           const int32_t* d_table, const int32_t* d_total, int max_patches,
                           float* d_patches, void* stream);
int dcx_extract_patches_f32(const float* d_images, int height, int width,
                            const int32_t* d_table, const int32_t* d_total, int max_patches,
                            float* d_patches, void* stream);

int dcx_refiner_forward(const dcx_refiner* rf, const float* d_patches, int max_patches,
                        const int32_t* d_total, const int32_t* d_table,
                        void* d_ws, size_t ws_bytes,
                        int32_t* d_corners, float* d_xy, float* d_heat, void* stream);

int dcx_argmax2d(const float* d_x, int k, int h, int w, int32_t* d_out, void* stream);

#define DCX_PIX_GRAY8          0
#define DCX_PIX_BGR8           1
#define DCX_PIX_BGR8_LEGACY14  2
size_t dcx_pipeline_workspace_bytes(const dcx_detector* det, const dcx_refiner* rf,
                                    int batch, int height, int width, int pool);
int dcx_infer_batch(const dcx_detector* det, const dcx_refiner* rf,
                    const uint8_t* d_frames_u8, long frame_stride, int pitch, int pixel_format,
                    int batch, int height, int width, int dust_bin, int pool,
                    void* d_ws, size_t ws_bytes,
                    int32_t* d_counts, int32_t* d_starts, int32_t* d_rows, float* d_xy, float* d_conf, void* stream);
size_t dcx_front_bytes(const dcx_detector* det, int batch, int height, int width);
int dcx_detector_front(const dcx_detector* det, const uint8_t* d_frames_u8, long frame_stride, int pitch, int pixel_format,
                       int batch, int height, int width, void* d_front, size_t front_bytes, void* stream);
int dcx_infer_batch_prefetched(const dcx_detector* det, const dcx_refiner* rf,
                               const uint8_t* d_frames_u8, long frame_stride, int pitch, int pixel_format,
                               int batch, int height, int width, int dust_bin, int pool,
                               void* d_ws, size_t ws_bytes, void* d_front, size_t front_bytes,
                               int32_t* d_counts, int32_t* d_starts, int32_t* d_rows, float* d_xy, float* d_conf,
                               void* detector_done_event, void* stream);
int dcx_stream_synchronize(void* stream);

#define DCX_PNP_OK          0
#define DCX_PNP_TOO_FEW     1
#define DCX_PNP_TRUNCATED   2
#define DCX_PNP_BAD_ID      3
#define DCX_PNP_DEGENERATE  4
#define DCX_PNP_NONFINITE   5
int dcx_solve_pnp_pool(const int32_t* d_counts, const int32_t* d_starts, const int32_t* d_rows,
                       const float* d_xy , int batch, int pool,
                       int col_count, int row_count, double square_len,
                       const double* h_camera9, const double* h_dist, int n_dist,
                       int32_t* d_status, double* d_pose ,
                       void* stream);

#define DCX_PNP_NO_CONSENSUS 6
size_t dcx_solve_pnp_ransac_workspace_bytes(int batch, int pool, int iterations);
int dcx_solve_pnp_ransac_pool(const int32_t* d_counts, const int32_t* d_starts, const int32_t* d_rows,
                              const float* d_xy , int batch, int pool,
                              int col_count, int row_count, double square_len,
                              const double* h_camera9, const double* h_dist, int n_dist,
                              int iterations, double reproj_error, int min_inliers, unsigned seed,
                              void* d_workspace, size_t workspace_bytes,
                              int32_t* d_status, double* d_pose , int32_t* d_info ,
                              uint8_t* d_inliers , void* stream);

#define DCX_CALIB_OK          0
#define DCX_CALIB_NO_VIEWS    1
#define DCX_CALIB_DEGENERATE  2
#define DCX_CALIB_NONFINITE   3
size_t dcx_calibrate_workspace_bytes(int batch);
int dcx_calibrate_pool(const int32_t* d_counts, const int32_t* d_starts, const int32_t* d_rows,
                       const float* d_xy , int batch, int pool,
                       int col_count, int row_count, double square_len, int image_width, int image_height,
                       void* d_workspace, size_t workspace_bytes,
                       int32_t* d_view_status , double* d_pose ,
                       double* h_result , void* stream);

#define DCX_CALIB_USE_INTRINSIC_GUESS  0x0001
#define DCX_CALIB_FIX_ASPECT_RATIO     0x0002
#define DCX_CALIB_FIX_PRINCIPAL_POINT  0x0004
#define DCX_CALIB_ZERO_TANGENT_DIST    0x0008
#define DCX_CALIB_FIX_FOCAL_LENGTH     0x0010
#define DCX_CALIB_FIX_K1               0x0020
#define DCX_CALIB_FIX_K2               0x0040
#define DCX_CALIB_FIX_K3               0x0080
#define DCX_CALIB_FIX_K4               0x0800
#define DCX_CALIB_FIX_K5               0x1000
#define DCX_CALIB_FIX_K6               0x2000
#define DCX_CALIB_RATIONAL_MODEL       0x4000
size_t dcx_calibrate_flags_workspace_bytes(int batch, int flags);
int dcx_calibrate_flags_pool(const int32_t* d_counts, const int32_t* d_starts, const int32_t* d_rows,
                             const float* d_xy , int batch, int pool,
                             int col_count, int row_count, double square_len, int image_width, int image_height,
                             int flags, const double* h_camera9 ,
                             const double* h_dist, int n_dist,
                             void* d_workspace, size_t workspace_bytes,
                             int32_t* d_view_status , double* d_pose ,
                             double* h_result , void* stream);

size_t dcx_calibrate_ransac_workspace_bytes(int batch, int pool, int iterations);
int dcx_calibrate_ransac_pool(const int32_t* d_counts, const int32_t* d_starts, const int32_t* d_rows,
                              const float* d_xy , int batch, int pool,
                              int col_count, int row_count, double square_len, int image_width, int image_height,
                              int iterations, double consensus_error, double reproj_error, int min_inliers, int rounds,
                              unsigned seed, void* d_workspace, size_t workspace_bytes,
                              int32_t* d_view_status , double* d_pose ,
                              int32_t* d_info , uint8_t* d_inliers ,
                              double* h_result , void* stream);

#define DCX_STEREO_OK          0
#define DCX_STEREO_NO_PAIRS    1
#define DCX_STEREO_DEGENERATE  2
#define DCX_STEREO_NONFINITE   3
size_t dcx_stereo_calibrate_workspace_bytes(int batch, int pool0, int pool1);
int dcx_stereo_calibrate_pool(const int32_t* d_counts0, const int32_t* d_starts0, const int32_t* d_rows0,
                              const float* d_xy0 , const uint8_t* d_mask0 ,
                              const int32_t* d_counts1, const int32_t* d_starts1, const int32_t* d_rows1,
                              const float* d_xy1, const uint8_t* d_mask1 ,
                              int batch, int pool0, int pool1, int col_count, int row_count, double square_len,
                              const double* h_camera9_0, const double* h_dist0, int n_dist0,
                              const double* h_camera9_1, const double* h_dist1, int n_dist1,
                              void* d_workspace, size_t workspace_bytes,
                              int32_t* d_view_status , double* d_pose ,
                              double* d_view_info , double* h_result , void* stream);

#define DCX_CAMERA_PINHOLE 0
#define DCX_CAMERA_FISHEYE 1
int dcx_stereo_calibrate_models_pool(const int32_t* d_counts0, const int32_t* d_starts0, const int32_t* d_rows0, const float* d_xy0,
                                     const uint8_t* d_mask0, const int32_t* d_counts1, const int32_t* d_starts1,
                                     const int32_t* d_rows1, const float* d_xy1, const uint8_t* d_mask1, int batch, int pool0,
                                     int pool1, int col_count, int row_count, double square_len, const double* h_camera9_0,
                                     const double* h_dist0, int n_dist0, const double* h_camera9_1, const double* h_dist1,
                                     int n_dist1, int model0, int model1, void* d_workspace, size_t workspace_bytes,
                                     int32_t* d_view_status , double* d_pose ,
                                     double* d_view_info , double* h_result , void* stream);

#define DCX_RIG_OK            0
#define DCX_RIG_NO_STAMPS     1
#define DCX_RIG_DEGENERATE    2
#define DCX_RIG_NONFINITE     3
#define DCX_RIG_DISCONNECTED  4
#define DCX_RIG_MAX_CAMERAS   8
typedef struct DcxRigCamera {
    const int32_t* d_counts;
    const int32_t* d_starts;
    const int32_t* d_rows;
    const float* d_xy;
    int pool;
    const uint8_t* d_mask;
    double camera9[9];
    double dist[8];
    int n_dist;
} DcxRigCamera;
size_t dcx_rig_calibrate_workspace_bytes(int n_cams, int batch, const int* h_pools);
int dcx_rig_calibrate_pool(int n_cams, const DcxRigCamera* h_cams, int batch, int col_count, int row_count, double square_len,
                           void* d_workspace, size_t workspace_bytes, int32_t* d_view_status ,
                           double* d_pose , double* d_view_info , int32_t* h_parents ,
                           double* h_result , void* stream);

int dcx_rig_calibrate_models_pool(int n_cams, const DcxRigCamera* h_cams, const int* h_models ,
                                  int batch, int col_count, int row_count, double square_len, void* d_workspace,
                                  size_t workspace_bytes, int32_t* d_view_status ,
                                  double* d_pose , double* d_view_info ,
                                  int32_t* h_parents , double* h_result , void* stream);

size_t dcx_rig_pose_workspace_bytes(int n_cams, int batch, const int* h_pools);
int dcx_rig_pose_pool(int n_cams, const DcxRigCamera* h_cams, const int* h_models ,
                      const double* h_rig , int batch, int col_count, int row_count,
                      double square_len, void* d_workspace, size_t workspace_bytes, int32_t* d_head ,
                      int32_t* d_status , double* d_pose ,
                      int32_t* d_info , int32_t* d_view_status ,
                      double* d_view_info , void* stream);

int dcx_undistort_rectify_map(const double* h_camera9, const double* h_dist, int n_dist,
                              const double* h_R9 , const double* h_P12 ,
                              int width, int height, int32_t* d_map , void* stream);
int dcx_rectify_points_pool(const int32_t* d_rows, const float* d_xy , int pool,
                            const double* h_camera9, const double* h_dist, int n_dist,
                            const double* h_R9 , const double* h_P12 ,
                            double* d_out , void* stream);
int dcx_remap_u8(const uint8_t* d_src, long frame_stride, int pitch, int src_h, int src_w, int channels ,
                 const int32_t* d_map, int out_h, int out_w, int batch, int border, uint8_t* d_out, void* stream);

int dcx_fisheye_solve_pnp_pool(const int32_t* d_counts, const int32_t* d_starts, const int32_t* d_rows,
                               const float* d_xy , int batch, int pool,
                               int col_count, int row_count, double square_len,
                               const double* h_camera9, const double* h_dist4 ,
                               int32_t* d_status, double* d_pose , void* stream);

int dcx_fisheye_solve_pnp_ransac_pool(const int32_t* d_counts, const int32_t* d_starts, const int32_t* d_rows, const float* d_xy,
                                      int batch, int pool, int col_count, int row_count, double square_len,
                                      const double* h_camera9, const double* h_dist4, int iterations, double reproj_error,
                                      int min_inliers, unsigned seed, void* d_workspace, size_t workspace_bytes, int32_t* d_status,
                                      double* d_pose, int32_t* d_info, uint8_t* d_inliers, void* stream);
size_t dcx_fisheye_calibrate_workspace_bytes(int batch);
int dcx_fisheye_calibrate_pool(const int32_t* d_counts, const int32_t* d_starts, const int32_t* d_rows,
                               const float* d_xy , int batch, int pool,
                               int col_count, int row_count, double square_len, int image_width, int image_height,
                               double focal0 , void* d_workspace, size_t workspace_bytes,
                               int32_t* d_view_status , double* d_pose ,
                               double* h_result , void* stream);
int dcx_fisheye_undistort_rectify_map(const double* h_camera9, const double* h_dist4,
                                      const double* h_R9 , const double* h_P12 ,
                                      int width, int height, int32_t* d_map , void* stream);
int dcx_fisheye_rectify_points_pool(const int32_t* d_rows, const float* d_xy , int pool,
                                    const double* h_camera9, const double* h_dist4,
                                    const double* h_R9 , const double* h_P12 ,
                                    double* d_out , void* stream);

#define DCX_COV_OK        0
#define DCX_COV_NO_VIEWS  1
#define DCX_COV_NO_DOF    2
#define DCX_COV_SINGULAR  3
#define DCX_COV_COV       0
#define DCX_COV_STD       81
#define DCX_COV_SIGMA2    90
#define DCX_COV_DOF       91
#define DCX_COV_POINTS    92
#define DCX_COV_VIEWS     93
#define DCX_COV_STATUS    94
#define DCX_COV_GLOBAL_WORDS 96
#define DCX_COV_POSE_WORDS   42
size_t dcx_calibrate_uncertainty_workspace_bytes(int batch);
int dcx_calibrate_uncertainty_pool(const int32_t* d_counts, const int32_t* d_starts, const int32_t* d_rows,
                                   const float* d_xy , int batch, int pool,
                                   int col_count, int row_count, double square_len, int model ,
                                   const double* h_theta , const int32_t* d_view_status ,
                                   const double* d_pose , const uint8_t* d_mask ,
                                   void* d_workspace, size_t workspace_bytes, double* d_global ,
                                   double* d_pose_cov , void* stream);

int dcx_resize_u8(const uint8_t* d_src, long frame_stride, int pitch, int src_h, int src_w, int channels ,
                  int out_h, int out_w, int batch, int interpolation , uint8_t* d_out,
                  void* stream);

int dcx_resize_area_u8(const uint8_t* d_src, long frame_stride, int pitch, int src_h, int src_w, int channels ,
                       int out_h, int out_w, int batch, uint8_t* d_out, void* stream);

size_t dcx_sgm_workspace_bytes(int batch, int height, int width, int num_disparities);
int dcx_sgm_u8(const uint8_t* d_left, long frame_stride_l, int pitch_l, const uint8_t* d_right, long frame_stride_r, int pitch_r,
               int batch, int height, int width, int min_disparity, int num_disparities, int p1, int p2, int uniqueness,
               int lr_max_diff, int16_t* d_disp16, void* d_workspace, size_t workspace_bytes, void* stream);
int dcx_sgm_u8_paths(const uint8_t* d_left, long frame_stride_l, int pitch_l, const uint8_t* d_right, long frame_stride_r, int pitch_r,
                     int batch, int height, int width, int min_disparity, int num_disparities, int p1, int p2, int uniqueness,
                     int lr_max_diff, int paths , int16_t* d_disp16, void* d_workspace, size_t workspace_bytes,
                     void* stream);
int dcx_disparity_to_points(const int16_t* d_disp16, int batch, int height, int width, int min_disparity,
                            const double* h_Q16 , float* d_xyz , void* stream);

size_t dcx_filter_speckles_workspace_bytes(int batch, int height, int width);
int dcx_filter_speckles_s16(const int16_t* d_in, int16_t* d_out, int batch, int height, int width, int new_val,
                            int max_speckle_size, int max_diff, void* d_workspace, size_t workspace_bytes, void* stream);

int dcx_conv_layer(const float* d_in, int n, int cin, int hin, int win,
                   const float* h_weight_oihw, const float* h_bias,
                   const float* h_bn_gamma, const float* h_bn_beta,
                   const float* h_bn_mean, const float* h_bn_var,
                   int cout, int ksize, int pad, int ups, int pool, int relu,
                   float* d_out, void* stream);
int dcx_nchw_to_c4(const float* d_nchw, int n, int c, int h, int w, float* d_c4, void* stream);
int dcx_c4_to_nchw(const float* d_c4, int n, int c, int h, int w, float* d_nchw, void* stream);

int dcx_set_timing(int enabled);
int dcx_get_timing(void);
int dcx_last_timings(float* h_ms4);

const char* dcx_conv_pick_name(int n, int cin, int ho, int wo, int cout, int ks, int pool, int epi);
const char* dcx_conv_pick_name_ups(int n, int cin, int ho, int wo, int cout, int ks, int pool, int epi, int ups);

int dcx_set_deterministic(int enabled);
int dcx_get_deterministic(void);

int dcx_set_tail_fence(int enabled);
int dcx_get_tail_fence(void);

int dcx_calibrate_xcd(int rounds, float* w8_out, void* stream);
int dcx_set_xcd_weights(const float* w8);
int dcx_get_xcd_weights(float* w8);

int dcx_profile_enable(int enabled);
int dcx_profile_enabled(void);
int dcx_profile_count(void);
int dcx_profile_filter(int kernel_id);
int dcx_profile_sample(int every);
int dcx_profile_fetch(int* kernel_ids, int* n_images, int* limited, double* flops_per_image, float* ms,
                      int max_records);
const char* dcx_profile_kernel_name(int kernel_id);
int dcx_profile_clocks(float* ghz, int max_records);
int dcx_profile_probe_words(int record, unsigned long long* out64);

#ifdef __cplusplus
}
#endif
#endif
```

Before: 10480 frames/s.

## Split first-layer prefetch into occupancy-bounded ranges overlapping prior detector

Adds a range-based first-conv launch using a grid-stride kernel with a bounded number of blocks per CU, reading weights from a single packed device image. Also adds an optional split where part of the batch's conv1 waits only on a mid-detector event of the previous batch, so it can overlap the previous detector's later layers. By default the split fraction is zero, but the remaining range runs through the bounded-occupancy kernel, aiming to leave CUs free for the concurrent compute stream. The risk is that lower conv1 parallelism lengthens the side-stream work.

```diff
diff --git a/deepcharuco_amd/_lib.py b/deepcharuco_amd/_lib.py
--- a/deepcharuco_amd/_lib.py
+++ b/deepcharuco_amd/_lib.py
@@ -63,6 +63,10 @@
     "dcx_detector_front": (_i, [_vp, _vp, _l, _i, _i, _i, _i, _i, _vp, _sz, _vp]),
     "dcx_infer_batch_prefetched": (_i, [_vp, _vp, _vp, _l, _i, _i, _i, _i, _i, _i, _i, _vp, _sz, _vp, _sz, _vp, _vp, _vp, _vp, _vp,
                                        _vp, _vp]),
+    "dcx_detector_front_range": (_i, [_vp, _vp, _l, _i, _i, _i, _i, _i, _vp, _sz, _i, _i, _i, _i, _vp]),
+    "dcx_infer_batch_prefetched_mid": (_i, [_vp, _vp, _vp, _l, _i, _i, _i, _i, _i, _i, _i, _vp, _sz, _vp, _sz, _vp, _vp, _vp, _vp, _vp,
+                                           _vp, _vp, _vp]),
+    "dcx_front_schedule": (_i, [_i, _i, _i, C.POINTER(_i), C.POINTER(_i), C.POINTER(_i)]),
     "dcx_stream_synchronize": (_i, [_vp]),
     "dcx_solve_pnp_pool": (_i, [_vp, _vp, _vp, _vp, _i, _i, _i, _i, C.c_double, C.POINTER(C.c_double), C.POINTER(C.c_double), _i,
                                _vp, _vp, _vp]),
diff --git a/deepcharuco_amd/csrc/dcx_api.hip b/deepcharuco_amd/csrc/dcx_api.hip
--- a/deepcharuco_amd/csrc/dcx_api.hip
+++ b/deepcharuco_amd/csrc/dcx_api.hip
@@ -113,6 +113,7 @@
     float* bias = nullptr;
     float* alpha = nullptr;
     float* beta = nullptr;
+    float* image = nullptr;
     int cin = 0, cout = 0, cout_pad = 0, ks = 3;
 };
 
@@ -129,6 +130,7 @@
     if (l.bias) (void)hipFree(l.bias);
     if (l.alpha) (void)hipFree(l.alpha);
     if (l.beta) (void)hipFree(l.beta);
+    if (l.image) (void)hipFree(l.image);
     l = DevLayer();
 }
 
@@ -169,6 +171,14 @@
     if (rc == 0) rc = upload(pad_vec(h.b, 64, 64), &l.bias);
     if (rc == 0) rc = upload(al, &l.alpha);
     if (rc == 0) rc = upload(be, &l.beta);
+    if (rc == 0) {
+        std::vector<float> image(w);
+        const std::vector<float> bias = pad_vec(h.b, 64, 64);
+        image.insert(image.end(), bias.begin(), bias.end());
+        image.insert(image.end(), al.begin(), al.end());
+        image.insert(image.end(), be.begin(), be.end());
+        rc = (int)image.size() == kConv1ImageFloats ? upload(image, &l.image) : DCX_E_SHAPE;
+    }
     if (rc != 0) { free_layer(l); return rc; }
     *out = l;
     return 0;
@@ -347,7 +357,7 @@
 int detector_run(const dcx_detector* det, const uint8_t* d_frames_u8, long frame_stride, int pitch, int pix,
                  const float* d_images_f32, int batch, int height, int width, void* d_ws, size_t ws_bytes,
                  bool with_heads, float* d_loc_nchw, float* d_ids_nchw, int32_t* zero_words, int n_zero, const float* act0,
-                 void* stream) {
+                 hipEvent_t mid, void* stream) {
     if (!det || !d_ws) return DCX_E_ARG;
     if ((d_frames_u8 == nullptr) == (d_images_f32 == nullptr)) return DCX_E_ARG;
     if (batch <= 0 || height < 8 || width < 8) return DCX_E_SHAPE;
@@ -370,6 +380,7 @@
     float* dst = buf1;
     for (const Step& st : steps) {
         const DevLayer& l = det->enc[st.layer];
+        if (st.layer == 5 && mid) DCX_CHECK_HIP(hipEventRecord(mid, s));
         DcxConvArgs a = conv_args(l, src, batch, l.cin / 4, 0, h / st.div, w / st.div, 0, 1, dst, l.cout / 4, nullptr);
         rc = dcx_launch_conv_mfma(a, 3, st.pool, DCX_EPI_BNRELU, s);
         if (rc) return rc;
@@ -402,7 +413,7 @@
                                     const float* d_images_f32, int batch, int height, int width, void* d_ws,
                                     size_t ws_bytes, float* d_loc_nchw, float* d_ids_nchw, void* stream) {
     return detector_run(det, d_frames_u8, frame_stride, pitch, DCX_PIX_GRAY8, d_images_f32, batch, height, width, d_ws, ws_bytes, true,
-                        d_loc_nchw, d_ids_nchw, nullptr, 0, nullptr, stream);
+                        d_loc_nchw, d_ids_nchw, nullptr, 0, nullptr, nullptr, stream);
 }
 
 extern "C" int dcx_detector_decode(const dcx_detector* det, int batch, int height, int width, void* d_ws,
@@ -590,10 +601,37 @@
                           (int32_t*)(front + F.ctrl), F.ctrl_words, (hipStream_t)stream);
 }
 
+extern "C" int dcx_detector_front_range(const dcx_detector* det, const uint8_t* d_frames_u8, long frame_stride, int pitch,
+                                        int pixel_format, int batch, int height, int width, void* d_front, size_t front_bytes,
+                                        int lo, int hi, int clear_ctrl, int occ, void* stream) {
+    if (!d_front) return DCX_E_ARG;
+    if (const int rc = check_batch_args(det, d_frames_u8, pitch, pixel_format, batch, height, width)) return rc;
+    if (lo < 0 || hi < lo || hi > batch) return DCX_E_SHAPE;
+    if (occ < 0 || occ > kConv1MaxOcc) return DCX_E_ARG;
+    const FrontWs F = front_layout(batch, height, width);
+    if (front_bytes < F.total) return DCX_E_WS;
+    if (lo == hi) return 0;
+    char* front = (char*)d_front;
+    hipStream_t s = (hipStream_t)stream;
+    float* act = (float*)(front + F.act);
+    int32_t* ctrl = clear_ctrl ? (int32_t*)(front + F.ctrl) : nullptr;
+    const DevLayer& l = det->first;
+    const int pt0 = dcx_prof_begin(DCX_PROF_CONV1A, hi - lo, 0, s);
+    int rc;
+    if (occ == 0)
+        rc = dcx_launch_conv1_u8(d_frames_u8 + (size_t)lo * frame_stride, frame_stride, pitch, pixel_format, hi - lo, height, width, 1,
+                                 l.w, l.bias, l.alpha, l.beta, act + (size_t)lo * 64 * height * width, nullptr, ctrl, F.ctrl_words, s);
+    else
+        rc = dcx_launch_conv1_u8_range(d_frames_u8, frame_stride, pitch, pixel_format, lo, hi, height, width, 1, l.image, act, ctrl,
+                                       F.ctrl_words, occ, s);
+    if (rc) return rc;
+    return dcx_prof_end(pt0, s);
+}
+
 namespace {
 int infer_range(const dcx_detector* det, const dcx_refiner* rf, const uint8_t* d_frames_u8, long frame_stride, int pitch, int pix,
                 int batch, int height, int width, int dust_bin, int pool, char* ws, size_t ws_bytes, char* front,
-                hipEvent_t detector_done, int32_t* d_counts, int32_t* d_starts, int32_t* d_rows, float* d_xy, float* d_conf,
+                hipEvent_t detector_mid, hipEvent_t detector_done, int32_t* d_counts, int32_t* d_starts, int32_t* d_rows, float* d_xy, float* d_conf,
                 hipStream_t s, bool timing) {
     void* stream = (void*)s;
     const PipeWs L = pipe_layout(det, rf, batch, height, width, pool);
@@ -603,7 +641,8 @@
     const FrontWs F = front_layout(batch, height, width);
     int32_t* ctrl = (int32_t*)(front ? front + F.ctrl : ws + L.ctrl);
     rc = detector_run(det, d_frames_u8, frame_stride, pitch, pix, nullptr, batch, height, width, ws + L.det, L.table - L.det,
-                      false, nullptr, nullptr, ctrl, L.ctrl_words, front ? (const float*)(front + F.act) : nullptr, stream);
+                      false, nullptr, nullptr, ctrl, L.ctrl_words, front ? (const float*)(front + F.act) : nullptr, detector_mid,
+                      stream);
     if (rc) return rc;
     if (detector_done) DCX_CHECK_HIP(hipEventRecord(detector_done, s));
     if (timing && (rc = timing_mark(1, s))) return rc;
@@ -646,14 +685,14 @@
     hipStream_t s = (hipStream_t)stream;
     char* ws = (char*)d_ws;
     return infer_range(det, rf, d_frames_u8, frame_stride, pitch, pixel_format, batch, height, width, dust_bin, pool, ws, ws_bytes,
-                       nullptr, nullptr, d_counts, d_starts, d_rows, d_xy, d_conf, s, true);
-}
-
-extern "C" int dcx_infer_batch_prefetched(const dcx_detector* det, const dcx_refiner* rf, const uint8_t* d_frames_u8,
-                                          long frame_stride, int pitch, int pixel_format, int batch, int height, int width,
-                                          int dust_bin, int pool, void* d_ws, size_t ws_bytes, void* d_front, size_t front_bytes,
-                                          int32_t* d_counts, int32_t* d_starts, int32_t* d_rows, float* d_xy, float* d_conf,
-                                          void* detector_done_event, void* stream) {
+                       nullptr, nullptr, nullptr, d_counts, d_starts, d_rows, d_xy, d_conf, s, true);
+}
+
+namespace {
+int infer_prefetched(const dcx_detector* det, const dcx_refiner* rf, const uint8_t* d_frames_u8, long frame_stride, int pitch,
+                     int pixel_format, int batch, int height, int width, int dust_bin, int pool, void* d_ws, size_t ws_bytes,
+                     void* d_front, size_t front_bytes, int32_t* d_counts, int32_t* d_starts, int32_t* d_rows, float* d_xy,
+                     float* d_conf, void* mid_event, void* done_event, void* stream) {
     if (!d_ws || !d_front || !d_counts || !d_starts || !d_rows) return DCX_E_ARG;
     if (rf != nullptr && d_xy == nullptr) return DCX_E_ARG;
     if (const int rc = check_batch_args(det, d_frames_u8, pitch, pixel_format, batch, height, width)) return rc;
@@ -661,8 +700,30 @@
     if (const int rc = dcx_check_dust_bin(dust_bin)) return rc;
     if (front_bytes < front_layout(batch, height, width).total) return DCX_E_WS;
     return infer_range(det, rf, d_frames_u8, frame_stride, pitch, pixel_format, batch, height, width, dust_bin, pool, (char*)d_ws,
-                       ws_bytes, (char*)d_front, (hipEvent_t)detector_done_event, d_counts, d_starts, d_rows, d_xy, d_conf,
-                       (hipStream_t)stream, true);
+                       ws_bytes, (char*)d_front, (hipEvent_t)mid_event, (hipEvent_t)done_event, d_counts, d_starts, d_rows, d_xy,
+                       d_conf, (hipStream_t)stream, true);
+}
+}
+
+extern "C" int dcx_infer_batch_prefetched(const dcx_detector* det, const dcx_refiner* rf, const uint8_t* d_frames_u8,
+                                          long frame_stride, int pitch, int pixel_format, int batch, int height, int width,
+                                          int dust_bin, int pool, void* d_ws, size_t ws_bytes, void* d_front, size_t front_bytes,
+                                          int32_t* d_counts, int32_t* d_starts, int32_t* d_rows, float* d_xy, float* d_conf,
+                                          void* detector_done_event, void* stream) {
+    return infer_prefetched(det, rf, d_frames_u8, frame_stride, pitch, pixel_format, batch, height, width, dust_bin, pool, d_ws,
+                            ws_bytes, d_front, front_bytes, d_counts, d_starts, d_rows, d_xy, d_conf, nullptr, detector_done_event,
+                            stream);
+}
+
+extern "C" int dcx_infer_batch_prefetched_mid(const dcx_detector* det, const dcx_refiner* rf, const uint8_t* d_frames_u8,
+                                              long frame_stride, int pitch, int pixel_format, int batch, int height, int width,
+                                              int dust_bin, int pool, void* d_ws, size_t ws_bytes, void* d_front,
+                                              size_t front_bytes, int32_t* d_counts, int32_t* d_starts, int32_t* d_rows,
+                                              float* d_xy, float* d_conf, void* detector_mid_event, void* detector_done_event,
+                                              void* stream) {
+    return infer_prefetched(det, rf, d_frames_u8, frame_stride, pitch, pixel_format, batch, height, width, dust_bin, pool, d_ws,
+                            ws_bytes, d_front, front_bytes, d_counts, d_starts, d_rows, d_xy, d_conf, detector_mid_event,
+                            detector_done_event, stream);
 }
 
 extern "C" int dcx_stream_synchronize(void* stream) { return (int)hipStreamSynchronize((hipStream_t)stream); }
diff --git a/deepcharuco_amd/csrc/dcx_common.h b/deepcharuco_amd/csrc/dcx_common.h
--- a/deepcharuco_amd/csrc/dcx_common.h
+++ b/deepcharuco_amd/csrc/dcx_common.h
@@ -69,6 +69,10 @@
 int dcx_launch_conv1_u8(const uint8_t* frames, long frame_stride, int pitch, int pix, int n, int h, int w, int pad,
                         const float* w9x64, const float* bias, const float* alpha, const float* beta,
                         float* out_c4, const int* n_limit, int32_t* zero_words, int n_zero, hipStream_t s);
+constexpr int kConv1MaxOcc = 8;
+constexpr int kConv1ImageFloats = 9 * 64 + 3 * 64;
+int dcx_launch_conv1_u8_range(const uint8_t* frames, long frame_stride, int pitch, int pix, int lo, int hi, int h, int w, int pad,
+                              const float* image, float* out_c4, int32_t* zero_words, int n_zero, int occ, hipStream_t s);
 int dcx_launch_conv1_f32(const float* images, long image_stride, int pitch, int n, int h, int w, int pad,
                          const float* w9x64, const float* bias, const float* alpha, const float* beta,
                          float* out_c4, const int* n_limit, hipStream_t s);
diff --git a/deepcharuco_amd/csrc/dcx_conv_mfma.hip b/deepcharuco_amd/csrc/dcx_conv_mfma.hip
--- a/deepcharuco_amd/csrc/dcx_conv_mfma.hip
+++ b/deepcharuco_amd/csrc/dcx_conv_mfma.hip
@@ -281,6 +281,7 @@
     return cus[dev];
 }
 
+constexpr int kFrontSplitPercent = 0, kFrontOccA = 3, kFrontOccB = 8;
 int dcx_env_knob(DcxKnob k) {
     static struct { const char* name; int unset; bool read; int value; } knobs[DCX_KNOB_COUNT] = {
         {"DCX_DETERMINISTIC", 0},
@@ -291,9 +292,25 @@
         {"DCX_W2HS_ROUNDS", 1},
         {"DCX_W2PS", 7},
         {"DCX_PROBE_U0", 0},
+        {"DCX_FRONT_SPLIT", -1},
+        {"DCX_FRONT_OCC_A", kFrontOccA},
+        {"DCX_FRONT_OCC_B", kFrontOccB},
     };
     if (!knobs[k].read) { const char* e = getenv(knobs[k].name); knobs[k].value = e ? atoi(e) : knobs[k].unset; knobs[k].read = true; }
     return knobs[k].value;
+}
+
+extern "C" int dcx_front_schedule(int batch, int height, int width, int* k, int* occ_a, int* occ_b) {
+    if (!k || !occ_a || !occ_b) return DCX_E_ARG;
+    if (batch <= 0 || height <= 0 || width <= 0) return DCX_E_SHAPE;
+    int pct = dcx_env_knob(DCX_KNOB_FRONT_SPLIT);
+    if (pct < 0) pct = kFrontSplitPercent;
+    if (pct > 100) pct = 100;
+    auto clamp_occ = [](int v, int lo) { return v < lo ? lo : v > kConv1MaxOcc ? kConv1MaxOcc : v; };
+    *k = (int)(((long)batch * pct + 50) / 100);
+    *occ_a = clamp_occ(dcx_env_knob(DCX_KNOB_FRONT_OCC_A), 1);
+    *occ_b = clamp_occ(dcx_env_knob(DCX_KNOB_FRONT_OCC_B), 0);
+    return 0;
 }
 
 namespace {
diff --git a/deepcharuco_amd/csrc/dcx_conv_shared.h b/deepcharuco_amd/csrc/dcx_conv_shared.h
--- a/deepcharuco_amd/csrc/dcx_conv_shared.h
+++ b/deepcharuco_amd/csrc/dcx_conv_shared.h
@@ -121,7 +121,7 @@
 int dcx_device_cu_count();
 int dcx_fill_xcd_cum(DcxConvArgs& a);
 enum DcxKnob { DCX_KNOB_DETERMINISTIC, DCX_KNOB_XCD_WALK, DCX_KNOB_OCC, DCX_KNOB_CT_OUTER, DCX_KNOB_W2HS, DCX_KNOB_W2HS_ROUNDS,
-               DCX_KNOB_W2PS, DCX_KNOB_PROBE_U0, DCX_KNOB_COUNT };
+               DCX_KNOB_W2PS, DCX_KNOB_PROBE_U0, DCX_KNOB_FRONT_SPLIT, DCX_KNOB_FRONT_OCC_A, DCX_KNOB_FRONT_OCC_B, DCX_KNOB_COUNT };
 int dcx_env_knob(DcxKnob k);
 
 template <void (*KERNEL)(const DcxConvArgs)>
diff --git a/deepcharuco_amd/csrc/dcx_first_dev.h b/deepcharuco_amd/csrc/dcx_first_dev.h
--- a/deepcharuco_amd/csrc/dcx_first_dev.h
+++ b/deepcharuco_amd/csrc/dcx_first_dev.h
@@ -48,7 +48,7 @@
     return inb ? v : 0.0f;
 }
 
-constexpr int kConv1LdsFloats = 9 * 64 + 3 * 64;
+constexpr int kConv1LdsFloats = kConv1ImageFloats;
 __device__ __forceinline__ void dcx_conv1_stage(float* sw, const float* __restrict__ w9x64, const float* __restrict__ bias,
                                                 const float* __restrict__ alpha, const float* __restrict__ beta) {
     const int tid = threadIdx.x;
diff --git a/deepcharuco_amd/csrc/dcx_misc.hip b/deepcharuco_amd/csrc/dcx_misc.hip
--- a/deepcharuco_amd/csrc/dcx_misc.hip
+++ b/deepcharuco_amd/csrc/dcx_misc.hip
@@ -1,6 +1,8 @@
 #include "dcx_cell_dev.h"
 #include "dcx_common.h"
 #include "dcx_first_dev.h"
+
+int dcx_device_cu_count();
 
 #include <stdlib.h>
 
@@ -41,6 +43,30 @@
 }
 
 template <typename PX>
+__global__ __launch_bounds__(256) void dcx_conv1_bounded_kernel(const uint8_t* __restrict__ in, long image_stride, int pitch,
+                                                                  int h, int w, int pad, const float4* __restrict__ image,
+                                                                  float* __restrict__ out, int ho, int wo, int lo, int hi, int bpi,
+                                                                  int32_t* __restrict__ zero_words, int n_zero) {
+    dcx_zero_words(zero_words, n_zero);
+    float4* out4 = reinterpret_cast<float4*>(out);
+    const int total = (hi - lo) * bpi;
+    for (int blk = blockIdx.x; blk < total; blk += gridDim.x) {
+        const int f = blk / bpi;
+        const int n = lo + f, p = (blk - f * bpi) * 256 + threadIdx.x;
+        if (p >= ho * wo) continue;
+        const int oy = p / wo, ox = p - oy * wo;
+        const uint8_t* img = in + (size_t)n * image_stride;
+        float x[9];
+#pragma unroll
+        for (int dy = 0; dy < 3; ++dy)
+#pragma unroll
+            for (int dx = 0; dx < 3; ++dx) x[dy * 3 + dx] = dcx_px_padded<PX>(img, pitch, h, w, oy - pad + dy, ox - pad + dx);
+#pragma unroll 1
+        for (int cq = 0; cq < 16; ++cq) out4[((size_t)n * 16 + cq) * (size_t)(ho * wo) + p] = dcx_conv1_quad(image, x, cq);
+    }
+}
+
+template <typename PX>
 __global__ __launch_bounds__(256) void dcx_conv1_tile_kernel(const uint8_t* __restrict__ in, long image_stride, int pitch,
                                                                int h, int w, int pad,
                                                                const float* __restrict__ w9x64,
@@ -162,6 +188,22 @@
                                           n_zero, s);
     });
 }
+int dcx_launch_conv1_u8_range(const uint8_t* frames, long frame_stride, int pitch, int pix, int lo, int hi, int h, int w, int pad,
+                              const float* image, float* out_c4, int32_t* zero_words, int n_zero, int occ, hipStream_t s) {
+    if (!frames || !image || !out_c4) return DCX_E_ARG;
+    if (occ < 1 || occ > kConv1MaxOcc) return DCX_E_ARG;
+    const int ho = h + 2 * pad - 2, wo = w + 2 * pad - 2;
+    if (ho <= 0 || wo <= 0 || lo < 0 || hi <= lo) return DCX_E_SHAPE;
+    const long bpi = ((long)ho * wo + 255) / 256, total = bpi * (hi - lo);
+    if ((long)ho * wo > 0x3fffffffL || total > 0x3fffffffL) return DCX_E_SHAPE;
+    const long cap = (long)occ * dcx_device_cu_count();
+    const unsigned grid = (unsigned)(total < cap ? total : cap);
+    return dcx_with_pix(pix, [&](auto px) {
+        hipLaunchKernelGGL((dcx_conv1_bounded_kernel<decltype(px)>), dim3(grid), dim3(256), 0, s, frames, frame_stride, pitch, h, w, pad,
+                           reinterpret_cast<const float4*>(image), out_c4, ho, wo, lo, hi, (int)bpi, zero_words, n_zero);
+        return (int)hipGetLastError();
+    });
+}
 int dcx_launch_conv1_f32(const float* images, long image_stride, int pitch, int n, int h, int w, int pad,
                          const float* w9x64, const float* bias, const float* alpha, const float* beta,
                          float* out_c4, const int* n_limit, hipStream_t s) {
diff --git a/deepcharuco_amd/inference.py b/deepcharuco_amd/inference.py
--- a/deepcharuco_amd/inference.py
+++ b/deepcharuco_amd/inference.py
@@ -137,13 +137,16 @@
 
 def launch_pipeline(det, ref, frames_ptr: int, b: int, h: int, w: int, bpp: int, pix: int, dust_bin_ids: int, pool: int,
                     ws: torch.Tensor, out_ptr: int, conf: bool = False, front: Optional[torch.Tensor] = None,
-                    detector_done: Optional[int] = None) -> None:
+                    detector_done: Optional[int] = None, detector_mid: Optional[int] = None) -> None:
     counts_p, starts_p, rows_p, xy_p, conf_p = ptrs(out_ptr, b, pool)
     head = (det.handle, ref.handle if ref else None, frames_ptr, h * w * bpp, w * bpp, pix, b, h, w, dust_bin_ids, pool,
             ws.data_ptr(), ws.numel())
     tail = (counts_p, starts_p, rows_p, xy_p if ref else None, conf_p if conf else None, _lib.current_stream())
     if front is None:
         _lib.check(_lib.lib().dcx_infer_batch(*head, *tail), "dcx_infer_batch")
+    elif detector_mid is not None:
+        _lib.check(_lib.lib().dcx_infer_batch_prefetched_mid(*head, front.data_ptr(), front.numel(), *tail[:-1], detector_mid,
+                                                             detector_done, tail[-1]), "dcx_infer_batch_prefetched_mid")
     else:
         _lib.check(_lib.lib().dcx_infer_batch_prefetched(*head, front.data_ptr(), front.numel(), *tail[:-1], detector_done, tail[-1]),
                    "dcx_infer_batch_prefetched")
@@ -152,6 +155,19 @@
 def launch_front(det, frames_ptr: int, b: int, h: int, w: int, bpp: int, pix: int, front: torch.Tensor) -> None:
     _lib.check(_lib.lib().dcx_detector_front(det.handle, frames_ptr, h * w * bpp, w * bpp, pix, b, h, w, front.data_ptr(),
                                              front.numel(), _lib.current_stream()), "dcx_detector_front")
+
+
+def launch_front_range(det, frames_ptr: int, b: int, h: int, w: int, bpp: int, pix: int, front: torch.Tensor, lo: int, hi: int,
+                       clear_ctrl: bool, occ: int) -> None:
+    _lib.check(_lib.lib().dcx_detector_front_range(det.handle, frames_ptr, h * w * bpp, w * bpp, pix, b, h, w, front.data_ptr(),
+                                                   front.numel(), lo, hi, int(clear_ctrl), occ, _lib.current_stream()),
+               "dcx_detector_front_range")
+
+
+def front_schedule(b: int, h: int, w: int):
+    k, oa, ob = _ctypes.c_int(), _ctypes.c_int(), _ctypes.c_int()
+    _lib.check(_lib.lib().dcx_front_schedule(b, h, w, _ctypes.byref(k), _ctypes.byref(oa), _ctypes.byref(ob)), "dcx_front_schedule")
+    return k.value, oa.value, ob.value
 
 
 def pipeline_workspace(det, ref, b: int, h: int, w: int, pool: int, ws: Optional[torch.Tensor] = None) -> torch.Tensor:
diff --git a/deepcharuco_amd/stream.py b/deepcharuco_amd/stream.py
--- a/deepcharuco_amd/stream.py
+++ b/deepcharuco_amd/stream.py
@@ -10,7 +10,7 @@
 
 from . import _lib
 from .corner_pool import views
-from .inference import (DEFAULT_KMAX, PIXEL_FORMATS, infer_batch, infer_batch_device, launch_front, launch_pipeline, packed_len, pipeline_workspace, solve_pnp_submit,
+from .inference import (DEFAULT_KMAX, PIXEL_FORMATS, infer_batch, infer_batch_device, front_schedule, launch_front, launch_front_range, launch_pipeline, packed_len, pipeline_workspace, solve_pnp_submit,
                         unpack_results)
 from .models._handles import unwrap
 from .pnp import (POSE_WORDS, ransac_workspace_bytes, solve_pnp_batch_device, solve_pnp_pool, solve_pnp_ransac_batch_device,
@@ -164,7 +164,8 @@
 
     def __init__(self, dust_bin_ids: int, deepc, refinenet=None, batch: int = 32, height: int = 240, width: int = 320,
                  kmax: int = DEFAULT_KMAX, compute_streams: int = 1, depth: Optional[int] = None, bgr: bool = False,
-                 raw: bool = False, timing: bool = False, prefetch: Optional[bool] = None):
+                 raw: bool = False, timing: bool = False, prefetch: Optional[bool] = None,
+                 front_cut: Optional[Tuple[float, int, int]] = None):
         det = unwrap(deepc)
         self.dev = det.device
         self.dust_bin_ids, self.deepc, self.refinenet = dust_bin_ids, deepc, refinenet
@@ -202,9 +203,14 @@
                     self.side = torch.cuda.Stream()
                     self.ev_front = [torch.cuda.Event() for _ in range(depth)]
                     self.ev_det = [torch.cuda.Event() for _ in range(depth)]
-                    for e in self.ev_det:
+                    self.ev_mid = [torch.cuda.Event() for _ in range(depth)]
+                    for e in self.ev_det + self.ev_mid:
                         e.record(self.side)
                     self._last_det: Optional[torch.cuda.Event] = None
+                    self._last_mid: Optional[torch.cuda.Event] = None
+                    self._cuts = {}
+                    self._front_cut = front_cut
+                    self._use_mid = (front_schedule(batch, height, width)[0] if front_cut is None else front_cut[0]) > 0
         self._pending: List[Optional[Tuple[int, torch.Tensor, torch.cuda.Stream]]] = [None] * depth
         self._ticket = 0
         self.gpu_ms: List[float] = []
@@ -264,13 +270,26 @@
             front = None
             if self._front is not None:
                 front = self._front[self._ticket % 2]
+                if n not in self._cuts:
+                    cut = self._front_cut
+                    self._cuts[n] = front_schedule(n, self.h, self.w) if cut is None else (
+                        min(n, max(0, int(n * cut[0] + 0.5))), int(cut[1]), int(cut[2]))
+                k, occ_a, occ_b = self._cuts[n]
                 with torch.cuda.stream(self.side):
                     self.side.wait_event(self.ev_in[slot])
-                    if self._last_det is not None:
-                        self.side.wait_event(self._last_det)
-                    launch_front(det, frames.data_ptr(), n, self.h, self.w, bpp, pix, front)
+                    if k > 0:
+                        if self._last_mid is not None:
+                            self.side.wait_event(self._last_mid)
+                        launch_front_range(det, frames.data_ptr(), n, self.h, self.w, bpp, pix, front, 0, k, True, occ_a)
+                    if k < n:
+                        if self._last_det is not None:
+                            self.side.wait_event(self._last_det)
+                        if k == 0 and occ_b == 0:
+                            launch_front(det, frames.data_ptr(), n, self.h, self.w, bpp, pix, front)
+                        else:
+                            launch_front_range(det, frames.data_ptr(), n, self.h, self.w, bpp, pix, front, k, n, k == 0, occ_b)
                     self.ev_front[slot].record(self.side)
-                self._last_det = self.ev_det[slot]
+                self._last_det, self._last_mid = self.ev_det[slot], self.ev_mid[slot] if self._use_mid else None
             with torch.cuda.stream(compute):
                 compute.wait_event(self.ev_in[slot])
                 if self.timing:
@@ -279,7 +298,8 @@
                     compute.wait_event(self.ev_front[slot])
                 launch_pipeline(det, ref, frames.data_ptr(), n, self.h, self.w, bpp, pix, self.dust_bin_ids, self.pool,
                                 pipeline_workspace(det, ref, n, self.h, self.w, self.pool), self.pin_out[slot].data_ptr(), front=front,
-                                detector_done=self.ev_det[slot].cuda_event if front is not None else None)
+                                detector_done=self.ev_det[slot].cuda_event if front is not None else None,
+                                detector_mid=self.ev_mid[slot].cuda_event if front is not None and self._use_mid else None)
                 self.ev_done[slot].record(compute)
         self._pending[slot] = (self._ticket, frames, compute)
         self._ticket += 1
diff --git a/include/deepcharuco_amd.h b/include/deepcharuco_amd.h
--- a/include/deepcharuco_amd.h
+++ b/include/deepcharuco_amd.h
@@ -89,6 +89,16 @@
                                void* d_ws, size_t ws_bytes, void* d_front, size_t front_bytes,
                                int32_t* d_counts, int32_t* d_starts, int32_t* d_rows, float* d_xy, float* d_conf,
                                void* detector_done_event, void* stream);
+int dcx_detector_front_range(const dcx_detector* det, const uint8_t* d_frames_u8, long frame_stride, int pitch, int pixel_format,
+                             int batch, int height, int width, void* d_front, size_t front_bytes,
+                             int lo, int hi, int clear_ctrl, int occ, void* stream);
+int dcx_infer_batch_prefetched_mid(const dcx_detector* det, const dcx_refiner* rf,
+                                   const uint8_t* d_frames_u8, long frame_stride, int pitch, int pixel_format,
+                                   int batch, int height, int width, int dust_bin, int pool,
+                                   void* d_ws, size_t ws_bytes, void* d_front, size_t front_bytes,
+                                   int32_t* d_counts, int32_t* d_starts, int32_t* d_rows, float* d_xy, float* d_conf,
+                                   void* detector_mid_event, void* detector_done_event, void* stream);
+int dcx_front_schedule(int batch, int height, int width, int* k, int* occ_a, int* occ_b);
 int dcx_stream_synchronize(void* stream);
 
 #define DCX_PNP_OK          0
```

After: 10500 frames/s (median of 2 runs). About the same (+0.2%).
